# Nextomics/NextPolish2

Measured on AMD Instinct MI355X. Metric: polished reference Mbp/s (whole node) at 30x HiFi + k21/k31; FASTA identical to oracle, higher is better.
Workload: dtype u8

## Files before the change

### nextpolish2_amd/csrc/np2_cand.hip

```cpp
#include "np2_common.hpp"
#include "np2_kernels.hpp"
#include "np2_blockscan.hpp"
#include "np2_lookback.hpp"

namespace np2 {

template <int MODE>
__device__ __forceinline__ void k_scan_small(const uint32_t np2_bid, const uint32_t np2_nb, const uint32_t *__restrict__ in, uint32_t *__restrict__ out,
                                                     uint32_t n_host, const uint32_t *__restrict__ n_dev,
                                                     uint32_t *__restrict__ total_out, bool write_end) {
    __shared__ uint32_t sh[16];
    const uint32_t n = n_dev ? min(*n_dev, n_host) : n_host;
    uint32_t total;
    if (MODE == 2) {
        total = block_scan_array<OpMinI32>(
            n, sh, [&](uint32_t i) { return in[i]; },
            [&](uint32_t i, uint32_t pre, uint32_t v) { out[i] = OpMinI32::apply(pre, v); });
    } else {
        total = block_scan_array<OpAdd>(
            n, sh, [&](uint32_t i) { return in[i]; },
            [&](uint32_t i, uint32_t pre, uint32_t v) { out[i] = MODE == 0 ? pre : pre + v; });
    }
    if (threadIdx.x == 0) {
        if (MODE == 0 && write_end) out[n] = total;
        if (total_out) *total_out = total;
    }
}

static constexpr uint32_t SCAN_LB_ITEMS = 8;
static constexpr uint32_t SCAN_LB_THREADS = 1024;
static constexpr uint32_t SCAN_LB_BLOCK = SCAN_LB_ITEMS * SCAN_LB_THREADS;
template <bool POPC>
__device__ __forceinline__ void scan_lb_excl_body(const uint32_t np2_bid, const uint32_t np2_nb, Lookback lb, uint32_t n_blocks, const uint32_t *__restrict__ in,
                                                      uint32_t *__restrict__ out, uint32_t n, bool write_end,
                                                      uint32_t *__restrict__ err) {
    __shared__ uint32_t sh[16];
    const uint32_t bid = lb_block_id(lb, sh);
    const uint32_t i0 = bid * SCAN_LB_BLOCK + threadIdx.x * SCAN_LB_ITEMS;
    uint32_t v[SCAN_LB_ITEMS], sum = 0;
    const bool wide = (((uintptr_t)in | (uintptr_t)out) & 15) == 0;
    if (wide && i0 + SCAN_LB_ITEMS <= (POPC ? n - 1 : n)) {
        const uint4 a = *reinterpret_cast<const uint4 *>(in + i0), b = *reinterpret_cast<const uint4 *>(in + i0 + 4);
        v[0] = a.x, v[1] = a.y, v[2] = a.z, v[3] = a.w, v[4] = b.x, v[5] = b.y, v[6] = b.z, v[7] = b.w;
    } else {
#pragma unroll
        for (uint32_t k = 0; k < SCAN_LB_ITEMS; ++k) v[k] = i0 + k < (POPC ? n - 1 : n) ? in[i0 + k] : 0u;
    }
    if (POPC) {
#pragma unroll
        for (uint32_t k = 0; k < SCAN_LB_ITEMS; ++k) v[k] = (uint32_t)__builtin_popcount(v[k]);
    }
#pragma unroll
    for (uint32_t k = 0; k < SCAN_LB_ITEMS; ++k) sum += v[k];
    uint32_t total, pre, dummy;
    uint32_t run = block_excl_scan<OpAdd, 16>(sum, sh, total);
    lb_exclusive2(lb, bid, total, 0u, sh, err, pre, dummy);
    run += pre;
    if (wide && i0 + SCAN_LB_ITEMS <= n) {
        uint4 a, b;
        a.x = run, a.y = a.x + v[0], a.z = a.y + v[1], a.w = a.z + v[2];
        b.x = a.w + v[3], b.y = b.x + v[4], b.z = b.y + v[5], b.w = b.z + v[6];
        *reinterpret_cast<uint4 *>(out + i0) = a;
        *reinterpret_cast<uint4 *>(out + i0 + 4) = b;
        run = b.w + v[7];
    } else {
#pragma unroll
        for (uint32_t k = 0; k < SCAN_LB_ITEMS; ++k) {
            if (i0 + k < n) out[i0 + k] = run;
            run += v[k];
        }
    }
    if (write_end && n && i0 <= n - 1 && n - 1 < i0 + SCAN_LB_ITEMS) out[n] = run;
    if (write_end && n == 0 && bid == 0 && threadIdx.x == 0) out[0] = 0;
}

__device__ __forceinline__ void k_scan_lb_excl(const uint32_t np2_bid, const uint32_t np2_nb, Lookback lb, uint32_t n_blocks, const uint32_t *__restrict__ in,
                                               uint32_t *__restrict__ out, uint32_t n, bool write_end, uint32_t *__restrict__ err) {
    scan_lb_excl_body<false>(np2_bid, np2_nb, lb, n_blocks, in, out, n, write_end, err);
}
__device__ __forceinline__ void k_scan_lb_popc(const uint32_t np2_bid, const uint32_t np2_nb, Lookback lb, uint32_t n_blocks, const uint32_t *__restrict__ in,
                                               uint32_t *__restrict__ out, uint32_t n, bool write_end, uint32_t *__restrict__ err) {
    scan_lb_excl_body<true>(np2_bid, np2_nb, lb, n_blocks, in, out, n, write_end, err);
}

struct CandCtx {
    const np2_read_t *reads;
    const uint8_t *nib;
    const uint64_t *ck_off;
    const uint32_t *ckpt;
    const uint32_t *lq_start;
    const uint32_t *lq_end;
    const uint32_t *pj;
    const uint32_t *pcount;
    const uint8_t *alive;
    const ReadInfo *rinfo;
    const uint32_t *tile_rd_off;
    const uint32_t *tile_rd;
    uint32_t n_tiles;
    uint32_t ksize;
    const uint64_t *rec_key;
    const uint32_t *rec_read;
    const uint32_t *tile_n;
    const uint16_t *rec_pidx;
    uint32_t bucket_cap;
    const uint32_t *refnib;
    uint32_t L;
};

__device__ __forceinline__ void cand_anchor(const CandCtx &cx, uint32_t r, const np2_read_t &rd, uint64_t ck_off, uint32_t start,
                                            uint32_t &col, uint32_t &t) {
    col = 0;
    t = rd.aln_t_s;
    const uint32_t ck_first = (rd.aln_t_s + CKPT - 1) >> CKPT_SHIFT;
    const uint32_t cki = start >> CKPT_SHIFT;
    if (r == 0) {
        col = start;
        t = start;
    } else if (cki >= ck_first) {
        col = cx.ckpt[ck_off + (cki - ck_first)];
        t = cki << CKPT_SHIFT;
    }
}

__device__ __forceinline__ uint32_t nth_col16(uint64_t m64, uint32_t n) {
    uint32_t col = 0;
    uint32_t m = (uint32_t)m64;
    uint32_t c = (uint32_t)__builtin_popcount(m);
    if (n > c) n -= c, col = 8, m = (uint32_t)(m64 >> 32);
    c = (uint32_t)__builtin_popcount(m & 0xFFFFu);
    if (n > c) n -= c, col += 4, m >>= 16;
    c = (uint32_t)__builtin_popcount(m & 0xFFu);
    if (n > c) n -= c, col += 2, m >>= 8;
    c = (uint32_t)__builtin_popcount(m & 0xFu);
    if (n > c) col += 1;
    return col;
}

__device__ uint32_t cand_measure(const CandCtx &cx, uint32_t r, const np2_read_t &rd, uint64_t ck_off, uint32_t start,
                                 uint32_t end, uint32_t &col_start) {
    uint32_t col_ck, t_ck;
    cand_anchor(cx, r, rd, ck_off, start, col_ck, t_ck);
    col_start = col_ck;
    if (end < t_ck) return 0;
    const uint32_t want_s = (start > t_ck ? start - t_ck : 0u) + 1;
    const uint32_t want_e = end + 1 - t_ck + 1;
    const uint8_t *base = cx.nib + rd.nib_off;
    const uint32_t n_cols = rd.n_cols;
    uint32_t seen = 0, len = 0;
    bool started = false;
    uint4 win = make_uint4(0, 0, 0, 0);
    uint32_t win_blk = 0xFFFFFFFFu;
    const uint64_t N1 = 0x1111111111111111ULL;
    for (uint32_t wi = col_ck >> 4;; ++wi) {
        const uint32_t c0 = wi << 4;
        if (c0 >= n_cols) break;
        if ((wi >> 1) != win_blk) {
            win_blk = wi >> 1;
            win = *reinterpret_cast<const uint4 *>(base + ((size_t)win_blk << 4));
        }
        const uint32_t r0 = (wi & 1) ? win.z : win.x, r1 = (wi & 1) ? win.w : win.y;
        const uint64_t w = (uint64_t)(((r0 & 0x0F0F0F0Fu) << 4) | ((r0 >> 4) & 0x0F0F0F0Fu)) |
                           ((uint64_t)(((r1 & 0x0F0F0F0Fu) << 4) | ((r1 >> 4) & 0x0F0F0F0Fu)) << 32);
        uint64_t valid = N1;
        if (c0 < col_ck) valid &= ~((1ULL << (4 * (col_ck - c0))) - 1ULL);
        if (n_cols - c0 < 16) valid &= (1ULL << (4 * (n_cols - c0))) - 1ULL;
        uint64_t nonins = (~(w >> 3)) & valid;
        if (c0 == 0) nonins |= valid & 1ULL;
        const uint64_t x = (w & 0x7777777777777777ULL) ^ 0x4444444444444444ULL;
        const uint64_t nongap = (x | (x >> 1) | (x >> 2)) & valid;
        const uint32_t cn = (uint32_t)__builtin_popcountll(nonins);
        uint32_t lo = 0, hi = 16;
        bool done = false;
        if (!started && seen + cn >= want_s) {
            lo = nth_col16(nonins, want_s - seen);
            col_start = c0 + lo;
            started = true;
        }
        if (seen + cn >= want_e) {
            hi = nth_col16(nonins, want_e - seen);
            done = true;
        }
        if (started) {
            uint64_t m = nongap;
            if (lo) m &= ~((1ULL << (4 * lo)) - 1ULL);
            if (hi < 16) m &= (1ULL << (4 * hi)) - 1ULL;
            len += (uint32_t)__builtin_popcountll(m);
        }
        seen += cn;
        if (done) break;
    }
    return started ? len : 0u;
}

struct NibReader {
    const uint8_t *base;
    uint64_t w;
    uint32_t wbase;
    __device__ __forceinline__ uint8_t get(uint32_t c) {
        const uint32_t b = c & ~15u;
        if (b != wbase) {
            const uint2 v = *reinterpret_cast<const uint2 *>(base + (b >> 1));
            const uint32_t x = ((v.x & 0x0F0F0F0Fu) << 4) | ((v.x >> 4) & 0x0F0F0F0Fu);
            const uint32_t y = ((v.y & 0x0F0F0F0Fu) << 4) | ((v.y >> 4) & 0x0F0F0F0Fu);
            w = (uint64_t)x | ((uint64_t)y << 32);
            wbase = b;
        }
        return (uint8_t)((w >> (4 * (c & 15))) & 15);
    }
};

__device__ void cand_write(const CandCtx &cx, uint32_t r, const np2_read_t &rd, uint32_t pj, uint32_t g, uint32_t col, uint32_t t,
                           uint32_t len, uint8_t *__restrict__ seq_out, uint64_t *kmer_out) {
    const uint8_t *base = cx.nib + rd.nib_off;
    const uint32_t limit = cx.lq_end[pj] + cx.ksize;
    bool have_kmer = false;
    if (col + cx.ksize <= rd.n_cols) {
        const uint32_t k = cx.ksize, W0 = col >> 4, sh = (col & 15) * 4;
        auto ld = [&](uint32_t W) -> uint64_t {
            const uint2 v = *reinterpret_cast<const uint2 *>(base + ((size_t)W << 3));
            const uint32_t x = ((v.x & 0x0F0F0F0Fu) << 4) | ((v.x >> 4) & 0x0F0F0F0Fu);
            const uint32_t y = ((v.y & 0x0F0F0F0Fu) << 4) | ((v.y >> 4) & 0x0F0F0F0Fu);
            return (uint64_t)x | ((uint64_t)y << 32);
        };
        const uint64_t x0 = ld(W0), x1 = ld(W0 + 1), x2 = ld(W0 + 2);
        uint64_t lo = sh ? (x0 >> sh) | (x1 << (64 - sh)) : x0, hi = sh ? (x1 >> sh) | (x2 << (64 - sh)) : x1;
        auto nmask = [](uint32_t n) -> uint64_t { return n >= 16 ? ~0ULL : ((1ULL << (4 * n)) - 1ULL); };
        const uint64_t N1 = 0x1111111111111111ULL;
        const uint32_t avail = min(32u, rd.n_cols - col);
        const uint64_t a_lo = nmask(avail), a_hi = avail > 16 ? nmask(avail - 16) : 0ULL;
        const uint64_t ng_lo = ~(lo >> 2) & N1 & a_lo, ng_hi = ~(hi >> 2) & N1 & a_hi;
        const uint32_t c_lo = (uint32_t)__builtin_popcountll(ng_lo);
        if (c_lo + (uint32_t)__builtin_popcountll(ng_hi) >= k) {
            uint32_t kk = k, C = 0;
            uint64_t m = ng_lo;
            if (kk > c_lo) kk -= c_lo, C = 16, m = ng_hi;
            uint32_t c = (uint32_t)__builtin_popcount((uint32_t)m);
            if (kk > c) kk -= c, C += 8, m >>= 32;
            uint32_t m32 = (uint32_t)m;
            c = (uint32_t)__builtin_popcount(m32 & 0xFFFFu);
            if (kk > c) kk -= c, C += 4, m32 >>= 16;
            c = (uint32_t)__builtin_popcount(m32 & 0xFFu);
            if (kk > c) kk -= c, C += 2, m32 >>= 8;
            c = (uint32_t)__builtin_popcount(m32 & 0xFu);
            if (kk > c) C += 1;
            const uint64_t u_lo = nmask(C + 1), u_hi = C + 1 > 16 ? nmask(C + 1 - 16) : 0ULL;
            const uint64_t hi4_lo = (lo >> 2) & N1 & u_lo, hi4_hi = (hi >> 2) & N1 & u_hi;
            const bool plain = (((lo | (lo >> 1)) & hi4_lo) | ((hi | (hi >> 1)) & hi4_hi)) == 0;
            const uint64_t r_lo = nmask(C) & ~0xFULL, r_hi = C > 16 ? nmask(C - 16) : 0ULL;
            const uint32_t ins = (uint32_t)__builtin_popcountll(lo & r_lo & 0x8888888888888888ULL) +
                                 (uint32_t)__builtin_popcountll(hi & r_hi & 0x8888888888888888ULL);
            const uint32_t steps = C ? C - 1 : 0u;
            if (plain && t + (steps - ins) <= limit) {
                lo &= u_lo, hi &= u_hi;
                uint64_t g_lo = hi4_lo, g_hi = hi4_hi;
                while (g_lo | g_hi) {
                    if (g_lo) {
                        const uint64_t below = (g_lo & (0 - g_lo)) - 1;
                        lo = (lo & below) | (((lo >> 4) | (hi << 60)) & ~below);
                        g_lo = ((g_lo >> 4) | (g_hi << 60)) & ~below;
                        hi >>= 4;
                        g_hi >>= 4;
                    } else {
                        const uint64_t below = (g_hi & (0 - g_hi)) - 1;
                        hi = (hi & below) | ((hi >> 4) & ~below);
                        g_hi = (g_hi >> 4) & ~below;
                    }
                }
                auto squeeze = [](uint64_t x) -> uint64_t {
                    uint64_t y = x & 0x3333333333333333ULL;
                    y = (y | (y >> 2)) & 0x0F0F0F0F0F0F0F0FULL;
                    y = (y | (y >> 4)) & 0x00FF00FF00FF00FFULL;
                    y = (y | (y >> 8)) & 0x0000FFFF0000FFFFULL;
                    return (y | (y >> 16)) & 0xFFFFFFFFULL;
                };
                const uint64_t mask = (1ULL << (2 * (uint64_t)k)) - 1;
                const uint64_t codes = (squeeze(lo) | (squeeze(hi) << 32)) & mask;
                uint64_t rb = __builtin_bitreverse64(codes);
                rb = ((rb >> 1) & 0x5555555555555555ULL) | ((rb & 0x5555555555555555ULL) << 1);
                const uint64_t fw = rb >> (64 - 2 * k), rv = ~codes & mask;
                *kmer_out = yak_hash64(fw < rv ? fw : rv, mask);
                have_kmer = true;
            }
        }
    }
    if (!have_kmer) {
        NibReader nr{base, 0, 0xFFFFFFFFu};
        const uint64_t ksize = cx.ksize, shift = 2 * (ksize - 1), mask = (1ULL << (2 * ksize)) - 1;
        uint64_t fw = 0, rv = 0, l = 0;
        for (uint32_t c = col; c < rd.n_cols && l < ksize; ++c) {
            const uint8_t nb = nr.get(c);
            if (c != col && !(nb & 8)) ++t;
            const uint8_t q = nb & 7;
            if (q != 4) {
                fw = ((fw << 2) | (uint64_t)q) & mask;
                rv = (rv >> 2) | ((3ULL ^ (uint64_t)q) << shift);
                ++l;
            }
            if (t > limit) break;
        }
        uint64_t km = INVALID_KMER;
        if (l >= ksize) km = yak_hash64(fw < rv ? fw : rv, mask);
        *kmer_out = km;
    }
    const uint32_t LUT_LO = 0x54474341u, LUT_HI = 0x004D4E2Du;
    uint32_t o = 0;
    for (uint32_t wi = col >> 3; o < len; ++wi) {
        const uint32_t raw = *reinterpret_cast<const uint32_t *>(base + ((size_t)wi << 2));
        uint32_t w = (((raw & 0x0F0F0F0Fu) << 4) | ((raw >> 4) & 0x0F0F0F0Fu)) & 0x77777777u;
        uint32_t nc = 8;
        if (wi == (col >> 3)) {
            const uint32_t skip = col & 7;
            w >>= 4 * skip;
            nc = 8 - skip;
        }
        const uint32_t vm = nc == 8 ? 0x11111111u : ((1u << (4 * nc)) - 1u) & 0x11111111u;
        const uint32_t x = w ^ 0x44444444u;
        uint32_t gap = ~(x | (x >> 1) | (x >> 2)) & vm;
        const uint32_t cnt = min(nc - (uint32_t)__builtin_popcount(gap), len - o);
        while (gap) {
            const uint32_t below = (gap & (0u - gap)) - 1u;
            w = (w & below) | ((w >> 4) & ~below);
            gap = (gap >> 4) & ~below;
        }
        const uint32_t lo4 = w & 0xFFFFu, hi4 = w >> 16;
        uint32_t s0 = (lo4 | (lo4 << 8)) & 0x00FF00FFu, s1 = (hi4 | (hi4 << 8)) & 0x00FF00FFu;
        s0 = (s0 | (s0 << 4)) & 0x0F0F0F0Fu;
        s1 = (s1 | (s1 << 4)) & 0x0F0F0F0Fu;
        const uint32_t a0 = __builtin_amdgcn_perm(LUT_HI, LUT_LO, s0), a1 = __builtin_amdgcn_perm(LUT_HI, LUT_LO, s1);
        if (cnt == 8) {
            __builtin_memcpy(seq_out + o, &a0, 4);
            __builtin_memcpy(seq_out + o + 4, &a1, 4);
        } else {
            const uint64_t a = (uint64_t)a0 | ((uint64_t)a1 << 32);
#pragma unroll
            for (uint32_t k = 0; k < 7; ++k)
                if (k < cnt) seq_out[o + k] = (uint8_t)(a >> (8 * k));
        }
        o += cnt;
    }
}

__device__ __forceinline__ uint32_t wave_sum(uint32_t v) {
    for (int o = 32; o > 0; o >>= 1) v += __shfl_xor(v, o);
    return v;
}
__device__ __forceinline__ uint32_t wave_excl(uint32_t v) {
    const uint32_t lane = threadIdx.x & 63;
    uint32_t x = v;
#pragma unroll
    for (int o = 1; o < 64; o <<= 1) {
        const uint32_t t = __shfl_up(x, o);
        if (lane >= (uint32_t)o) x += t;
    }
    return x - v;
}

static constexpr uint32_t RM_WAVES = 8;
static constexpr uint32_t RM_RPW = 4;
static_assert(RM_RPW % 4 == 0 && RM_RPW <= 16, "regions per wavefront");
static constexpr uint32_t RM_REG = 4 * RM_RPW;
static constexpr uint32_t CAND_CLEAN = 0xFFFFFFFFu;
static constexpr uint32_t CLEAN_MAX_LEN = 64;

__device__ __forceinline__ void wave_lds_sync() {
    __builtin_amdgcn_fence(__ATOMIC_RELEASE, "wavefront");
    __builtin_amdgcn_wave_barrier();
    __builtin_amdgcn_fence(__ATOMIC_ACQUIRE, "wavefront");
}
__device__ __forceinline__ uint32_t lanes_below(uint64_t m) {
    return __builtin_amdgcn_mbcnt_hi((uint32_t)(m >> 32), __builtin_amdgcn_mbcnt_lo((uint32_t)m, 0u));
}
__device__ __forceinline__ np2_read_t rinfo_read(const ReadInfo &ri) {
    return np2_read_t{ri.aln_t_s, ri.aln_t_e, (uint64_t)ri.nib16 << 4, ri.n_cols, 0u};
}

__device__ __forceinline__ void region_measure_inline(const CandCtx &cx, uint32_t g, uint32_t st, uint32_t en, uint32_t la, uint32_t lb,
                                                      uint32_t *__restrict__ kept_read, uint32_t *__restrict__ kept_len,
                                                      uint32_t *__restrict__ kept_col, uint32_t &kept, uint32_t &bytes, uint32_t &mx) {
    const uint32_t lane = threadIdx.x & 63;
    kept = 0, bytes = 0, mx = 0;
    for (uint32_t c0 = la; c0 < lb && kept < LQSEQ_MAX_CAN_COUNT; c0 += 64) {
        const uint32_t i = c0 + lane;
        uint32_t r = 0, len = 0, col = 0;
        if (i < lb) {
            r = cx.tile_rd[i];
            const ReadInfo ri = cx.rinfo[r];
            if (ri.pcount != 0 && ri.pj <= g && g - ri.pj < ri.pcount) len = cand_measure(cx, r, rinfo_read(ri), ri.ck_off, st, en, col);
        }
        const uint64_t ne = __ballot(len > 0);
        const uint32_t before = kept + lanes_below(ne);
        const bool keep = len > 0 && before < LQSEQ_MAX_CAN_COUNT;
        if (keep) {
            const size_t slot = (size_t)g * LQSEQ_MAX_CAN_COUNT + before;
            kept_read[slot] = r;
            kept_len[slot] = len;
            kept_col[slot] = col;
        }
        kept = min(kept + (uint32_t)__builtin_popcountll(ne), (uint32_t)LQSEQ_MAX_CAN_COUNT);
        bytes += wave_sum(keep ? len : 0u);
        mx = max(mx, keep ? len : 0u);
    }
    for (int o = 32; o > 0; o >>= 1) mx = max(mx, (uint32_t)__shfl_xor(mx, o));
}

__device__ __forceinline__ void k_region_measure(const uint32_t np2_bid0, const uint32_t np2_nb, CandCtx cx, uint32_t n_reg, uint32_t *__restrict__ kept_read,
                                                        uint32_t *__restrict__ kept_len, uint32_t *__restrict__ kept_col,
                                                        uint32_t *__restrict__ reg_ncand, uint32_t *__restrict__ reg_bytes,
                                                        uint32_t *__restrict__ reg_maxlen, uint32_t *__restrict__ blk_sum) {
    const uint32_t np2_bid = xcd_order(np2_bid0, np2_nb);
    __shared__ uint32_t s_reads[RM_REG][64];
    __shared__ uint32_t s_dm[RM_REG][2];
    __shared__ uint32_t s_len[RM_REG][64];
    __shared__ uint32_t s_col[RM_REG][64];
    __shared__ uint32_t s_q[4][RM_RPW * 64];
    const uint32_t lane = threadIdx.x & 63, wv = (uint32_t)__builtin_amdgcn_readfirstlane((int)(threadIdx.x >> 6));
    const uint32_t n_mb = (n_reg + 3) / 4, g0 = (np2_bid * 4 + wv) * RM_RPW, mb0 = g0 / 4;
    uint32_t nq = 0;
    uint32_t st[RM_RPW], en[RM_RPW], tile[RM_RPW], la[RM_RPW], lb[RM_RPW], tn[RM_RPW];
    bool live[RM_RPW];
#pragma unroll
    for (uint32_t h = 0; h < RM_RPW; ++h) {
        const uint32_t g = g0 + h;
        live[h] = g < n_reg;
        const uint32_t gg = live[h] ? g : n_reg - 1;
        st[h] = cx.lq_start[gg], en[h] = cx.lq_end[gg];
    }
#pragma unroll
    for (uint32_t h = 0; h < RM_RPW; ++h) {
        tile[h] = min(en[h] >> TILE_SHIFT, cx.n_tiles - 1);
        la[h] = cx.tile_rd_off[tile[h]], lb[h] = cx.tile_rd_off[tile[h] + 1];
        tn[h] = cx.rec_pidx ? cx.tile_n[tile[h]] : 0u;
    }
    const ReadInfo r0 = cx.rinfo[0];
    uint32_t rr[RM_RPW], lo[RM_RPW], hi[RM_RPW], refw[RM_RPW];
    bool wok[RM_RPW];
#pragma unroll
    for (uint32_t h = 0; h < RM_RPW; ++h) {
        const uint32_t g = g0 + h, nlist = lb[h] - la[h], we = en[h] + cx.ksize + 2;
        wok[h] = live[h] && cx.rec_pidx != nullptr && nlist != 0 && nlist <= 64 && en[h] - st[h] + 1 <= CLEAN_MAX_LEN && we < cx.L &&
                 (st[h] >> TILE_SHIFT) == tile[h] && (we >> TILE_SHIFT) == tile[h] && tn[h] <= cx.bucket_cap &&
                 r0.pcount != 0 && r0.pj <= g && g - r0.pj < r0.pcount;
        rr[h] = (wok[h] && lane < nlist) ? cx.tile_rd[la[h] + lane] : 0xFFFFFFFFu;
        const uint32_t w0 = st[h] >> 3, w1 = (en[h] + cx.ksize) >> 3;
        refw[h] = 0;
        if (wok[h] && w0 + lane <= w1) {
            uint32_t m = 0x44444444u;
            if (lane == 0) m &= 0xFFFFFFFFu << (4 * (st[h] & 7));
            if (w0 + lane == w1) m &= 0xFFFFFFFFu >> (4 * (7 - ((en[h] + cx.ksize) & 7)));
            refw[h] = cx.refnib[w0 + lane] & m;
        }
        lo[h] = 0, hi[h] = 0;
        if (wok[h] && tn[h]) {
            const uint32_t tstart = tile[h] << TILE_SHIFT;
            const uint32_t j0 = (st[h] - tstart) >> 4, j1 = ((we - tstart) >> 4) + 1;
            lo[h] = cx.rec_pidx[(size_t)tile[h] * (TILE / 16) + j0];
            hi[h] = j1 < TILE / 16 ? (uint32_t)cx.rec_pidx[(size_t)tile[h] * (TILE / 16) + j1] : tn[h];
        }
    }
    uint32_t pjv[RM_RPW], pcv[RM_RPW], tev[RM_RPW], rpos[RM_RPW], rq[RM_RPW];
#pragma unroll
    for (uint32_t h = 0; h < RM_RPW; ++h) {
        pjv[h] = 0, pcv[h] = 0, tev[h] = 0, rpos[h] = 0xFFFFFFFFu, rq[h] = 0;
        if (rr[h] != 0xFFFFFFFFu) {
            const uint4 q = *reinterpret_cast<const uint4 *>(&cx.rinfo[rr[h]].aln_t_e);
            tev[h] = q.x, pjv[h] = q.y, pcv[h] = q.z;
        }
        const uint32_t i = lo[h] + lane;
        if (i < hi[h]) {
            const uint64_t a = (uint64_t)tile[h] * cx.bucket_cap + i;
            rpos[h] = (uint32_t)(cx.rec_key[a] >> 32), rq[h] = cx.rec_read[a];
        }
    }
    uint32_t fastmask = 0;
#pragma unroll
    for (uint32_t h = 0; h < RM_RPW; ++h) {
        const uint32_t slot = wv * RM_RPW + h;
        const bool fast = wok[h] && (uint32_t)__builtin_amdgcn_readfirstlane((int)rr[h]) == 0 && __ballot(refw[h] != 0) == 0;
        if (fast) fastmask |= 1u << h;
        s_reads[slot][lane] = rr[h];
        if (lane < 2) s_dm[slot][lane] = 0;
    }
    wave_lds_sync();
    auto mark = [&](uint32_t slot, uint32_t nlist, uint32_t pos, uint32_t q, uint32_t ws, uint32_t we) {
        if (pos >= ws && pos <= we) {
            uint32_t x = 0, y = nlist;
            while (x < y) {
                const uint32_t m = (x + y) >> 1;
                if (s_reads[slot][m] < q) x = m + 1; else y = m;
            }
            if (x < nlist && s_reads[slot][x] == q) atomicOr(&s_dm[slot][x >> 5], 1u << (x & 31));
        }
    };
#pragma unroll
    for (uint32_t h = 0; h < RM_RPW; ++h) {
        if (!((fastmask >> h) & 1u)) continue;
        const uint32_t slot = wv * RM_RPW + h, nlist = lb[h] - la[h], ws = st[h], we = en[h] + cx.ksize + 2;
        mark(slot, nlist, rpos[h], rq[h], ws, we);
        for (uint32_t c0 = lo[h] + 64; c0 < hi[h]; c0 += 64) {
            const uint32_t i = c0 + lane;
            if (i < hi[h]) {
                const uint64_t a = (uint64_t)tile[h] * cx.bucket_cap + i;
                mark(slot, nlist, (uint32_t)(cx.rec_key[a] >> 32), cx.rec_read[a], ws, we);
            }
        }
    }
    wave_lds_sync();
    uint32_t state[RM_RPW];
#pragma unroll
    for (uint32_t h = 0; h < RM_RPW; ++h) {
        state[h] = 0;
        if (!((fastmask >> h) & 1u)) continue;
        const uint32_t g = g0 + h, slot = wv * RM_RPW + h;
        const bool paired = rr[h] != 0xFFFFFFFFu && pcv[h] != 0 && pjv[h] <= g && g - pjv[h] < pcv[h];
        const bool marked = (s_dm[slot][lane >> 5] >> (lane & 31)) & 1u;
        const bool ends_inside = tev[h] < en[h] + cx.ksize;
        const uint32_t stt = !paired ? 0u : ((marked || ends_inside) && rr[h] != 0) ? 2u : 1u;
        state[h] = stt;
        const uint64_t dq = __ballot(stt == 2u);
        if (stt == 2u) s_q[wv][nq + lanes_below(dq)] = (slot << 6) | lane;
        nq += (uint32_t)__builtin_popcountll(dq);
    }
    uint32_t sum_k[RM_RPW / 4] = {}, sum_b[RM_RPW / 4] = {}, sum_m[RM_RPW / 4] = {};
#pragma unroll
    for (uint32_t h = 0; h < RM_RPW; ++h) {
        if (!live[h] || ((fastmask >> h) & 1u)) continue;
        const uint32_t g = g0 + h;
        uint32_t kept, bytes, mx;
        region_measure_inline(cx, g, st[h], en[h], la[h], lb[h], kept_read, kept_len, kept_col, kept, bytes, mx);
        if (lane == 0) {
            reg_ncand[g] = kept;
            reg_bytes[g] = bytes;
            reg_maxlen[g] = mx;
        }
        sum_k[h / 4] += kept, sum_b[h / 4] += bytes, sum_m[h / 4] += mx;
    }
    wave_lds_sync();
    for (uint32_t e = lane; e < nq; e += 64) {
        const uint32_t w = s_q[wv][e], slot = w >> 6, ln = w & 63;
        const uint32_t g = (np2_bid * 4 + slot / RM_RPW) * RM_RPW + slot % RM_RPW;
        const uint32_t r = s_reads[slot][ln];
        const ReadInfo ri = cx.rinfo[r];
        uint32_t col = 0;
        const uint32_t len = cand_measure(cx, r, rinfo_read(ri), ri.ck_off, cx.lq_start[g], cx.lq_end[g], col);
        s_len[slot][ln] = len;
        s_col[slot][ln] = col;
    }
    wave_lds_sync();
#pragma unroll
    for (uint32_t h = 0; h < RM_RPW; ++h) {
        if (!((fastmask >> h) & 1u)) continue;
        const uint32_t g = g0 + h, slot = wv * RM_RPW + h;
        uint32_t len = 0, col = CAND_CLEAN;
        if (state[h] == 1u) len = en[h] - st[h] + 1;
        else if (state[h] == 2u) len = s_len[slot][lane], col = s_col[slot][lane];
        const uint64_t ne = __ballot(len > 0);
        const uint32_t before = lanes_below(ne);
        const bool keep = len > 0 && before < LQSEQ_MAX_CAN_COUNT;
        if (keep) {
            const size_t ks = (size_t)g * LQSEQ_MAX_CAN_COUNT + before;
            kept_read[ks] = rr[h];
            kept_len[ks] = len;
            kept_col[ks] = col;
        }
        const uint32_t kept = min((uint32_t)__builtin_popcountll(ne), (uint32_t)LQSEQ_MAX_CAN_COUNT);
        const uint32_t bytes = wave_sum(keep ? len : 0u);
        uint32_t mx = keep ? len : 0u;
        for (int o = 32; o > 0; o >>= 1) mx = max(mx, (uint32_t)__shfl_xor(mx, o));
        if (lane == 0) {
            reg_ncand[g] = kept;
            reg_bytes[g] = bytes;
            reg_maxlen[g] = mx;
        }
        sum_k[h / 4] += kept, sum_b[h / 4] += bytes, sum_m[h / 4] += mx;
    }
#pragma unroll
    for (uint32_t q = 0; q < RM_RPW / 4; ++q)
        if (lane == 0 && mb0 + q < n_mb) {
            blk_sum[mb0 + q] = sum_k[q];
            blk_sum[n_mb + mb0 + q] = sum_b[q];
            blk_sum[2 * n_mb + mb0 + q] = sum_m[q];
        }
}

__device__ __forceinline__ void k_cand_offsets(const uint32_t np2_bid, const uint32_t np2_nb, const uint32_t *__restrict__ blk_sum, uint32_t n_blk,
                                                       uint32_t n_reg, uint32_t *__restrict__ blk_coff,
                                                       uint32_t *__restrict__ blk_soff, uint32_t *__restrict__ cand_off,
                                                       uint32_t *__restrict__ reg_soff, uint32_t *__restrict__ n_cand,
                                                       uint32_t *__restrict__ n_bytes, uint32_t *__restrict__ grow) {
    __shared__ uint32_t sh[16];
    const uint32_t ta = block_scan_array<OpAdd>(
        n_blk, sh, [&](uint32_t i) { return blk_sum[i]; }, [&](uint32_t i, uint32_t pre, uint32_t) { blk_coff[i] = pre; });
    const uint32_t tb = block_scan_array<OpAdd>(
        n_blk, sh, [&](uint32_t i) { return blk_sum[n_blk + i]; },
        [&](uint32_t i, uint32_t pre, uint32_t) { blk_soff[i] = pre; });
    const uint32_t tc = block_scan_array<OpAdd>(
        n_blk, sh, [&](uint32_t i) { return blk_sum[2 * n_blk + i]; }, [&](uint32_t, uint32_t, uint32_t) {});
    if (threadIdx.x == 0) {
        cand_off[n_reg] = ta;
        reg_soff[n_reg] = tb;
        *n_cand = ta;
        *n_bytes = tb;
        *grow = tc;
    }
}

__device__ __forceinline__ void k_cand_offsets_lb(const uint32_t np2_bid, const uint32_t np2_nb, Lookback lb, uint32_t n_blocks, const uint32_t *__restrict__ blk_sum,
                                                         uint32_t n_blk, uint32_t n_reg, uint32_t *__restrict__ blk_coff,
                                                         uint32_t *__restrict__ blk_soff, uint32_t *__restrict__ cand_off,
                                                         uint32_t *__restrict__ reg_soff, uint32_t *__restrict__ n_cand,
                                                         uint32_t *__restrict__ n_bytes, uint32_t *__restrict__ grow,
                                                         uint32_t *__restrict__ err) {
    __shared__ uint32_t sh[8];
    const uint32_t bid = lb_block_id(lb, sh);
    const uint32_t i0 = (bid * 256 + threadIdx.x) * 4;
    uint32_t a[4], b[4], sa = 0, sb = 0;
#pragma unroll
    for (uint32_t k = 0; k < 4; ++k) {
        a[k] = i0 + k < n_blk ? blk_sum[i0 + k] : 0u;
        b[k] = i0 + k < n_blk ? blk_sum[n_blk + i0 + k] : 0u;
        sa += a[k];
        sb += b[k];
    }
    uint32_t ta, tb, pa, pb;
    uint32_t ra = block_excl_scan<OpAdd, 4>(sa, sh, ta);
    uint32_t rb = block_excl_scan<OpAdd, 4>(sb, sh, tb);
    lb_exclusive2(lb, bid, ta, tb, sh, err, pa, pb);
    ra += pa, rb += pb;
#pragma unroll
    for (uint32_t k = 0; k < 4; ++k)
        if (i0 + k < n_blk) {
            blk_coff[i0 + k] = ra;
            blk_soff[i0 + k] = rb;
            ra += a[k];
            rb += b[k];
        }
    if (bid == n_blocks - 1 && threadIdx.x == 255) {
        cand_off[n_reg] = ra;
        reg_soff[n_reg] = rb;
        *n_cand = ra;
        *n_bytes = rb;
    }
    if (bid == 0) {
        uint32_t c = 0, tc;
        for (uint32_t i = threadIdx.x; i < n_blk; i += 256) c += blk_sum[2 * n_blk + i];
        (void)block_excl_scan<OpAdd, 4>(c, sh, tc);
        if (threadIdx.x == 0) *grow = tc;
    }
}

static constexpr uint32_t MERGE_LB_BLOCKS = 32;
__device__ __forceinline__ void k_lq_merge_scan_lb(const uint32_t np2_bid, const uint32_t np2_nb, Lookback lb, const uint32_t *__restrict__ raw_start,
                                                   const uint32_t *__restrict__ raw_end, const uint32_t *__restrict__ n_raw, uint32_t n_host,
                                                   uint32_t *__restrict__ headflag, uint32_t *__restrict__ hidx, uint32_t *__restrict__ err) {
    __shared__ uint32_t sh[16];
    const uint32_t bid = lb_block_id(lb, sh);
    const uint32_t n = min(*n_raw, n_host);
    const uint32_t seg = ((n + MERGE_LB_BLOCKS - 1) / MERGE_LB_BLOCKS + 1023u) & ~1023u;
    const uint32_t lo = min(bid * seg, n), hi = min(lo + seg, n);
    auto flag = [&](uint32_t j) { return (j >= 1 && raw_end[j] >= raw_start[j - 1]) ? 0u : 1u; };
    uint32_t cnt = 0;
    for (uint32_t j = lo + threadIdx.x; j < hi; j += 1024) cnt += flag(j);
    uint32_t total, pre, dummy;
    (void)block_excl_scan<OpAdd, 16>(cnt, sh, total);
    lb_exclusive2(lb, bid, total, 0u, sh, err, pre, dummy);
    uint32_t carry = pre;
    for (uint32_t j0 = lo; j0 < hi; j0 += 1024) {
        const uint32_t j = j0 + threadIdx.x;
        const uint32_t v = j < hi ? flag(j) : 0u;
        uint32_t tot;
        const uint32_t ex = block_excl_scan<OpAdd, 16>(v, sh, tot);
        if (j < hi) {
            hidx[j] = carry + ex;
            headflag[j] = v;
        }
        carry += tot;
    }
}

__device__ __forceinline__ void k_region_write(const uint32_t np2_bid0, const uint32_t np2_nb, CandCtx cx, uint32_t n_reg, const uint32_t *__restrict__ kept_read,
                                                      const uint32_t *__restrict__ kept_len,
                                                      const uint32_t *__restrict__ kept_col,
                                                      const uint32_t *__restrict__ reg_ncand,
                                                      const uint32_t *__restrict__ reg_bytes,
                                                      const uint32_t *__restrict__ blk_coff,
                                                      const uint32_t *__restrict__ blk_soff,
                                                      uint32_t *__restrict__ cand_off, uint32_t *__restrict__ reg_soff,
                                                      uint32_t cand_cap,
                                                      uint32_t seq_cap, uint32_t *__restrict__ cand_order,
                                                      uint64_t *__restrict__ cand_kmer, uint32_t *__restrict__ cand_seq_off,
                                                      uint8_t *__restrict__ cand_seq) {
    const uint32_t np2_bid = xcd_order(np2_bid0, np2_nb);
    __shared__ __attribute__((aligned(4))) uint8_t s_str[RM_REG][CLEAN_MAX_LEN];
    __shared__ uint64_t s_km[RM_REG];
    __shared__ uint32_t s_so[RM_REG][64];
    __shared__ uint32_t s_oc[RM_REG];
    __shared__ uint32_t s_q[4][RM_RPW * 64];
    const uint32_t lane = threadIdx.x & 63, wv = (uint32_t)__builtin_amdgcn_readfirstlane((int)(threadIdx.x >> 6));
    const uint32_t g0 = (np2_bid * 4 + wv) * RM_RPW, mb0 = g0 / 4;
    uint32_t nq = 0;
    uint32_t oc = 0, ob = 0;
    if (g0 < n_reg) oc = blk_coff[mb0], ob = blk_soff[mb0];
    uint32_t clean_h = 0;
    uint32_t my_len[RM_RPW], my_so[RM_RPW], my_ci[RM_RPW];
    bool my_clean[RM_RPW];
    uint32_t n[RM_RPW], rb[RM_RPW], st[RM_RPW], ln0[RM_RPW];
#pragma unroll
    for (uint32_t h = 0; h < RM_RPW; ++h) {
        const uint32_t g = g0 + h;
        n[h] = 0, rb[h] = 0, st[h] = 0, ln0[h] = 0;
        if (g < n_reg) n[h] = reg_ncand[g], rb[h] = reg_bytes[g], st[h] = cx.lq_start[g], ln0[h] = cx.lq_end[g] - st[h] + 1;
    }
    uint32_t len[RM_RPW], col[RM_RPW], rd_[RM_RPW], refc[RM_RPW];
#pragma unroll
    for (uint32_t h = 0; h < RM_RPW; ++h) {
        const size_t ks = (size_t)(g0 + h) * LQSEQ_MAX_CAN_COUNT + lane;
        const bool act = lane < n[h];
        len[h] = act ? kept_len[ks] : 0u;
        col[h] = act ? kept_col[ks] : 0u;
        rd_[h] = act ? kept_read[ks] : 0u;
        const uint32_t p = st[h] + lane;
        refc[h] = (n[h] && lane < ln0[h] && ln0[h] <= CLEAN_MAX_LEN) ? cx.refnib[p >> 3] >> (4 * (p & 7)) : 0u;
    }
#pragma unroll
    for (uint32_t h = 0; h < RM_RPW; ++h) {
        const uint32_t g = g0 + h, slot = wv * RM_RPW + h;
        my_len[h] = 0, my_so[h] = 0, my_ci[h] = 0, my_clean[h] = false;
        if (g >= n_reg) continue;
        if (g == n_reg - 1 && lane == 0 && cand_off[n_reg] < cand_cap) cand_seq_off[cand_off[n_reg]] = reg_soff[n_reg];
        if (lane == 0) {
            cand_off[g] = oc;
            reg_soff[g] = ob;
            s_oc[slot] = oc;
        }
        const bool act = lane < n[h];
        const uint32_t so = ob + wave_excl(len[h]);
        const uint32_t ci = oc + lane;
        const bool ok = act && ci < cand_cap && (uint64_t)so + len[h] <= seq_cap;
        if (ok) {
            cand_order[ci] = rd_[h];
            cand_seq_off[ci] = so;
        }
        const bool clean = ok && col[h] == CAND_CLEAN;
        const uint64_t cm = __ballot(clean);
        const bool queued = ok && (!clean || (lane == 0 && rd_[h] == 0));
        my_len[h] = len[h], my_so[h] = so, my_ci[h] = ci, my_clean[h] = clean && !queued;
        s_so[slot][lane] = so;
        if (cm) {
            clean_h |= 1u << h;
            if (lane < ln0[h]) s_str[slot][lane] = (uint8_t)((0x54474341u >> (8 * (refc[h] & 3))) & 0xFFu);
        }
        const uint64_t dq = __ballot(queued);
        if (queued) s_q[wv][nq + lanes_below(dq)] = (slot << 6) | lane;
        nq += (uint32_t)__builtin_popcountll(dq);
        oc += n[h];
        ob += rb[h];
    }
    wave_lds_sync();
    for (uint32_t e = lane; e < nq; e += 64) {
        const uint32_t w = s_q[wv][e], slot = w >> 6, li = w & 63;
        const uint32_t g = (np2_bid * 4 + slot / RM_RPW) * RM_RPW + slot % RM_RPW;
        const size_t ks = (size_t)g * LQSEQ_MAX_CAN_COUNT + li;
        const uint32_t r = kept_read[ks], len = kept_len[ks];
        uint32_t col = kept_col[ks];
        const ReadInfo ri = cx.rinfo[r];
        const np2_read_t rd = rinfo_read(ri);
        const uint32_t t0 = max(cx.lq_start[g], rd.aln_t_s);
        if (col == CAND_CLEAN) col = t0;
        const uint32_t ci = s_oc[slot] + li;
        uint64_t km;
        cand_write(cx, r, rd, ri.pj, g, col, t0, len, cand_seq + s_so[slot][li], &km);
        cand_kmer[ci] = km;
        if (li == 0 && r == 0) s_km[slot] = km;
    }
    wave_lds_sync();
#pragma unroll
    for (uint32_t h = 0; h < RM_RPW; ++h) {
        if (!((clean_h >> h) & 1u)) continue;
        const uint32_t slot = wv * RM_RPW + h;
        if (my_clean[h]) {
            cand_kmer[my_ci[h]] = s_km[slot];
            typedef uint32_t u32_any __attribute__((aligned(1)));
            uint8_t *dst = cand_seq + my_so[h];
            const uint32_t L4 = my_len[h] & ~3u;
            for (uint32_t j = 0; j < L4; j += 4) *reinterpret_cast<u32_any *>(dst + j) = *reinterpret_cast<const uint32_t *>(&s_str[slot][j]);
            for (uint32_t j = L4; j < my_len[h]; ++j) dst[j] = s_str[slot][j];
        }
    }
}

void launch_scan_small_excl(hipStream_t s, const uint32_t *in, uint32_t *out, uint32_t n, const uint32_t *n_dev,
                            uint32_t *total_out, bool write_end) {
    NP2_LAUNCH(k_scan_small<0>, dim3(1), 1024, s, in, out, n, n_dev, total_out, write_end);
}
void launch_scan_lb_excl(hipStream_t s, const Lookback &lb, const uint32_t *in, uint32_t *out, uint32_t n, bool write_end,
                          uint32_t *err) {
    const uint32_t nb = scan_lb_blocks(n);
    NP2_LAUNCH(k_scan_lb_excl, dim3(nb), SCAN_LB_THREADS, s, lb, nb, in, out, n, write_end, err);
}
void launch_scan_lb_popc(hipStream_t s, const Lookback &lb, const uint32_t *bits, uint32_t *out, uint32_t n_words, uint32_t *err) {
    const uint32_t nb = scan_lb_blocks((uint64_t)n_words + 1);
    NP2_LAUNCH(k_scan_lb_popc, dim3(nb), SCAN_LB_THREADS, s, lb, nb, bits, out, n_words + 1, false, err);
}
uint32_t scan_lb_blocks(uint64_t n) { return (uint32_t)std::max<uint64_t>(1, (n + SCAN_LB_BLOCK - 1) / SCAN_LB_BLOCK); }
void launch_scan_small_incl(hipStream_t s, const int32_t *in, int32_t *out, uint32_t n, const uint32_t *n_dev) {
    NP2_LAUNCH(k_scan_small<1>, dim3(1), 1024, s, (const uint32_t *)in, (uint32_t *)out, n, n_dev, (uint32_t *)nullptr, false);
}
void launch_scan_small_min(hipStream_t s, const int32_t *in, int32_t *out, uint32_t n, const uint32_t *n_dev) {
    NP2_LAUNCH(k_scan_small<2>, dim3(1), 1024, s, (const uint32_t *)in, (uint32_t *)out, n, n_dev, (uint32_t *)nullptr, false);
}
static CandCtx mk_cand(const CandPtrs &c) {
    return CandCtx{c.reads, c.nib,    c.ck_off, c.ckpt,        c.lq_start, c.lq_end, c.pj,
                   c.pcount, c.alive, c.rinfo, c.tile_rd_off, c.tile_rd, c.n_tiles,  c.ksize,
                   c.rec_key, c.rec_read, c.tile_n, c.rec_pidx, c.bucket_cap, c.refnib, c.L};
}
void launch_region_measure(hipStream_t s, const CandPtrs &c, uint32_t n_reg, uint32_t *kept_read, uint32_t *kept_len,
                           uint32_t *kept_col, uint32_t *reg_ncand, uint32_t *reg_bytes, uint32_t *reg_maxlen,
                           uint32_t *blk_sum) {
    if (n_reg)
        NP2_LAUNCH_WAVES(k_region_measure, RM_WAVES, dim3((n_reg + RM_REG - 1) / RM_REG), 256, s,
                         mk_cand(c), n_reg, kept_read, kept_len, kept_col, reg_ncand, reg_bytes, reg_maxlen, blk_sum);
}
uint32_t cand_offsets_blocks(uint32_t n_reg) { return ((n_reg + 3) / 4 + 1023) / 1024; }
void launch_cand_offsets(hipStream_t s, const uint32_t *blk_sum, uint32_t n_reg, uint32_t *blk_coff, uint32_t *blk_soff,
                         uint32_t *cand_off, uint32_t *reg_soff, uint32_t *n_cand, uint32_t *n_bytes, uint32_t *grow,
                         const Lookback *lb, uint32_t *err) {
    if (lb)
        NP2_LAUNCH(k_cand_offsets_lb, dim3(cand_offsets_blocks(n_reg)), 256, s, *lb, cand_offsets_blocks(n_reg), blk_sum, (n_reg + 3) / 4, n_reg, blk_coff, blk_soff, cand_off, reg_soff, n_cand, n_bytes, grow, err);
    else
        NP2_LAUNCH(k_cand_offsets, dim3(1), 1024, s, blk_sum, (n_reg + 3) / 4, n_reg, blk_coff, blk_soff, cand_off, reg_soff, n_cand, n_bytes, grow);
}
void launch_lq_merge_scan_lb(hipStream_t s, const Lookback &lb, const uint32_t *raw_start, const uint32_t *raw_end, const uint32_t *n_raw,
                             uint32_t n_host, uint32_t *headflag, uint32_t *hidx, uint32_t *err) {
    NP2_LAUNCH(k_lq_merge_scan_lb, dim3(MERGE_LB_BLOCKS), 1024, s, lb, raw_start, raw_end, n_raw, n_host, headflag, hidx, err);
}
uint32_t lq_merge_lb_blocks() { return MERGE_LB_BLOCKS; }
void launch_region_write(hipStream_t s, const CandPtrs &c, uint32_t n_reg, const uint32_t *kept_read,
                         const uint32_t *kept_len, const uint32_t *kept_col, const uint32_t *reg_ncand,
                         const uint32_t *reg_bytes, const uint32_t *blk_coff, const uint32_t *blk_soff, uint32_t *cand_off,
                         uint32_t *reg_soff, uint32_t cand_cap, uint32_t seq_cap, uint32_t *cand_order, uint64_t *cand_kmer,
                         uint32_t *cand_seq_off, uint8_t *cand_seq) {
    if (n_reg)
        NP2_LAUNCH(k_region_write, dim3((n_reg + RM_REG - 1) / RM_REG), 256, s, mk_cand(c), n_reg, kept_read, kept_len, kept_col, reg_ncand, reg_bytes, blk_coff, blk_soff, cand_off, reg_soff, cand_cap, seq_cap, cand_order, cand_kmer, cand_seq_off, cand_seq);
}

}
```

### nextpolish2_amd/csrc/np2_ctx.hpp

```cpp
#pragma once
#include "../../include/np2.h"
#include "np2_abi.hpp"
#include "np2_common.hpp"
#include "np2_kernels.hpp"
#include "np2_hostcpu.hpp"

#include <algorithm>
#include <chrono>
#include <cstdio>
#include <cstdlib>
#include <cstring>
#include <map>
#include <memory>
#include <exception>
#include <mutex>
#include <stdexcept>
#include <string>
#include <vector>

namespace np2h {

using namespace np2;


// ... 273 lines not shown
        }
        return true;
    }
};
inline PinnedPool &pinned_pool() {
    static PinnedPool *p = new PinnedPool();
    return *p;
}

struct PinnedBuf {
    void *p = nullptr;
    size_t cap = 0;
    ~PinnedBuf() {
        if (p) pinned_pool().put(p);
    }
    void *ensure(size_t n) {
        if (n > cap) {
            if (p) pinned_pool().put(p);
            p = nullptr;
            cap = 0;
            const size_t want = n + n / 4 + 65536;
            p = pinned_pool().get(want);
            if (!p) throw Np2Error(NP2_E_NOMEM, "hipHostMalloc failed");
            cap = want;
        }
        return p;
    }
};

struct CtxDeviceState {
    hipStream_t stream = nullptr, stream_out = nullptr;
    hipEvent_t ev_out = nullptr;
    uint32_t *mbox_host = nullptr, *mbox_dev = nullptr;
    void destroy() {
        if (ev_out) (void)hipEventDestroy(ev_out);
        if (stream_out) (void)hipStreamDestroy(stream_out);
        if (stream) (void)hipStreamDestroy(stream);
        if (mbox_host) (void)hipHostFree(mbox_host);
        *this = CtxDeviceState();
    }
};
struct CtxStatePool {
    std::mutex mu;
    std::map<int, std::vector<CtxDeviceState>> idle;
    bool get(int device, CtxDeviceState &out) {
        std::lock_guard<std::mutex> l(mu);
        auto &v = idle[device];
        if (v.empty()) return false;
        out = v.back();
        v.pop_back();
        return true;
    }
    void put(int device, CtxDeviceState &st) {
        {
            std::lock_guard<std::mutex> l(mu);
            auto &v = idle[device];
            if (v.size() < 32) {
                v.push_back(st);
                st = CtxDeviceState();
                return;
            }
        }
        st.destroy();
    }
};
inline CtxStatePool &ctx_state_pool() {
    static CtxStatePool *p = new CtxStatePool();
    return *p;
}

struct YakTable {
    uint32_t k = 0, cap_log2 = 0;
    std::shared_ptr<DevBuf<uint64_t>> table;
    std::shared_ptr<DevBuf<uint32_t>> ord;
    YakDev dev() const { return YakDev{table->p, cap_log2, k, ord ? ord->p : nullptr}; }
};

struct Timing {
    std::vector<std::string> names;
    std::vector<float> ms;
    std::string joined;
    std::vector<std::pair<std::string, float>> host;
};
inline double now_ms() {
    return std::chrono::duration<double, std::milli>(std::chrono::steady_clock::now().time_since_epoch()).count();
}


}

using namespace np2h;

struct np2_contig {
    np2_contig() {
        reads.cached = nib.cached = refnib.cached = ck_off.cached = ckpt.cached = descs.cached = true;
        tile_rd_off.cached = tile_rd.cached = true;
    }
    uint32_t L = 0, R = 0;
    uint64_t nib_bytes = 0, n_cols = 0, n_ckpt = 0;
    DevBuf<np2_read_t> reads;
    DevBuf<uint8_t> nib;
    DevBuf<uint8_t> refnib;
    uint32_t ref_stride = 0;
    DevBuf<uint64_t> ck_off;
    DevBuf<uint32_t> ckpt;
    uint32_t n_chunks = 0;
    DevBuf<ChunkDesc> descs;
    uint32_t n_tiles = 0;
    DevBuf<uint32_t> tile_rd_off, tile_rd;
    uint32_t tile_cap = TILE_CAP;
};

struct np2_ctx {
    int device = 0;
    hipStream_t stream = nullptr;
    hipStream_t stream_out = nullptr;
    hipEvent_t ev_out = nullptr;
    uint8_t *out_host[2] = {nullptr, nullptr};
    size_t out_host_cap[2] = {0, 0};
    int out_slot = 0;
    bool out_pending = false;
    uint64_t out_len = 0;
    std::vector<YakTable> yaks;
    std::string err;
    bool trace = false;
    std::map<std::string, std::vector<uint8_t>> trace_items;
    Timing timing;
    std::vector<std::pair<std::string, std::pair<hipEvent_t, hipEvent_t>>> pending_events;

    PinnedBuf pin_d2h, pin_h2d;
    uint32_t *mbox_host = nullptr, *mbox_dev = nullptr;
    uint32_t mbox_seq = 0;
    bool borrowed_state = false;
    uint8_t *sink_dst = nullptr;
    uint64_t sink_cap = 0;
    uint32_t last_first_pos = 0, last_last_pos = 0;
    const uint8_t *last_dbase = nullptr;
    const uint32_t *last_dpos = nullptr;
    DevBuf<uint32_t> shard_bounds;
    uint64_t last_len = 0;
    bool reuse_identical_pass = true;
    bool h2d_inflight = false;
    bool stage_timing = false;
    DevBuf<uint8_t> tmp;
    DevBuf<uint64_t> keys_raw, keys;
    DevBuf<uint32_t> vals_raw, vals;
    DevBuf<uint32_t> npos, ncount, nminr, nbesti, node_off, run_start, run_end, n0_besti, emit, eoff;
    DevBuf<uint16_t> nbases, ndelta;
    DevBuf<int64_t> nscore;
    DevBuf<int32_t> cov, mval, smin;
    DevBuf<uint8_t> alive, cns_base, cns_cls, lq_kind, lq_nothead;
    DevBuf<uint32_t> cns_pos, lq_next, rflag, rstart, rend, ridx, raw_start, raw_end, headflag, hidx, lq_start,
        lq_end;
    DevBuf<uint32_t> pj, pcount, reg_ncand, reg_bytes, reg_soff, reg_maxlen, blk_sum, blk_coff, blk_soff, kept_read, kept_len, kept_col, cand_off, cand_order, cand_seq_off, kill_ids;
    DevBuf<uint64_t> cand_kmer;
    DevBuf<uint8_t> cand_seq;
    DevBuf<uint16_t> kscore;
    DevBuf<uint32_t> scal;
    DevBuf<uint64_t> lb_status;
    DevBuf<uint32_t> lb_ticket;
    uint32_t lb_ticket_total = 0, lb_epoch = 0;
    bool lb_dirty = false;
    static constexpr size_t LB_MAX_BLOCKS = 1u << 20;
    DevBuf<uint32_t> mlen;
    DevBuf<uint8_t> reg_lable, grp, cns_base2, rech_groups, rech_groups_tmp;
    DevBuf<uint8_t> votepack;
    DevBuf<uint8_t> votepack2;
    DevBuf<uint32_t> rech_headjobs;
    DevBuf<uint32_t> ecount, eval, eval_s, eflag, eidx, seed_cand, keep_n, keep_list, cns_pos2, sp_idx_s,
        sp_idx_e, ap_g, ap_s, ap_e, rech, rech_joboff, job_len,
        job_off32;
    DevBuf<int32_t> ew, ap_delta, ap_shift;
    DevBuf<uint64_t> ekey, ekey_s;
    DevBuf<uint16_t> keep_ks;
    DevBuf<uint32_t> long_list;
    DevBuf<uint64_t> bt_path;
    DevBuf<uint64_t> chunk_st;
    uint32_t chunk_epoch = 0;
    DevBuf<uint32_t> tile_cur, tile_n, tile_scan, tile_scanb, tile_nn, tile_nr, tile_noff, tile_roff;
    uint32_t tile_cap = TILE_CAP;
    uint32_t bucket_cap = 0;
    DevBuf<uint2> nrec;
    DevBuf<uint8_t> votebuf;
    DevBuf<uint32_t> band, band_n, band_off;
    DevBuf<int64_t> run_gain, tile_gain;
    DevBuf<uint8_t> out_snap;
    DevBuf<uint8_t> run_flag;
    uint32_t deep_min = 65536;
    DevBuf<uint32_t> lq_list, hbits;
    DevBuf<uint16_t> tile_pidx;
    bool pidx_valid = false;
    DevBuf<ReadInfo> rinfo;
    DevBuf<uint32_t> lqc, lqoff;
    DevBuf<uint8_t> pflag;
    DevBuf<uint32_t> dp_list;
    DevBuf<uint16_t> pf_slots;
    DevBuf<uint32_t> pf_bad, pf_bad2;
    DevBuf<uint64_t> pf_prof;
    bool front_fused = false;
    struct Hooks {
        bool front_unfused = false, pf_prof = false, edge_sort = false;
        bool test_misspeculate = false, shard_spec_log = false, phase_profile = false, exact_grow = false, no_speculate = false;
        bool has_grow_guess = false;
        uint32_t grow_guess = 0;
        bool has_pf_cap = false, has_pf_cap_big = false, has_pf_halo = false, has_pf_cov_max = false;
        uint32_t pf_cap = 0, pf_cap_big = 0, pf_halo = 0, pf_cov_max = 0;
        void read() {
            auto on = [](const char *n) { return getenv(n) != nullptr; };
            auto u32 = [](const char *n, bool &has, uint32_t &v) {
                if (const char *e = getenv(n)) has = true, v = (uint32_t)atol(e);
            };
            front_unfused = on("NP2_FRONT_UNFUSED"), pf_prof = on("NP2_PF_PROF"), edge_sort = on("NP2_EDGE_SORT");
            test_misspeculate = on("NP2_TEST_MISSPECULATE");
            shard_spec_log = on("NP2_SHARD_SPEC_LOG"), phase_profile = on("NP2_PHASE_PROFILE"), exact_grow = on("NP2_EXACT_GROW");
            no_speculate = on("NP2_NO_SPECULATE");
            u32("NP2_TEST_GROW_GUESS", has_grow_guess, grow_guess);
            u32("NP2_PF_CAP", has_pf_cap, pf_cap), u32("NP2_PF_CAP_BIG", has_pf_cap_big, pf_cap_big);
            u32("NP2_PF_HALO", has_pf_halo, pf_halo), u32("NP2_PF_COV_MAX", has_pf_cov_max, pf_cov_max);
        }
    } hooks;
    bool pf_big = getenv("NP2_PF_BIG") != nullptr;
    uint32_t front_redos = 0;
    DevBuf<uint16_t> kscore_saved;
    DevBuf<uint8_t> sstr;
    DevBuf<uint64_t> soff;
    DevBuf<uint16_t> sscore;
};


namespace np2h {


enum Scal { S_ERR = 0, S_NNODES, S_NRUNS, S_BEST, S_PATHBEGIN, S_NRAW, S_NREG, S_DUP, S_LAST0, S_LAST1, S_GAIN0,
            S_GAIN1, S_DEEP, S_NDPLIST, S_NRECH, S_NGROUPS, S_NLONG, S_NLQ, S_PF, S_M0, S_M1, S_M2, S_M3, S_NC, S_SB, S_GROW,
            S_NBAD, S_PFOUT, S_PFGAIN0, S_PFGAIN1, S_PFEND0, S_PFEND1, S_NBAD2, S_PFPAD, S_COUNT = 34 };
static_assert(S_M1 % 2 == 0 && S_LAST0 % 2 == 0 && S_GAIN0 % 2 == 0 && S_PFGAIN0 % 2 == 0 && S_PFEND0 % 2 == 0,
              "64-bit device counters live in these slot pairs");

static constexpr int NP2_MAX_YAK = 15;
static constexpr uint32_t SCAL_TOTAL = 96;
static_assert(S_COUNT + 2 * (NP2_MAX_YAK + 2) <= SCAL_TOTAL && S_COUNT < 64, "round counters behind the posted block; the mailbox holds 64 words");

inline double thread_cpu_ms() {
    timespec ts;
    clock_gettime(CLOCK_THREAD_CPUTIME_ID, &ts);
    return ts.tv_sec * 1e3 + ts.tv_nsec * 1e-6;
}
struct WallTimer {
    np2_ctx *cx;
    const char *name;
    double t0, c0 = 0;
    WallTimer(np2_ctx *c, const char *n);
    ~WallTimer();
};

struct EventTimer {
    np2_ctx *cx;
    hipEvent_t a = nullptr, b = nullptr;
    bool on;
    EventTimer(np2_ctx *c, const char *name, bool always = false)
        : cx(c), on((always || c->stage_timing) && !tl_recorder()) {
        if (!on) return;
        (void)hipEventCreate(&a);
        (void)hipEventCreate(&b);
        (void)hipEventRecord(a, cx->stream);
        cx->pending_events.push_back({name, {a, b}});
    }
    ~EventTimer() {
        if (on) (void)hipEventRecord(b, cx->stream);
    }
};

inline WallTimer::WallTimer(np2_ctx *c, const char *n) : cx(c), name(n), t0(c->stage_timing ? now_ms() : 0.0), c0(c->stage_timing ? thread_cpu_ms() : 0.0) {}
inline WallTimer::~WallTimer() {
    if (cx->stage_timing) {
        cx->timing.host.push_back({name, (float)(now_ms() - t0)});
        if (strncmp(name, "wall", 4) == 0) cx->timing.host.push_back({std::string("cpu") + (name + 4), (float)(thread_cpu_ms() - c0)});
    }
}

inline void flush_timings(np2_ctx *cx) {
    std::map<std::string, float> acc;
    std::vector<std::string> order;
    for (auto &e : cx->pending_events) {
        float ms = 0;
        (void)hipEventSynchronize(e.second.second);
        (void)hipEventElapsedTime(&ms, e.second.first, e.second.second);
        if (!acc.count(e.first)) order.push_back(e.first);
        acc[e.first] += ms;
        (void)hipEventDestroy(e.second.first);
        (void)hipEventDestroy(e.second.second);
    }
    cx->pending_events.clear();
    for (auto &h : cx->timing.host) {
        if (!acc.count(h.first)) order.push_back(h.first);
        acc[h.first] += h.second;
    }
    cx->timing.host.clear();
    cx->timing.names = order;
    cx->timing.ms.clear();
    cx->timing.joined.clear();
    for (auto &n : order) {
        cx->timing.ms.push_back(acc[n]);
        cx->timing.joined += n;
        cx->timing.joined.push_back('\0');
    }
    cx->timing.joined.push_back('\0');
}
// ... 193 lines not shown
```

### nextpolish2_amd/csrc/np2_host.cpp

```cpp
#include "../../include/np2.h"
#include "np2_common.hpp"
#include "np2_kernels.hpp"
#include "np2_ctx.hpp"
#include "np2_phase_host.hpp"

#include <algorithm>
#include <atomic>
#include <thread>
#include <chrono>
#include <cstdio>
#include <cstdlib>
#include <cstring>
#include <map>
#include <mutex>
#include <stdexcept>
#include <string>
#include <unordered_map>
#include <unordered_set>
#include <future>
#include <functional>
#include <vector>

using namespace np2;

// ... 773 lines not shown
        launch_dp_short(s, gp, c->refnib.p, cx->run_start.p, cx->scal.p + S_NRUNS, n_runs, cx->run_end.p, cx->run_gain.p,
                        cx->emit.p, cx->scal.p + S_PATHBEGIN, cx->bt_path.p, dp_list, n_dp_list);
        launch_dp_long(s, gp, cx->run_start.p, n_runs, cx->nrec.p, cx->nscore.p, cx->nbesti.p, cx->n0_besti.p,
                       cx->run_end.p, (int64_t *)(cx->scal.p + S_LAST0), cx->run_gain.p, cx->emit.p,
                       cx->scal.p + S_PATHBEGIN, cx->bt_path.p, cx->run_flag.p, dp_list, n_dp_list);
        launch_dp_finish(s, gp, cx->run_start.p, cx->scal.p + S_NRUNS, cx->nscore.p, cx->nbesti.p, cx->n0_besti.p,
                         (const int64_t *)(cx->scal.p + S_LAST0), (unsigned long long *)(cx->scal.p + S_GAIN0),
                         cx->scal.p + S_DUP , cx->scal.p + S_BEST,
                         cx->run_gain.p, (const long long *)cx->tile_gain.p,
                         (c->L + TILE - 1) >> TILE_SHIFT, cx->emit.p, cx->scal.p + S_PATHBEGIN, cx->bt_path.p);
        exclusive_total(cx, cx->emit.p, cx->eoff.p, (size_t)L + 1);
        launch_bt_write(s, gp, cx->run_start.p, cx->scal.p + S_NRUNS, n_runs, cx->emit.p, cx->eoff.p, cx->bt_path.p,
                        cx->cns_pos.p, cx->cns_base.p, cx->cns_cls.p, cx->lq_nothead.p, cx->lqc.p);
        exclusive_total(cx, cx->lqc.p, cx->lqoff.p, (size_t)n_runs + 1);
        launch_lq_list(s, gp, cx->run_start.p, cx->scal.p + S_NRUNS, n_runs, cx->emit.p, cx->eoff.p, cx->bt_path.p,
                       cx->lqoff.p, lq_cap, cx->lq_list.p, cx->scal.p + S_ERR);
        launch_default_tail(s, gp, cx->scal.p + S_BEST, M_p, cx->cns_base.p, cx->cns_cls.p, cx->lq_list.p,
                            cx->lqoff.p + n_runs, lq_cap, cx->scal.p + S_ERR);
    }
    lq_regions_issue(cx, cb, M_p, n_lq);
}

bool front_can_fuse(np2_ctx *cx) {
    return !cx->hooks.front_unfused && cx->bucket_cap != 0 && cx->pidx_valid;
}
void pass_front_fused_issue(np2_ctx *cx, np2_contig *c, uint32_t T) {
    hipStream_t s = cx->stream;
    const uint32_t L = c->L;
    const uint32_t n_tiles = (L + TILE - 1) >> TILE_SHIFT;
    const CnsBounds cb = cns_buffers(cx, c, T, std::min<uint32_t>(T, L), T);
    cx->pf_slots.ensure(pf_slot_entries(n_tiles, T));
    cx->pf_bad.ensure((size_t)n_tiles + 2);
    cx->pf_bad2.ensure((size_t)n_tiles + 2);
    const np2_ctx::Hooks &hk = cx->hooks;
    const uint32_t cap_lim = hk.has_pf_cap ? hk.pf_cap : PF_CAP, cap_big = hk.has_pf_cap_big ? hk.pf_cap_big : PF_CAP_BIG,
                   halo_lim = (hk.has_pf_halo ? hk.pf_halo : PF_HALO) & ~15u, cov_max = hk.has_pf_cov_max ? hk.pf_cov_max : PF_COV_MAX;
    PfTile a{cx->keys_raw.p, cx->vals_raw.p, cx->tile_n.p, cx->tile_scan.p, cx->tile_pidx.p, cx->alive.p, c->reads.p,
             c->tile_rd_off.p, c->tile_rd.p, c->refnib.p, cx->pf_slots.p, cx->tile_nn.p, cx->tile_nr.p,
             (long long *)cx->tile_gain.p, cx->scal.p + S_PF, cx->scal.p + S_NBAD, cx->pf_bad.p, cx->scal.p + S_NBAD2, cx->pf_bad2.p,
             (long long *)(cx->scal.p + S_PFEND0), (unsigned long long *)(cx->scal.p + S_PFGAIN0), nullptr, L, n_tiles, cx->bucket_cap,
             cap_lim, cap_big, halo_lim, std::min(cov_max, cx->deep_min), cx->pf_big ? 1u : 0u};
    uint32_t *const M_p = cx->eoff.p + L;
    uint32_t *const n_lq = cx->scal.p + S_NRUNS;
    const bool prof = cx->hooks.pf_prof && tl_recorder() == nullptr;
    if (prof) {
        cx->pf_prof.ensure((size_t)n_tiles * 8 + 8);
        zero32(cx, cx->pf_prof.p, (size_t)n_tiles * 8, 8);
        a.prof = (unsigned long long *)cx->pf_prof.p;
    }
    {
        EventTimer t(cx, "pass_front");
        launch_pf_tile(s, a);
        if (prof) {
            auto st = d2h(cx, cx->pf_prof.p, (size_t)n_tiles * 8);
            double sum[8] = {0}, mx[8] = {0};
            size_t cnt = 0;
            for (uint32_t t = 0; t < n_tiles; ++t) {
                const uint64_t *q = st.data() + (size_t)t * 8;
                if (!q[7] || !q[0]) continue;
                ++cnt;
                for (int i = 1; i < 8; ++i) {
                    const double d = (double)(q[i] - q[i - 1]);
                    sum[i] += d, mx[i] = std::max(mx[i], d);
                }
            }
            {
                auto tn = d2h(cx, cx->tile_n.p, n_tiles);
                uint32_t h[6] = {0};
                for (uint32_t v : tn) ++h[v <= 480 ? 0 : v <= 960 ? 1 : v <= 1440 ? 2 : v <= 1920 ? 3 : v <= 3584 ? 4 : 5];
                fprintf(stderr, "[pf_prof] records per tile <=480 / 960 / 1440 / 1920 / 3584 / more: %u %u %u %u %u %u; ", h[0], h[1], h[2], h[3], h[4], h[5]);
            }
            fprintf(stderr, "listed for the middle / the big variant: %u / %u; ", d2h(cx, cx->scal.p + S_NBAD, 1)[0], d2h(cx, cx->scal.p + S_NBAD2, 1)[0]);
            fprintf(stderr, "tiles %zu of %u; mean / max clocks per phase (loads, cover+nodes, offsets+sort, DP, reduce, count+scan, write):", cnt, n_tiles);
            for (int i = 1; i < 8; ++i) fprintf(stderr, " %.0f/%.0f", cnt ? sum[i] / cnt : 0.0, mx[i]);
            fprintf(stderr, "\n");
        }
        const bool wide = n_tiles >= 2048;
        Lookback lb{};
        if (wide) lb = next_lookback(cx, tile_scan_blocks(n_tiles));
        launch_tile_offsets(s, cx->tile_nn.p, cx->tile_nr.p, n_tiles, cx->tile_noff.p, cx->tile_roff.p, M_p, n_lq,
                            cx->scal.p + S_BEST, S_NLQ + 1 - S_BEST, wide ? &lb : nullptr, cx->scal.p + S_ERR,
                            (const long long *)cx->tile_gain.p, (unsigned long long *)(cx->scal.p + S_PFGAIN0));
        launch_pf_compact(s, n_tiles, cx->pf_slots.p, cx->tile_scan.p, cx->tile_nn.p, cx->tile_noff.p, cx->tile_roff.p,
                          cx->cns_pos.p, cx->cns_base.p, cx->cns_cls.p, cx->lq_nothead.p, cx->lq_list.p, cb.lq_cap,
                          cx->scal.p + S_ERR, cx->scal.p + S_PF, cx->scal.p + S_PFOUT, cx->scal.p + S_NBAD, cx->scal.p + S_NBAD2);
    }
    lq_regions_issue(cx, cb, M_p, n_lq);
}

void pass_front_issue(np2_ctx *cx, np2_contig *c, uint32_t T, int pass, bool force_unfused = false) {
    cx->front_fused = !force_unfused && front_can_fuse(cx);
    if (!cx->front_fused || cx->trace) {
        uint32_t n_nodes = 0, n_runs = 0;
        {
            WallTimer w(cx, "wall_graph");
            build_graph(cx, c, T, n_nodes, n_runs);
        }
        trace_graph(cx, c, pass, n_nodes);
        if (!cx->front_fused) {
            consensus_and_regions_issue(cx, c, n_nodes, n_runs, T);
            return;
        }
    }
    pass_front_fused_issue(cx, c, T);
}
void consensus_and_regions_finish(np2_ctx *cx, np2_contig *c, uint32_t T, int pass, uint32_t &M, uint32_t &n_reg, bool whole_contig = true) {
    const uint32_t *M_p = cx->eoff.p + c->L;
    std::vector<uint32_t> sc = fetch_scal(cx, cx->scal.p + S_M0, M_p);
    if (cx->front_fused) {
        const int64_t total = (int64_t)(((uint64_t)sc[S_PFGAIN1] << 32) | sc[S_PFGAIN0]);
        const int64_t end_rel = (int64_t)(((uint64_t)sc[S_PFEND1] << 32) | sc[S_PFEND0]);
        const bool negative = end_rel <= SCORE_NEG / 2 || total + end_rel < 0;
        if (sc[S_PFOUT] & PF_NEED_BIG) cx->pf_big = true;
        if ((sc[S_PFOUT] & PF_REDO) || negative) {
            ++cx->front_redos;
            cx->timing.host.push_back({"front_redo", 1.0f});
            pass_front_issue(cx, c, T, pass, true);
            sc = fetch_scal(cx, cx->scal.p + S_M0, M_p);
        }
    }
    check_region_err(cx, sc[S_ERR]);
    if (!cx->front_fused && sc[S_BEST] == 0xFFFFFFFFu && !whole_contig)
        throw Np2Error(NP2_E_UNSUPPORTED,
                       "best path score is negative at the end of a shard (the reference's default node is chosen by the whole "
                       "contig's score): polish this contig unsharded");
    M = sc[S_M0];
    if (M == 0) throw Np2Error(NP2_E_REFPANIC, "reference would panic: empty consensus");
    n_reg = sc[S_NRAW] ? sc[S_NREG] : 0;
}

void extract_candidates(np2_ctx *cx, np2_contig *c, uint32_t n_reg, uint16_t min_kmer_count, int pass,
                        PassCounts &pc) {
    hipStream_t s = cx->stream;
    const uint32_t R = c->R;
    REFPANIC_IF(cx->yaks.empty(), "index out of bounds: opt.yak[0]");
    if ((uint64_t)n_reg * LQSEQ_MAX_CAN_COUNT >= 0xFFFFFFF0ull) throw Np2Error(NP2_E_NOMEM, "too many LQ regions");
    const uint32_t NC_cap = n_reg * LQSEQ_MAX_CAN_COUNT;
    static const uint64_t exact_from = getenv("NP2_CAND_EXACT_FROM") ? strtoull(getenv("NP2_CAND_EXACT_FROM"), nullptr, 10) : (1ull << 28);
    const bool exact_bytes = c->n_cols >= exact_from && !cx->trace;
    uint32_t SB_cap = (uint32_t)std::min<uint64_t>(c->n_cols + 64, 0xFFFFFFF0ull);
    cx->mval.ensure(R + 2);
    cx->smin.ensure(R + 2);
    cx->pj.ensure(R + 2);
    cx->pcount.ensure(R + 2);
    cx->rinfo.ensure(R + 2);
    cx->reg_ncand.ensure(n_reg + 2);
    cx->reg_bytes.ensure(n_reg + 2);
    cx->reg_soff.ensure(n_reg + 2);
    cx->reg_maxlen.ensure(n_reg + 2);
    cx->blk_sum.ensure(3 * ((size_t)n_reg / 4 + 2));
    cx->blk_coff.ensure((size_t)n_reg / 4 + 2);
    cx->blk_soff.ensure((size_t)n_reg / 4 + 2);
    cx->cand_off.ensure(n_reg + 2);
    cx->kept_read.ensure((size_t)NC_cap + 2);
    cx->kept_len.ensure((size_t)NC_cap + 2);
    cx->kept_col.ensure((size_t)NC_cap + 2);
    cx->cand_order.ensure((size_t)NC_cap + 2);
    cx->cand_kmer.ensure((size_t)NC_cap + 2);
    cx->cand_seq_off.ensure((size_t)NC_cap + 2);
    if (!exact_bytes) cx->cand_seq.ensure((size_t)SB_cap + 64);
    cx->kscore.ensure((size_t)NC_cap + 2);
    cx->long_list.ensure((size_t)NC_cap + 2);
    CandPtrs cp{c->reads.p,   c->nib.p,   c->ck_off.p,      c->ckpt.p,    cx->lq_start.p, cx->lq_end.p, cx->pj.p,
                cx->pcount.p, cx->alive.p, cx->rinfo.p, c->tile_rd_off.p, c->tile_rd.p, c->n_tiles, cx->yaks[0].k,
                cx->keys_raw.p, cx->vals_raw.p, cx->tile_n.p,
                (cx->pidx_valid && cx->bucket_cap) ? cx->tile_pidx.p : nullptr, cx->bucket_cap,
                (const uint32_t *)c->refnib.p, c->L};
    {
        EventTimer t(cx, "candidates");
        launch_read_m(s, c->reads.p, R, cx->alive.p, cx->lq_start.p, n_reg, cx->mval.p);
        scan_incl_min(cx, cx->mval.p, cx->smin.p, R);
        launch_pair_count(s, c->reads.p, R, cx->alive.p, cx->lq_start.p, cx->lq_end.p, n_reg, cx->smin.p, cx->pj.p,
                          cx->pcount.p, c->ck_off.p, cx->rinfo.p);
        launch_region_measure(s, cp, n_reg, cx->kept_read.p, cx->kept_len.p, cx->kept_col.p, cx->reg_ncand.p,
                              cx->reg_bytes.p, cx->reg_maxlen.p, cx->blk_sum.p);
        {
            const bool wide = n_reg > 0;
            Lookback lb{};
            if (wide) lb = next_lookback(cx, cand_offsets_blocks(n_reg));
            launch_cand_offsets(s, cx->blk_sum.p, n_reg, cx->blk_coff.p, cx->blk_soff.p, cx->cand_off.p, cx->reg_soff.p,
                                cx->scal.p + S_NC, cx->scal.p + S_SB, cx->scal.p + S_GROW, wide ? &lb : nullptr,
                                cx->scal.p + S_ERR);
        }
        if (exact_bytes) {
            const std::vector<uint32_t> sc = fetch_scal(cx);
            check_region_err(cx, sc[S_ERR]);
            pc.resolve(sc);
            SB_cap = (uint32_t)std::min<uint64_t>((uint64_t)pc.SB + 64, SB_cap);
            cx->cand_seq.ensure((size_t)SB_cap + 64);
        }
        launch_region_write(s, cp, n_reg, cx->kept_read.p, cx->kept_len.p, cx->kept_col.p, cx->reg_ncand.p,
                            cx->reg_bytes.p, cx->blk_coff.p, cx->blk_soff.p, cx->cand_off.p, cx->reg_soff.p, NC_cap + 1,
                            SB_cap, cx->cand_order.p, cx->cand_kmer.p, cx->cand_seq_off.p, cx->cand_seq.p);
    }
    {
        EventTimer t(cx, "kmer_score");
        launch_cand_score(s, cx->yaks[0].dev(), cx->cand_seq_off.p, cx->cand_seq.p, cx->cand_kmer.p, cx->scal.p + S_NC,
                          NC_cap, min_kmer_count, cx->kscore.p, cx->long_list.p, cx->scal.p + S_NLONG);
    }
    pc.n_reg = n_reg;
    pc.NC_cap = NC_cap;
    pc.SB_cap = SB_cap;
    pc.known = exact_bytes;
    if (cx->trace) pc.resolve(fetch_scal(cx));
    trace_region_tables(cx, pass, "cand", pc, false);
}

Cns fetch_cns(np2_ctx *cx, uint32_t M) {
    Cns c;
    c.pos = d2h(cx, cx->cns_pos.p, M);
    c.base = d2h(cx, cx->cns_base.p, M);
    return c;
}

struct ResultOut {
    uint8_t *bases = nullptr;
    uint32_t *pos = nullptr;
    uint64_t len = 0;
    bool want_pos = true;
    bool want_bases = true;
    void release() {
        if (bases) pinned_pool().put(bases), bases = nullptr;
        if (pos) pinned_pool().put(pos), pos = nullptr;
    }
};
void fetch_result(np2_ctx *cx, const uint32_t *dpos, const uint8_t *dbase, const uint32_t *M_p, uint32_t M_cap, ResultOut &r,
                  uint32_t M_likely = 0xFFFFFFFFu) {
    const double t0 = now_ms();
    std::vector<uint32_t> sc;
    if (cx->sink_dst && cx->sink_cap) launch_copy_len(cx->stream, cx->sink_dst, dbase, M_p, 1, cx->sink_cap);
    if (r.want_bases || r.want_pos) {
        const uint32_t seq = ++cx->mbox_seq;
        launch_post(cx->stream, cx->scal.p, S_COUNT, cx->mbox_dev, seq, cx->scal.p + S_M0, M_p, nullptr, nullptr, nullptr, nullptr,
                    nullptr, nullptr, dpos, cx->scal.p + S_M1);
        if (r.want_bases) r.bases = (uint8_t *)pinned_pool().get((size_t)M_cap + 1);
        if (r.want_pos) r.pos = (uint32_t *)pinned_pool().get(((size_t)M_cap + 1) * 4);
        if ((r.want_bases && !r.bases) || (r.want_pos && !r.pos)) throw Np2Error(NP2_E_NOMEM, "pinned result allocation failed");
        uint32_t first = std::min(M_cap, M_likely);
        const bool exact_b = r.want_bases && op_d2h_len(cx, r.bases, dbase, M_p, 1, M_cap);
        const bool exact_p = r.want_pos && op_d2h_len(cx, r.pos, dpos, M_p, 4, (size_t)M_cap * 4);
        if (r.want_bases && !exact_b) op_d2h(cx, r.bases, dbase, first);
        if (r.want_pos && !exact_p) op_d2h(cx, r.pos, dpos, (size_t)first * 4);
        if ((exact_b || !r.want_bases) && (exact_p || !r.want_pos)) first = M_cap;
        op_sync(cx);
        if (__atomic_load_n(&cx->mbox_host[0], __ATOMIC_ACQUIRE) != seq)
            throw Np2Error(NP2_E_DEVICE, "mailbox not posted after a synchronisation");
        sc.assign(cx->mbox_host + 1, cx->mbox_host + 1 + S_COUNT);
        if (sc[S_M0] > first && sc[S_M0] <= M_cap) {
            const uint32_t rest = sc[S_M0] - first;
            if (r.want_bases) op_d2h(cx, r.bases + first, dbase + first, rest);
            if (r.want_pos) op_d2h(cx, r.pos + first, dpos + first, (size_t)rest * 4);
            op_sync(cx);
        }
    } else {
        sc = fetch_scal(cx, cx->scal.p + S_M0, M_p, nullptr, nullptr, nullptr, nullptr, nullptr, nullptr, dpos, cx->scal.p + S_M1);
    }
    check_region_err(cx, sc[S_ERR]);
    const uint32_t M = sc[S_M0];
    if (M == 0) throw Np2Error(NP2_E_REFPANIC, "reference would panic: empty consensus");
    if (M > M_cap) throw Np2Error(NP2_E_DEVICE, "internal: consensus longer than its bound");
    r.len = M;
    cx->last_first_pos = sc[S_M1];
    cx->last_last_pos = sc[S_M2];
    cx->last_dbase = dbase;
    cx->last_dpos = dpos;
    cx->last_len = M;
    if (cx->stage_timing) cx->timing.host.push_back({"wall_fetch_result", (float)(now_ms() - t0)});
}

struct PolishRun {
    np2_ctx *cx = nullptr;
    np2_contig *c = nullptr;
    np2_opts_t o{};
    uint32_t own_lo = 0, own_hi = 0xFFFFFFFFu;
    uint32_t T = 0, pass = 0, M = 0, n_reg = 0;
    bool reuse = false;
    bool front_issued = false;
    uint32_t grow_prev = 0xFFFFFFFFu;
    bool wide_votes = false;
    uint64_t key_add = 0;
    PassCounts pc;
    bool final_pass() const { return pass + 1 == o.iter_count; }
};

void run_begin(PolishRun &r) {
    np2_ctx *cx = r.cx;
    if (r.o.iter_count < 1) throw Np2Error(NP2_E_ARG, "iter_count must be >= 1");
    HIPCHK(hipSetDevice(cx->device));
    cx->trace_items.clear();
    cx->last_dbase = nullptr;
    cx->last_dpos = nullptr;
    cx->scal.ensure(SCAL_TOTAL);
    cx->alive.ensure(r.c->R + 2);
    {
        WallTimer w(cx, "wall_diff");
        run_diff(cx, r.c, r.T);
    }
    launch_init_alive(cx->stream, r.c->reads.p, r.c->R, cx->alive.p);
    r.pass = 0;
    r.reuse = false;
}

void run_pass_front(PolishRun &r) {
    np2_ctx *cx = r.cx;
    np2_contig *c = r.c;
    if (!r.reuse) {
        {
            WallTimer w(cx, "wall_cns_lq");
            if (!r.front_issued) pass_front_issue(cx, c, r.T, (int)r.pass);
            r.front_issued = false;
            consensus_and_regions_finish(cx, c, r.T, (int)r.pass, r.M, r.n_reg, !r.wide_votes);
        }
        if (cx->trace) {
            trace_cns(cx, (int)r.pass, "cns_raw", fetch_cns(cx, r.M));
            trace_put(cx, (int)r.pass, "lq.start", d2h(cx, cx->lq_start.p, r.n_reg));
            trace_put(cx, (int)r.pass, "lq.end", d2h(cx, cx->lq_end.p, r.n_reg));
        }
    }
    if (r.n_reg == 0) return;
    if (!r.reuse) {
        r.pc = PassCounts();
        r.pc.M = r.M;
        WallTimer w(cx, "wall_extract");
        extract_candidates(cx, c, r.n_reg, r.o.min_kmer_count, (int)r.pass, r.pc);
    } else if (r.pc.NC_cap) {
        op_copy_d2d(cx, cx->kscore.p, cx->kscore_saved.p, (size_t)(r.pc.known ? r.pc.NC : r.pc.NC_cap) * 2);
    }
}

void run_vote_pass(PolishRun &r, VoteData &vd, const std::function<void()> *after_front = nullptr) {
    np2_ctx *cx = r.cx;
    vd = VoteData();
    vd.R = r.c->R;
    run_pass_front(r);
    if (after_front) (*after_front)();
    if (r.n_reg == 0) return;
    WallTimer w(cx, "wall_vote");
    const bool may_reuse = cx->reuse_identical_pass && !cx->trace;
    if (may_reuse && r.pc.NC_cap) {
        cx->kscore_saved.ensure((size_t)r.pc.NC_cap + 2);
        op_copy_d2d(cx, cx->kscore_saved.p, cx->kscore.p, (size_t)(r.pc.known ? r.pc.NC : r.pc.NC_cap) * 2);
    }
    vote_collect(cx, r.c, r.pc, r.o.model_ref != 0, r.o.use_all_reads != 0, (int)r.pass, r.own_lo, r.own_hi, vd, r.wide_votes, r.key_add);
    if (r.pc.known) r.grow_prev = r.pc.grow;
}

void run_apply_losers(PolishRun &r, const std::vector<uint32_t> &losers) {
    np2_ctx *cx = r.cx;
    if (r.n_reg) trace_put(cx, (int)r.pass, "invalid_ids", losers);
    for (uint32_t id : losers) REFPANIC_IF(id >= r.c->R, "index out of bounds: alignseqs[id]");
    const bool may_reuse = cx->reuse_identical_pass && !cx->trace;
// ... 1180 lines not shown
```

### nextpolish2_amd/csrc/np2_kernels.hip

```cpp
#include "np2_common.hpp"
#include "np2_kernels.hpp"
#include "np2_blockscan.hpp"
#include "np2_nib128.hpp"
#include "../../include/np2.h"

namespace np2 {

__device__ __forceinline__ uint8_t ref_code(const uint8_t *__restrict__ refnib, uint32_t p) {
    return (refnib[p >> 1] >> (4 * (p & 1))) & 7;
}

__device__ __forceinline__ void k_encode_ref(const uint32_t np2_bid, const uint32_t np2_nb, const uint8_t *__restrict__ read0, uint32_t L, uint8_t *__restrict__ refnib,
                             uint32_t nbytes_total, uint32_t stride, uint32_t *__restrict__ err) {
    uint32_t i = np2_bid * blockDim.x + threadIdx.x;
    if (i >= nbytes_total) return;
    uint32_t c0 = 2 * i, c1 = 2 * i + 1;
    uint8_t b = c0 < L ? read0[i] : 0;
    uint8_t hi = c0 < L ? (b >> 4) : 0, lo = c1 < L ? (b & 15) : 0;
    if ((c0 < L && c0 != 0 && (hi & 8)) || (c1 < L && (lo & 8))) atomicOr(err, 1u);
    if (c0 < L && (hi & 7) == 7) atomicOr(err, 1u);
    if (c1 < L && (lo & 7) == 7) atomicOr(err, 1u);
    refnib[i] = (uint8_t)((hi & 7) | ((lo & 7) << 4));
    const uint8_t nx = c1 + 1 < L ? (uint8_t)((read0[i + 1] >> 4) & 7) : (uint8_t)0;
    refnib[stride + i] = (uint8_t)(((hi & 7) << 4) | (lo & 7));
    refnib[2 * (size_t)stride + i] = (uint8_t)(((lo & 7) << 4) | nx);
}

__device__ __forceinline__ void k_post(const uint32_t np2_bid, const uint32_t np2_nb, uint32_t *__restrict__ scal, uint32_t n_scal, uint32_t *__restrict__ mbox, uint32_t seq,
                       uint32_t *__restrict__ dst0, const uint32_t *__restrict__ src0, uint32_t *__restrict__ dst1,
                       const uint32_t *__restrict__ src1, uint32_t *__restrict__ dst2, const uint32_t *__restrict__ src2,
                       uint32_t *__restrict__ dst3, const uint32_t *__restrict__ src3,
                       const uint32_t *__restrict__ ends_of, uint32_t *__restrict__ ends_dst) {
    if (threadIdx.x == 0) {
        if (dst0) *dst0 = *src0;
        if (dst1) *dst1 = *src1;
        if (dst2) *dst2 = *src2;
        if (dst3) *dst3 = *src3;
        if (ends_of) {
            const uint32_t n = *dst0;
            ends_dst[0] = n ? ends_of[0] : 0u;
            ends_dst[1] = n ? ends_of[n - 1] : 0u;
        }
    }
    __threadfence();
    if (threadIdx.x < n_scal)
        mbox[1 + threadIdx.x] = __hip_atomic_load(&scal[threadIdx.x], __ATOMIC_RELAXED, __HIP_MEMORY_SCOPE_AGENT);
    __threadfence_system();
    if (threadIdx.x == 0) __hip_atomic_store(&mbox[0], seq, __ATOMIC_RELEASE, __HIP_MEMORY_SCOPE_SYSTEM);
}
__device__ __forceinline__ void k_fill(const uint32_t np2_bid, const uint32_t np2_nb, uint8_t *__restrict__ p, uint64_t n, uint32_t v4) {
    const uint64_t o = ((uint64_t)np2_bid * 256 + threadIdx.x) * 16;
    if (o >= n) return;
    if ((((uintptr_t)p) & 15) == 0 && o + 16 <= n) {
        *reinterpret_cast<uint4 *>(p + o) = make_uint4(v4, v4, v4, v4);
    } else {
        for (uint64_t i = o; i < min(o + 16, n); ++i) p[i] = (uint8_t)v4;
    }
}
__device__ __forceinline__ void k_copy(const uint32_t np2_bid, const uint32_t np2_nb, uint8_t *__restrict__ dst, const uint8_t *__restrict__ src, uint64_t n) {
    const uint64_t o = ((uint64_t)np2_bid * 256 + threadIdx.x) * 16;
    if (o >= n) return;
    const uintptr_t al = ((uintptr_t)dst) | ((uintptr_t)src);
    if ((al & 15) == 0 && o + 16 <= n) {
        *reinterpret_cast<uint4 *>(dst + o) = *reinterpret_cast<const uint4 *>(src + o);
    } else if ((al & 3) == 0 && o + 16 <= n) {
#pragma unroll
        for (uint32_t q = 0; q < 4; ++q)
            *reinterpret_cast<uint32_t *>(dst + o + 4 * q) = *reinterpret_cast<const uint32_t *>(src + o + 4 * q);
    } else {
        for (uint64_t i = o; i < min(o + 16, n); ++i) dst[i] = src[i];
    }
}
__device__ __forceinline__ void k_copy_len(const uint32_t np2_bid, const uint32_t np2_nb, uint8_t *__restrict__ dst, const uint8_t *__restrict__ src,
                                           const uint32_t *__restrict__ n_dev, uint32_t elem, uint64_t cap) {
    k_copy(np2_bid, np2_nb, dst, src, min((uint64_t)*n_dev * elem, cap));
}
__device__ __forceinline__ void k_copy_counted(const uint32_t np2_bid, const uint32_t np2_nb, uint32_t *__restrict__ dst, const uint32_t *__restrict__ src,
                                               const uint32_t *__restrict__ n_dev, uint32_t cap) {
    const uint32_t n = min(*n_dev, cap);
    const bool wide = ((((uintptr_t)dst) | ((uintptr_t)src)) & 15) == 0;
    for (uint64_t o = ((uint64_t)np2_bid * 256 + threadIdx.x) * 4; o < n; o += (uint64_t)np2_nb * 256 * 4) {
        if (wide && o + 4 <= n) {
            *reinterpret_cast<uint4 *>(dst + o) = *reinterpret_cast<const uint4 *>(src + o);
        } else {
            for (uint64_t i = o; i < min(o + 4, (uint64_t)n); ++i) dst[i] = src[i];
        }
    }
}
__device__ __forceinline__ void k_init_alive(const uint32_t np2_bid, const uint32_t np2_nb, const np2_read_t *__restrict__ reads, uint32_t R, uint8_t *__restrict__ alive) {
    uint32_t r = np2_bid * blockDim.x + threadIdx.x;
    if (r < R) alive[r] = (reads[r].flags & NP2_READ_DROPPED) ? 0 : 1;
}
__device__ __forceinline__ void k_kill_flagged(const uint32_t np2_bid, const uint32_t np2_nb, const uint8_t *__restrict__ flag, uint32_t n, uint8_t *__restrict__ alive) {
    uint32_t i = np2_bid * blockDim.x + threadIdx.x;
    if (i < n && flag[i]) alive[i] = 0;
}
__device__ __forceinline__ void k_kill_reads(const uint32_t np2_bid, const uint32_t np2_nb, const uint32_t *__restrict__ ids, uint32_t n, uint8_t *__restrict__ alive) {
    uint32_t i = np2_bid * blockDim.x + threadIdx.x;
    if (i < n) alive[ids[i]] = 0;
}
__device__ __forceinline__ void k_revive_reads(const uint32_t np2_bid, const uint32_t np2_nb, const uint32_t *__restrict__ ids, uint32_t n, uint8_t *__restrict__ alive) {
    uint32_t i = np2_bid * blockDim.x + threadIdx.x;
    if (i < n) alive[ids[i]] = 1;
}

struct Graph {
    const uint8_t *refnib;
    const uint32_t *node_off;
    NodeArrays nd;
    const int32_t *cov;
    uint32_t L;
    const uint2 *nrec;
    const uint32_t *deep;
};
__device__ __forceinline__ void n0_key(const Graph &g, uint32_t p, uint16_t &bases, uint16_t &delta) {
    const uint8_t c = ref_code(g.refnib, p);
    if (p >= 2) {
        bases = (uint16_t)((ref_code(g.refnib, p - 2) << 8) | (ref_code(g.refnib, p - 1) << 4) | c);
        delta = 0;
    } else if (p == 1) {
        bases = (uint16_t)(0x0F00 | (ref_code(g.refnib, 0) << 4) | c);
        delta = 1;
    } else {
        bases = (uint16_t)(0x4FF0 | c);
        delta = 0;
    }
}
__device__ __forceinline__ uint32_t n0_count(const Graph &g, uint32_t p) {
    uint32_t e0 = 0;
    for (uint32_t i = g.node_off[p]; i < g.node_off[p + 1]; ++i)
    {
        const uint2 rc = g.nrec[i];
        if (node_delta3((uint16_t)rc.x, (uint16_t)(rc.x >> 16)) == 0) e0 += rc.y;
    }
    return (uint32_t)g.cov[p] - e0;
}

__device__ __forceinline__ int64_t early_run_base(const Graph &g, uint32_t a) {
    if (a != 1 && a != 2) return 0;
    int64_t s = 10 * (int64_t)(int32_t)n0_count(g, 0) - 4 * (int64_t)g.cov[0];
    if (a == 2) s += 6 * (int64_t)g.cov[1];
    return s;
}

static constexpr uint32_t RW_P = 13;
static constexpr uint32_t RW_N = 8;
struct __attribute__((packed, aligned(4))) U32x4 {
    uint32_t x, y, z, w;
};
struct __attribute__((packed, aligned(4))) U32x2 {
    uint32_t x, y;
};
__device__ __forceinline__ uint32_t short_run_len(const uint32_t (&off)[RW_P + 1], uint32_t a, uint32_t L) {
    const uint32_t lim = min(RW_P, L - a);
    uint32_t len = RW_P;
#pragma unroll
// ... 854 lines not shown
        }
        lq_kind[p] = kind;
        lq_next[p] = pp;
        if (kind == LQK_LINK) lq_nothead[pp] = 1;
    }
}

__device__ __forceinline__ void k_lq_region(const uint32_t np2_bid, const uint32_t np2_nb, const uint32_t *__restrict__ cns_pos, const uint8_t *__restrict__ cns_base,
                            const uint32_t *__restrict__ M_p, const uint32_t *__restrict__ lq_list,
                            const uint32_t *__restrict__ n_lq_p, uint32_t lq_cap,
                            const uint8_t *__restrict__ lq_kind, const uint32_t *__restrict__ lq_next,
                            const uint8_t *__restrict__ lq_nothead, uint32_t *__restrict__ hbits,
                            uint32_t *__restrict__ rstart, uint32_t *__restrict__ rend) {
    const uint32_t M = *M_p, n_lq = min(*n_lq_p, lq_cap);
    for (uint32_t j = np2_bid * blockDim.x + threadIdx.x; j < n_lq; j += np2_nb * blockDim.x) {
        const uint32_t p = M - 1 - lq_list[j];
        if (lq_nothead[p]) continue;
        uint32_t q = p;
        while (lq_kind[q] == LQK_LINK) q = lq_next[q];
        if (lq_kind[q] != LQK_CLOSE) continue;
        const uint32_t pe = lq_next[q];
        const uint32_t lq_e = pe - 2;
        uint32_t lq_s = p > 2 ? p - 2 : 1;
#define CP(x) cns_pos[M - 1 - (x)]
#define CB(x) cns_base[M - 1 - (x)]
        for (;;) {
            const uint32_t i = M - 1 - lq_s;
            if (lq_s <= 1) break;
            if (lq_s >= 9 && i + 8 < M) {
                uint32_t ps[9];
                uint8_t bs[9];
                __builtin_memcpy(ps, cns_pos + i, 36);
                __builtin_memcpy(bs, cns_base + i, 9);
                uint32_t k = 0;
                while (k < 8 && (ps[k + 1] == ps[k] || bs[k + 1] == bs[k])) ++k;
                lq_s -= k;
                if (k < 8) break;
            } else {
                if (CP(lq_s - 1) == CP(lq_s) || CB(lq_s - 1) == CB(lq_s)) --lq_s; else break;
            }
        }
        rend[p] = CP(lq_s);
        rstart[p] = CP(lq_e);
#undef CP
#undef CB
        atomicOr(&hbits[p >> 5], 1u << (p & 31));
    }
}
__device__ __forceinline__ void k_lq_bits_count(const uint32_t np2_bid, const uint32_t np2_nb, const uint32_t *__restrict__ hbits, uint32_t n_words,
                                uint32_t *__restrict__ wcnt) {
    const uint32_t w = np2_bid * blockDim.x + threadIdx.x;
    if (w <= n_words) wcnt[w] = w < n_words ? (uint32_t)__builtin_popcount(hbits[w]) : 0u;
}
__device__ __forceinline__ void k_scatter_regions(const uint32_t np2_bid, const uint32_t np2_nb, const uint32_t *__restrict__ hbits, uint32_t n_words,
                                  const uint32_t *__restrict__ woff, const uint32_t *__restrict__ rstart,
                                  const uint32_t *__restrict__ rend, uint32_t *__restrict__ raw_start,
                                  uint32_t *__restrict__ raw_end, uint32_t *__restrict__ n_raw) {
    const uint32_t w = np2_bid * blockDim.x + threadIdx.x;
    if (w == 0) *n_raw = woff[n_words];
    if (w >= n_words) return;
    uint32_t bits = hbits[w], k = woff[w];
    for (; bits; bits &= bits - 1, ++k) {
        const uint32_t p = (w << 5) + (uint32_t)__builtin_ctz(bits);
        raw_start[k] = rstart[p];
        raw_end[k] = rend[p];
    }
}

__device__ __forceinline__ void k_lq_merge_flag(const uint32_t np2_bid, const uint32_t np2_nb, const uint32_t *__restrict__ raw_start, const uint32_t *__restrict__ raw_end,
                                const uint32_t *__restrict__ n_raw, uint32_t *__restrict__ headflag) {
    const uint32_t n = *n_raw;
    for (uint32_t j = np2_bid * blockDim.x + threadIdx.x; j < n; j += np2_nb * blockDim.x)
        headflag[j] = !(j >= 1 && raw_end[j] >= raw_start[j - 1]);
}
__device__ __forceinline__ void k_lq_merge_scan(const uint32_t np2_bid, const uint32_t np2_nb, const uint32_t *__restrict__ raw_start, const uint32_t *__restrict__ raw_end,
                                                const uint32_t *__restrict__ n_raw, uint32_t n_host, uint32_t *__restrict__ headflag,
                                                uint32_t *__restrict__ hidx) {
    __shared__ uint32_t sh[16];
    const uint32_t n = min(*n_raw, n_host);
    block_scan_array<OpAdd>(
        n, sh, [&](uint32_t j) { return (j >= 1 && raw_end[j] >= raw_start[j - 1]) ? 0u : 1u; },
        [&](uint32_t j, uint32_t pre, uint32_t v) {
            hidx[j] = pre;
            headflag[j] = v;
        });
}
__device__ __forceinline__ void k_lq_merge_write(const uint32_t np2_bid, const uint32_t np2_nb, const uint32_t *__restrict__ raw_start, const uint32_t *__restrict__ raw_end,
                                 const uint32_t *__restrict__ n_raw, const uint32_t *__restrict__ headflag,
                                 const uint32_t *__restrict__ hidx, uint32_t *__restrict__ lq_start,
                                 uint32_t *__restrict__ lq_end, uint32_t *__restrict__ n_reg) {
    const uint32_t n = *n_raw;
    for (uint32_t j = np2_bid * blockDim.x + threadIdx.x; j < n; j += np2_nb * blockDim.x) {
        if (headflag[j]) {
            uint32_t l = j;
            while (l + 1 < n && !headflag[l + 1]) ++l;
            lq_end[hidx[j]] = raw_end[j];
            lq_start[hidx[j]] = raw_start[l];
        }
        if (j == n - 1) *n_reg = hidx[j] + headflag[j];
    }
}

__device__ __forceinline__ uint32_t count_ge_desc(const uint32_t *a, uint32_t n, uint32_t v) {
    uint32_t lo = 0, hi = n;
    while (lo < hi) {
        uint32_t mid = (lo + hi) >> 1;
        if (a[mid] >= v) lo = mid + 1; else hi = mid;
    }
    return lo;
}
__device__ __forceinline__ uint32_t count_gt_desc(const uint32_t *a, uint32_t n, uint32_t v) {
    uint32_t lo = 0, hi = n;
    while (lo < hi) {
        uint32_t mid = (lo + hi) >> 1;
        if (a[mid] > v) lo = mid + 1; else hi = mid;
    }
    return lo;
}

__device__ __forceinline__ void k_read_m(const uint32_t np2_bid, const uint32_t np2_nb, const np2_read_t *__restrict__ reads, uint32_t R, const uint8_t *__restrict__ alive,
                         const uint32_t *__restrict__ lq_start, uint32_t n_reg, int32_t *__restrict__ mval) {
    uint32_t r = np2_bid * blockDim.x + threadIdx.x;
    if (r >= R) return;
    if (!alive[r]) {
        mval[r] = 0x7FFFFFFF;
        return;
    }
    const uint32_t c = count_ge_desc(lq_start, n_reg, reads[r].aln_t_s);
    mval[r] = c ? (int32_t)(c - 1) : 0;
}

__device__ __forceinline__ void k_pair_count(const uint32_t np2_bid, const uint32_t np2_nb, const np2_read_t *__restrict__ reads, uint32_t R, const uint8_t *__restrict__ alive,
                             const uint32_t *__restrict__ lq_start, const uint32_t *__restrict__ lq_end,
                             uint32_t n_reg, const int32_t *__restrict__ smin, uint32_t *__restrict__ pj,
                             uint32_t *__restrict__ pcount, const uint64_t *__restrict__ ck_off,
                             ReadInfo *__restrict__ rinfo) {
    uint32_t r = np2_bid * blockDim.x + threadIdx.x;
    if (r >= R) return;
    uint32_t cnt = 0, j = 0;
    const np2_read_t rd = reads[r];
    if (alive[r]) {
        const uint32_t s = min((uint32_t)smin[r], n_reg - 1);
        const uint32_t ts = rd.aln_t_s, te = rd.aln_t_e;
        if (!(lq_start[s] < ts || lq_end[s] > te)) {
            j = count_gt_desc(lq_end, n_reg, te);
            cnt = s - j + 1;
        }
    }
    pj[r] = j;
    pcount[r] = cnt;
    rinfo[r] = ReadInfo{rd.aln_t_s, rd.n_cols, (uint32_t)(rd.nib_off >> 4), (uint32_t)ck_off[r], rd.aln_t_e, j, cnt, 0u};
}

static constexpr uint64_t YAK_EMPTY = ~0ULL;

__global__ void k_yak_insert(const uint64_t *__restrict__ words, const uint64_t *__restrict__ bucket_off,
                             uint32_t n_buckets, uint64_t *__restrict__ table, uint32_t cap_log2,
                             uint32_t *__restrict__ dup_flag, uint32_t gap) {
    const uint32_t b = blockIdx.y;
    if (b >= n_buckets) return;
    const uint64_t n = bucket_off[b + 1] - bucket_off[b] - gap;
    const uint64_t capm = (1ULL << cap_log2) - 1;
    uint64_t *tb = table + ((uint64_t)b << cap_log2);
    for (uint64_t i = (uint64_t)blockIdx.x * blockDim.x + threadIdx.x; i < n; i += (uint64_t)gridDim.x * blockDim.x) {
        const uint64_t w = words[bucket_off[b] + i];
        const uint64_t key = w >> 10;
        uint64_t s = key & capm;
        for (;;) {
            const unsigned long long old = atomicCAS((unsigned long long *)&tb[s], (unsigned long long)YAK_EMPTY,
                                                     (unsigned long long)w);
            if (old == YAK_EMPTY) break;
            if ((old >> 10) == key) {
                atomicOr(dup_flag, 1u);
                break;
            }
            s = (s + 1) & capm;
        }
    }
}

__global__ void k_yak_insert_dup(const uint64_t *__restrict__ words, const uint64_t *__restrict__ bucket_off,
                                 uint32_t n_buckets, uint64_t *__restrict__ table, uint32_t cap_log2,
                                 uint32_t *__restrict__ ord, uint32_t gap) {
    const uint32_t b = blockIdx.y;
    if (b >= n_buckets) return;
    const uint64_t n = bucket_off[b + 1] - bucket_off[b] - gap;
    const uint64_t capm = (1ULL << cap_log2) - 1;
    uint64_t *tb = table + ((uint64_t)b << cap_log2);
    uint32_t *ob = ord + ((uint64_t)b << cap_log2);
    for (uint64_t i = (uint64_t)blockIdx.x * blockDim.x + threadIdx.x; i < n; i += (uint64_t)gridDim.x * blockDim.x) {
        const uint64_t w = words[bucket_off[b] + i];
        uint64_t s = (w >> 10) & capm;
        while (atomicCAS((unsigned long long *)&tb[s], (unsigned long long)YAK_EMPTY, (unsigned long long)w) != YAK_EMPTY)
            s = (s + 1) & capm;
        ob[s] = (uint32_t)i;
    }
}

__device__ __forceinline__ uint16_t yak_get(const YakDev &y, uint64_t x, uint16_t min_count) {
    const uint64_t capm = (1ULL << y.cap_log2) - 1;
    const uint64_t *tb = y.table + ((x & 1023) << y.cap_log2);
    const uint64_t key = x >> 10;
    uint64_t s = key & capm;
    if (y.ord) {
        const uint32_t *ob = y.ord + ((x & 1023) << y.cap_log2);
        uint16_t c = 0;
        int64_t at = -1;
        for (;;) {
            const uint64_t w = tb[s];
            if (w == YAK_EMPTY) return c;
            if ((w >> 10) == key && (uint16_t)(w & 1023) >= min_count && (int64_t)ob[s] > at) at = ob[s], c = (uint16_t)(w & 1023);
            s = (s + 1) & capm;
        }
    }
    for (;;) {
        const uint64_t w = tb[s];
        if (w == YAK_EMPTY) return 0;
        if ((w >> 10) == key) {
            const uint16_t c = (uint16_t)(w & 1023);
            return c >= min_count ? c : 0;
        }
        s = (s + 1) & capm;
    }
}

__device__ __forceinline__ void k_lookup(const uint32_t np2_bid, const uint32_t np2_nb, YakDev y, const uint64_t *__restrict__ hashes, uint64_t n, uint16_t min_count,
                         uint16_t *__restrict__ out) {
    uint64_t i = (uint64_t)np2_bid * blockDim.x + threadIdx.x;
    if (i < n) out[i] = yak_get(y, hashes[i], min_count);
}

__device__ __forceinline__ uint16_t wave_score_string_any(const YakDev &y, const uint8_t *__restrict__ s, uint32_t len,
                                                          uint16_t min_count) {
    const uint32_t lane = threadIdx.x & 63;
    const uint32_t k = y.k;
    const uint64_t mask = (1ULL << (2 * (uint64_t)k)) - 1, shift = 2 * ((uint64_t)k - 1);
    uint32_t mn = 0xFFFFFFFFu;
    if (len >= k) {
        for (uint32_t st = lane; st + k <= len; st += 64) {
            uint64_t fw = 0, rv = 0;
            bool ok = true;
            for (uint32_t j = 0; j < k; ++j) {
                const uint64_t c = ascii_to_code(s[st + j]);
                if (c >= 4) {
                    ok = false;
                    break;
                }
                fw = ((fw << 2) | c) & mask;
                rv = (rv >> 2) | ((3ULL ^ c) << shift);
            }
            if (ok) mn = min(mn, (uint32_t)yak_get(y, yak_hash64(fw < rv ? fw : rv, mask), min_count));
        }
    }
    for (int o = 32; o > 0; o >>= 1) mn = min(mn, (uint32_t)__shfl_xor(mn, o));
    return mn == 0xFFFFFFFFu ? (uint16_t)0 : (uint16_t)mn;
}
__device__ __forceinline__ uint16_t wave_score_string(const YakDev &y, const uint8_t *__restrict__ s, uint32_t len,
                                                      uint16_t min_count) {
    const uint32_t lane = threadIdx.x & 63;
    const uint32_t k = y.k;
    const uint64_t mask = (1ULL << (2 * (uint64_t)k)) - 1;
    uint32_t mn = 0xFFFFFFFFu;
    if (len >= k) {
        for (uint32_t st = lane; st + k <= len; st += 64) {
            uint64_t codes = 0, bad = 0;
#pragma unroll
            for (uint32_t wd = 0; wd < 4; ++wd) {
                uint64_t x;
                __builtin_memcpy(&x, s + st + 8 * wd, 8);
                uint64_t c = ((x >> 1) ^ (x >> 2)) & 0x0303030303030303ULL;
                c = (c | (c >> 6)) & 0x000F000F000F000FULL;
                c = (c | (c >> 12)) & 0x000000FF000000FFULL;
                c = (c | (c >> 24)) & 0xFFFFULL;
                codes |= c << (16 * wd);
                uint64_t b = (x >> 3) & 0x0101010101010101ULL;
                b = (b | (b >> 7)) & 0x0003000300030003ULL;
                b = (b | (b >> 14)) & 0x0000000F0000000FULL;
                b = (b | (b >> 28)) & 0xFFULL;
                bad |= b << (8 * wd);
            }
            if ((bad & ((1ULL << k) - 1ULL)) == 0) {
                codes &= mask;
                uint64_t rb = __builtin_bitreverse64(codes);
                rb = ((rb >> 1) & 0x5555555555555555ULL) | ((rb & 0x5555555555555555ULL) << 1);
                const uint64_t fw = rb >> (64 - 2 * k), rv = ~codes & mask;
                mn = min(mn, (uint32_t)yak_get(y, yak_hash64(fw < rv ? fw : rv, mask), min_count));
            }
        }
    }
    for (int o = 32; o > 0; o >>= 1) mn = min(mn, (uint32_t)__shfl_xor(mn, o));
    return mn == 0xFFFFFFFFu ? (uint16_t)0 : (uint16_t)mn;
}

__device__ __forceinline__ void k_score_strings(const uint32_t np2_bid, const uint32_t np2_nb, YakDev y, const uint8_t *__restrict__ strs, const uint64_t *__restrict__ off,
                                uint64_t n, uint16_t min_count, uint16_t *__restrict__ out, uint32_t own_strings) {
    const uint64_t w = ((uint64_t)np2_bid * (blockDim.x >> 6)) + (uint32_t)__builtin_amdgcn_readfirstlane((int)(threadIdx.x >> 6));
    if (w >= n) return;
    const uint16_t sc = own_strings ? wave_score_string(y, strs + off[w], (uint32_t)(off[w + 1] - off[w]), min_count)
                                    : wave_score_string_any(y, strs + off[w], (uint32_t)(off[w + 1] - off[w]), min_count);
    if ((threadIdx.x & 63) == 0) out[w] = sc;
}

__device__ __forceinline__ void k_cand_score(const uint32_t np2_bid, const uint32_t np2_nb, YakDev y, const uint32_t *__restrict__ cand_seq_off, const uint64_t *__restrict__ cand_kmer,
                             const uint32_t *__restrict__ n_cand_p, uint16_t min_count,
                             uint16_t *__restrict__ kscore, uint32_t *__restrict__ long_list,
                             uint32_t *__restrict__ n_long) {
    const uint32_t c = np2_bid * blockDim.x + threadIdx.x;
    const bool live = c < *n_cand_p;
    const uint32_t len = live ? cand_seq_off[c + 1] - cand_seq_off[c] : 0u;
    const bool is_long = live && len > y.k;
    const uint64_t m = __ballot(is_long);
    if (m) {
        const uint32_t lane = threadIdx.x & 63, lead = (uint32_t)__builtin_ctzll(m);
        uint32_t base = 0;
        if (lane == lead) base = atomicAdd(n_long, (uint32_t)__builtin_popcountll(m));
        base = __shfl(base, lead);
        if (is_long) long_list[base + (uint32_t)__builtin_popcountll(m & ((1ULL << lane) - 1ULL))] = c;
    }
    if (!live) return;
    uint16_t sc = 0;
    if (!is_long) {
        const uint64_t km = cand_kmer[c];
        if (km != INVALID_KMER) sc = yak_get(y, km, min_count);
    }
    kscore[c] = sc;
}
__device__ __forceinline__ void k_cand_score_long(const uint32_t np2_bid, const uint32_t np2_nb, YakDev y, const uint32_t *__restrict__ cand_seq_off,
                                  const uint8_t *__restrict__ cand_seq, const uint32_t *__restrict__ long_list,
                                  const uint32_t *__restrict__ n_long, uint16_t min_count,
                                  uint16_t *__restrict__ kscore) {
    const uint32_t nl = *n_long;
    for (uint32_t w = (uint32_t)__builtin_amdgcn_readfirstlane((int)((np2_bid * blockDim.x + threadIdx.x) >> 6)); w < nl; w += (np2_nb * blockDim.x) >> 6) {
        const uint32_t c = long_list[w];
        const uint16_t sc = wave_score_string(y, cand_seq + cand_seq_off[c], cand_seq_off[c + 1] - cand_seq_off[c],
                                              min_count);
        if ((threadIdx.x & 63) == 0) kscore[c] = sc;
    }
}

}

namespace np2 {
static inline dim3 grid1(uint64_t n, uint32_t bs = 256) { return dim3((unsigned)((n + bs - 1) / bs)); }

void launch_encode_ref(hipStream_t s, const uint8_t *read0, uint32_t L, uint8_t *refnib, uint32_t nbytes,
                       uint32_t stride, uint32_t *err) {
    NP2_LAUNCH(k_encode_ref, grid1(nbytes), 256, s, read0, L, refnib, nbytes, stride, err);
}
void launch_post(hipStream_t s, uint32_t *scal, uint32_t n_scal, uint32_t *mbox, uint32_t seq, uint32_t *d0,
                 const uint32_t *s0, uint32_t *d1, const uint32_t *s1, uint32_t *d2, const uint32_t *s2, uint32_t *d3,
                 const uint32_t *s3, const uint32_t *ends_of, uint32_t *ends_dst) {
    NP2_LAUNCH(k_post, dim3(1), 64, s, scal, n_scal, mbox, seq, d0, s0, d1, s1, d2, s2, d3, s3, ends_of, ends_dst);
}
void launch_fill(hipStream_t s, uint8_t *p, uint64_t bytes, uint8_t byte) {
    if (bytes) NP2_LAUNCH(k_fill, grid1((bytes + 15) / 16), 256, s, p, bytes, 0x01010101u * byte);
}
void launch_copy(hipStream_t s, uint8_t *dst, const uint8_t *src, uint64_t bytes) {
    if (bytes) NP2_LAUNCH(k_copy, grid1((bytes + 15) / 16), 256, s, dst, src, bytes);
}
void launch_copy_len(hipStream_t s, uint8_t *dst, const uint8_t *src, const uint32_t *n_dev, uint32_t elem, uint64_t cap_bytes) {
    if (cap_bytes) NP2_LAUNCH(k_copy_len, grid1((cap_bytes + 15) / 16), 256, s, dst, src, n_dev, elem, cap_bytes);
}
void launch_copy_counted(hipStream_t s, uint32_t *dst, const uint32_t *src, const uint32_t *n_dev, uint32_t cap) {
    if (cap) NP2_LAUNCH(k_copy_counted, dim3(std::max<uint32_t>(1, std::min<uint32_t>((cap + 1023) / 1024, 2048))), 256, s, dst, src, n_dev, cap);
}
void launch_init_alive(hipStream_t s, const np2_read_t *reads, uint32_t R, uint8_t *alive) {
    NP2_LAUNCH(k_init_alive, grid1(R), 256, s, reads, R, alive);
}
void launch_kill_flagged(hipStream_t s, const uint8_t *flag, uint32_t n, uint8_t *alive) {
    if (n) NP2_LAUNCH(k_kill_flagged, grid1(n), 256, s, flag, n, alive);
}
void launch_kill_reads(hipStream_t s, const uint32_t *ids, uint32_t n, uint8_t *alive) {
    if (n) NP2_LAUNCH(k_kill_reads, grid1(n), 256, s, ids, n, alive);
}
void launch_revive_reads(hipStream_t s, const uint32_t *ids, uint32_t n, uint8_t *alive) {
    if (n) NP2_LAUNCH(k_revive_reads, grid1(n), 256, s, ids, n, alive);
}
static Graph mk_graph(const GraphPtrs &gp) { return Graph{gp.refnib, gp.node_off, gp.nd, gp.cov, gp.L, gp.nrec, gp.deep}; }

void launch_dp_short(hipStream_t s, const GraphPtrs &gp, const void *refw, const uint32_t *run_start,
                     const uint32_t *n_runs, uint32_t max_runs, uint32_t *run_end, int64_t *run_gain, uint32_t *emit,
                     uint32_t *path_begin, uint64_t *path, uint32_t *dp_list, uint32_t *n_dp_list) {
    if (max_runs)
        NP2_LAUNCH(k_dp_bt_short, dim3(std::min<uint32_t>((max_runs + 63) / 64, DP_GRID_CAP)), 64, s, run_start, n_runs, mk_graph(gp), (const uint32_t *)refw, run_end, run_gain, emit, path_begin, path, dp_list, n_dp_list);
}
void launch_dp_long(hipStream_t s, const GraphPtrs &gp, const uint32_t *run_start, uint32_t max_runs, const uint2 *nrec,
                    int64_t *nscore, uint32_t *nbesti, uint32_t *n0_besti, uint32_t *run_end, int64_t *last_n0_score,
                    int64_t *run_gain, uint32_t *emit, uint32_t *path_begin, uint64_t *path, uint8_t *run_flag,
                    const uint32_t *dp_list, const uint32_t *n_dp_list) {
    if (!max_runs) return;
    NP2_LAUNCH(k_dp_bt_oct, dim3(std::min<uint32_t>((max_runs + 7) / 8, 2048u)), 64, s, run_start, mk_graph(gp), nrec, nscore, nbesti, n0_besti, run_end, last_n0_score, run_gain, emit, path_begin, path, run_flag, dp_list, n_dp_list);
    NP2_LAUNCH(k_dp_bt_long, dim3(std::min<uint32_t>((max_runs + DP_BLOCK - 1) / DP_BLOCK, 512u)), DP_BLOCK, s, run_start, mk_graph(gp), nrec, nscore, nbesti, n0_besti, run_end, last_n0_score, run_gain, emit, path_begin, path, run_flag, dp_list, n_dp_list);
}
void launch_dp_finish(hipStream_t s, const GraphPtrs &gp, const uint32_t *run_start, const uint32_t *n_runs,
                      const int64_t *nscore, const uint32_t *nbesti, const uint32_t *n0_besti, const int64_t *last_n0_score,
                      unsigned long long *total_gain, uint32_t *blocks_done, uint32_t *best_idx, const int64_t *run_gain,
                      const long long *tile_gain, uint32_t n_tiles, uint32_t *emit, uint32_t *path_begin, uint64_t *path) {
    NP2_LAUNCH(k_dp_finish, dim3(64), 256, s, run_gain, n_runs, tile_gain, n_tiles, total_gain, blocks_done, mk_graph(gp), nscore, last_n0_score, run_start, nbesti, n0_besti, best_idx, emit, path_begin, path);
}
static inline dim3 run_grid(uint32_t bound) { return dim3(std::max<uint32_t>(1, std::min<uint32_t>((bound + 256) / 256, 4096))); }
void launch_bt_write(hipStream_t s, const GraphPtrs &gp, const uint32_t *run_start, const uint32_t *n_runs,
                     uint32_t run_bound, const uint32_t *emit, const uint32_t *eoff, const uint64_t *path,
                     uint32_t *cns_pos, uint8_t *cns_base, uint8_t *cns_cls, uint8_t *lq_nothead, uint32_t *lqc) {
    NP2_LAUNCH(k_cns_write, grid1(gp.L), 256, s, gp.refnib, gp.pflag, emit, eoff, gp.L, cns_pos, cns_base, cns_cls, lq_nothead);
    NP2_LAUNCH(k_cns_runs, run_grid(4 * (uint64_t)run_bound > 0xFFFFFFF0ull ? 0xFFFFFFF0u : 4 * run_bound), 256, s, run_start, n_runs, run_bound, gp.node_off, emit, eoff, path, cns_pos, cns_base, cns_cls, lq_nothead, lqc);
}
void launch_lq_list(hipStream_t s, const GraphPtrs &gp, const uint32_t *run_start, const uint32_t *n_runs,
                    uint32_t run_bound, const uint32_t *emit, const uint32_t *eoff, const uint64_t *path,
                    const uint32_t *lqoff, uint32_t cap, uint32_t *lq_list, uint32_t *err) {
    NP2_LAUNCH(k_lq_list, run_grid(run_bound), 256, s, run_start, n_runs, run_bound, gp.node_off, emit, eoff, path, lqoff, cap, lq_list, err);
}
void launch_default_tail(hipStream_t s, const GraphPtrs &gp, const uint32_t *best_idx, const uint32_t *M_p, uint8_t *cns_base,
                         uint8_t *cns_cls, uint32_t *lq_list, uint32_t *n_lq, uint32_t cap, uint32_t *err) {
    NP2_LAUNCH(k_default_tail, 1, 64, s, best_idx, gp.node_off, gp.pflag, gp.L, M_p, cns_base, cns_cls, lq_list, n_lq, cap, err);
}
static inline dim3 lq_grid(uint32_t cap) { return dim3(std::max<uint32_t>(1, std::min<uint32_t>((cap + 2047) / 2048, 2048))); }
void launch_lq_scan(hipStream_t s, const uint32_t *cns_pos, const uint8_t *cns_base, const uint8_t *cns_cls,
                    const uint32_t *M_p, const uint32_t *lq_list, const uint32_t *n_lq, uint32_t lq_cap, uint8_t *lq_kind,
                    uint32_t *lq_next, uint8_t *lq_nothead, uint32_t *hbits, uint32_t n_hwords, uint32_t *rstart, uint32_t *rend) {
    NP2_LAUNCH(k_lq_scan, lq_grid(std::max(lq_cap, n_hwords / 4)), 256, s, cns_pos, cns_base, cns_cls, M_p, lq_list, n_lq, lq_cap, lq_kind, lq_next, lq_nothead, hbits, n_hwords);
    NP2_LAUNCH(k_lq_region, lq_grid(lq_cap), 256, s, cns_pos, cns_base, M_p, lq_list, n_lq, lq_cap, lq_kind, lq_next, lq_nothead, hbits, rstart, rend);
}
void launch_lq_bits_count(hipStream_t s, const uint32_t *hbits, uint32_t n_words, uint32_t *wcnt) {
    NP2_LAUNCH(k_lq_bits_count, grid1((uint64_t)n_words + 1), 256, s, hbits, n_words, wcnt);
}
void launch_scatter_regions(hipStream_t s, const uint32_t *hbits, uint32_t n_words, const uint32_t *woff,
                            const uint32_t *rstart, const uint32_t *rend, uint32_t *raw_start, uint32_t *raw_end,
                            uint32_t *n_raw) {
    NP2_LAUNCH(k_scatter_regions, grid1(std::max<uint32_t>(n_words, 1)), 256, s, hbits, n_words, woff, rstart, rend, raw_start, raw_end, n_raw);
}
void launch_lq_merge_flag(hipStream_t s, const uint32_t *raw_start, const uint32_t *raw_end, const uint32_t *n_raw,
                          uint32_t *headflag) {
    NP2_LAUNCH(k_lq_merge_flag, dim3(256), 256, s, raw_start, raw_end, n_raw, headflag);
}
void launch_lq_merge_scan(hipStream_t s, const uint32_t *raw_start, const uint32_t *raw_end, const uint32_t *n_raw, uint32_t n_host,
                          uint32_t *headflag, uint32_t *hidx) {
    NP2_LAUNCH(k_lq_merge_scan, dim3(1), 1024, s, raw_start, raw_end, n_raw, n_host, headflag, hidx);
}
void launch_lq_merge_write(hipStream_t s, const uint32_t *raw_start, const uint32_t *raw_end, const uint32_t *n_raw,
                           const uint32_t *headflag, const uint32_t *hidx, uint32_t *lq_start, uint32_t *lq_end,
                           uint32_t *n_reg) {
    NP2_LAUNCH(k_lq_merge_write, dim3(256), 256, s, raw_start, raw_end, n_raw, headflag, hidx, lq_start, lq_end, n_reg);
}
void launch_read_m(hipStream_t s, const np2_read_t *reads, uint32_t R, const uint8_t *alive, const uint32_t *lq_start,
                   uint32_t n_reg, int32_t *mval) {
    NP2_LAUNCH(k_read_m, grid1(R), 256, s, reads, R, alive, lq_start, n_reg, mval);
}
void launch_pair_count(hipStream_t s, const np2_read_t *reads, uint32_t R, const uint8_t *alive,
                       const uint32_t *lq_start, const uint32_t *lq_end, uint32_t n_reg, const int32_t *smin,
                       uint32_t *pj, uint32_t *pcount, const uint64_t *ck_off, ReadInfo *rinfo) {
    NP2_LAUNCH(k_pair_count, grid1(R), 256, s, reads, R, alive, lq_start, lq_end, n_reg, smin, pj, pcount, ck_off, rinfo);
}
void launch_yak_insert(hipStream_t s, const uint64_t *words, const uint64_t *bucket_off, uint32_t n_buckets,
                       uint64_t max_bucket, uint64_t *table, uint32_t cap_log2, uint32_t *dup_flag, uint32_t gap) {
    uint32_t gx = (uint32_t)((max_bucket + 255) / 256);
    if (gx == 0) gx = 1;
    if (gx > 64) gx = 64;
    hipLaunchKernelGGL(k_yak_insert, dim3(gx, n_buckets), dim3(256), 0, s, words, bucket_off, n_buckets, table,
                       cap_log2, dup_flag, gap);
}
void launch_yak_insert_dup(hipStream_t s, const uint64_t *words, const uint64_t *bucket_off, uint32_t n_buckets,
                           uint64_t max_bucket, uint64_t *table, uint32_t cap_log2, uint32_t *ord, uint32_t gap) {
    uint32_t gx = (uint32_t)((max_bucket + 255) / 256);
    gx = std::min<uint32_t>(64, std::max<uint32_t>(1, gx));
    hipLaunchKernelGGL(k_yak_insert_dup, dim3(gx, n_buckets), dim3(256), 0, s, words, bucket_off, n_buckets, table,
                       cap_log2, ord, gap);
}
void launch_lookup(hipStream_t s, const YakDev &y, const uint64_t *hashes, uint64_t n, uint16_t min_count,
                   uint16_t *out) {
    if (n) NP2_LAUNCH(k_lookup, grid1(n), 256, s, y, hashes, n, min_count, out);
}
void launch_score_strings(hipStream_t s, const YakDev &y, const uint8_t *strs, const uint64_t *off, uint64_t n,
                          uint16_t min_count, uint16_t *out, bool own_strings) {
    if (n) NP2_LAUNCH(k_score_strings, grid1(n * 64), 256, s, y, strs, off, n, min_count, out, own_strings ? 1u : 0u);
}
void launch_cand_score(hipStream_t s, const YakDev &y, const uint32_t *cand_seq_off, const uint8_t *cand_seq,
                       const uint64_t *cand_kmer, const uint32_t *n_cand_p, uint32_t cand_cap, uint16_t min_count,
                       uint16_t *kscore, uint32_t *long_list, uint32_t *n_long) {
    if (!cand_cap) return;
    NP2_LAUNCH(k_cand_score, grid1(cand_cap), 256, s, y, cand_seq_off, cand_kmer, n_cand_p, min_count, kscore, long_list, n_long);
    NP2_LAUNCH(k_cand_score_long, dim3(std::max<uint32_t>(16, std::min<uint32_t>(1024, cand_cap / 4096))), 256, s, y, cand_seq_off, cand_seq, long_list, n_long, min_count, kscore);
}
}
```

### nextpolish2_amd/csrc/np2_kernels.hpp

```cpp
#pragma once
#include <cstddef>
#include <cstdint>
#include <hip/hip_runtime.h>
#include "../../include/np2.h"
#include "np2_lookback.hpp"
#include "np2_launch.hpp"

namespace np2 {

static constexpr uint32_t TILE_SHIFT = 10;
static constexpr uint32_t TILE = 1u << TILE_SHIFT;
static constexpr uint32_t TILE_CAP = 4096;

static constexpr uint32_t DENSE_COLS = 4096;
struct ChunkDesc {
    uint64_t nib_off;
    uint64_t ckbase;
    uint32_t read, ts;
    uint32_t c0, ncols;
    uint32_t first_chunk;
    uint32_t aln_t_e, nck;
    uint32_t pad0;
    uint32_t pad[4];
};

struct NodeArrays {
    uint32_t *pos;
    uint16_t *bases;
    uint16_t *delta;
    uint32_t *count;
    uint32_t *minr;
};
struct GraphPtrs {
    const uint8_t *refnib;
    const uint32_t *node_off;
    NodeArrays nd;
    const int32_t *cov;
    uint32_t L;
    const uint2 *nrec;
    const uint32_t *deep;
    const uint8_t *pflag;
};
struct __attribute__((aligned(16))) ReadInfo {
    uint32_t aln_t_s, n_cols;
    uint32_t nib16;
    uint32_t ck_off;
    uint32_t aln_t_e;
    uint32_t pj, pcount;
    uint32_t pad;
};
struct CandPtrs {
    const np2_read_t *reads;
    const uint8_t *nib;
    const uint64_t *ck_off;
    const uint32_t *ckpt;
    const uint32_t *lq_start;
    const uint32_t *lq_end;
    const uint32_t *pj;
    const uint32_t *pcount;
    const uint8_t *alive;
    const ReadInfo *rinfo;
    const uint32_t *tile_rd_off;
    const uint32_t *tile_rd;
    uint32_t n_tiles;
    uint32_t ksize;
    const uint64_t *rec_key;
    const uint32_t *rec_read;
    const uint32_t *tile_n;
    const uint16_t *rec_pidx;
    uint32_t bucket_cap;
    const uint32_t *refnib;
    uint32_t L;
};
struct YakDev {
    const uint64_t *table;
    uint32_t cap_log2;
    uint32_t k;
    const uint32_t *ord;
};

void launch_encode_ref(hipStream_t s, const uint8_t *read0, uint32_t L, uint8_t *refnib, uint32_t nbytes, uint32_t stride, uint32_t *err);
void launch_chunk_counts(hipStream_t s, const ChunkDesc *descs, uint32_t n_chunks, const uint8_t *nib, uint64_t *chunk_st, uint32_t epoch);
void launch_diff_reads(hipStream_t s, const ChunkDesc *descs, uint32_t n_chunks, const uint8_t *nib, const uint64_t *refw,
                       const uint8_t *refnib, const uint8_t *refeo, uint32_t eo_stride, uint32_t L, uint64_t *keys, uint32_t *vals, uint32_t *tile_cur,
                       uint32_t n_tiles, uint32_t bucket_cap, uint64_t ovf_base, uint32_t ovf_cap, uint32_t *ovf_cnt,
                       uint32_t *ckpt, uint64_t *chunk_st, uint32_t epoch, uint32_t *err);
void launch_post(hipStream_t s, uint32_t *scal, uint32_t n_scal, uint32_t *mbox, uint32_t seq, uint32_t *d0 = nullptr,
                 const uint32_t *s0 = nullptr, uint32_t *d1 = nullptr, const uint32_t *s1 = nullptr, uint32_t *d2 = nullptr,
                 const uint32_t *s2 = nullptr, uint32_t *d3 = nullptr, const uint32_t *s3 = nullptr,
                 const uint32_t *ends_of = nullptr, uint32_t *ends_dst = nullptr);
void launch_fill(hipStream_t s, uint8_t *p, uint64_t bytes, uint8_t byte);
void launch_copy(hipStream_t s, uint8_t *dst, const uint8_t *src, uint64_t bytes);
void launch_copy_len(hipStream_t s, uint8_t *dst, const uint8_t *src, const uint32_t *n_dev, uint32_t elem, uint64_t cap_bytes);
void launch_copy_counted(hipStream_t s, uint32_t *dst, const uint32_t *src, const uint32_t *n_dev, uint32_t cap);
void launch_init_alive(hipStream_t s, const np2_read_t *reads, uint32_t R, uint8_t *alive);
void launch_kill_reads(hipStream_t s, const uint32_t *ids, uint32_t n, uint8_t *alive);
void launch_revive_reads(hipStream_t s, const uint32_t *ids, uint32_t n, uint8_t *alive);
void launch_kill_flagged(hipStream_t s, const uint8_t *flag, uint32_t n, uint8_t *alive);
void launch_dp_short(hipStream_t s, const GraphPtrs &gp, const void *refw, const uint32_t *run_start,
                     const uint32_t *n_runs, uint32_t max_runs, uint32_t *run_end, int64_t *run_gain, uint32_t *emit,
                     uint32_t *path_begin, uint64_t *path, uint32_t *dp_list, uint32_t *n_dp_list);
void launch_dp_long(hipStream_t s, const GraphPtrs &gp, const uint32_t *run_start, uint32_t max_runs, const uint2 *nrec,
                    int64_t *nscore, uint32_t *nbesti, uint32_t *n0_besti, uint32_t *run_end, int64_t *last_n0_score,
                    int64_t *run_gain, uint32_t *emit, uint32_t *path_begin, uint64_t *path, uint8_t *run_flag,
                    const uint32_t *dp_list, const uint32_t *n_dp_list);
void launch_dp_finish(hipStream_t s, const GraphPtrs &gp, const uint32_t *run_start, const uint32_t *n_runs,
                      const int64_t *nscore, const uint32_t *nbesti, const uint32_t *n0_besti, const int64_t *last_n0_score,
                      unsigned long long *total_gain, uint32_t *blocks_done, uint32_t *best_idx, const int64_t *run_gain,
                      const long long *tile_gain, uint32_t n_tiles, uint32_t *emit, uint32_t *path_begin, uint64_t *path);
void launch_bt_write(hipStream_t s, const GraphPtrs &gp, const uint32_t *run_start, const uint32_t *n_runs,
                     uint32_t run_bound, const uint32_t *emit, const uint32_t *eoff, const uint64_t *path,
                     uint32_t *cns_pos, uint8_t *cns_base, uint8_t *cns_cls, uint8_t *lq_nothead, uint32_t *lqc);
void launch_lq_list(hipStream_t s, const GraphPtrs &gp, const uint32_t *run_start, const uint32_t *n_runs,
                    uint32_t run_bound, const uint32_t *emit, const uint32_t *eoff, const uint64_t *path,
                    const uint32_t *lqoff, uint32_t cap, uint32_t *lq_list, uint32_t *err);
void launch_default_tail(hipStream_t s, const GraphPtrs &gp, const uint32_t *best_idx, const uint32_t *M_p, uint8_t *cns_base,
                         uint8_t *cns_cls, uint32_t *lq_list, uint32_t *n_lq, uint32_t cap, uint32_t *err);
void launch_lq_scan(hipStream_t s, const uint32_t *cns_pos, const uint8_t *cns_base, const uint8_t *cns_cls,
                    const uint32_t *M_p, const uint32_t *lq_list, const uint32_t *n_lq, uint32_t lq_cap, uint8_t *lq_kind,
                    uint32_t *lq_next, uint8_t *lq_nothead, uint32_t *hbits, uint32_t n_hwords, uint32_t *rstart, uint32_t *rend);
void launch_lq_merge_scan_lb(hipStream_t s, const Lookback &lb, const uint32_t *raw_start, const uint32_t *raw_end, const uint32_t *n_raw,
                             uint32_t n_host, uint32_t *headflag, uint32_t *hidx, uint32_t *err);
uint32_t lq_merge_lb_blocks();
void launch_lq_merge_scan(hipStream_t s, const uint32_t *raw_start, const uint32_t *raw_end, const uint32_t *n_raw, uint32_t n_host,
                          uint32_t *headflag, uint32_t *hidx);
void launch_scan_lb_popc(hipStream_t s, const Lookback &lb, const uint32_t *bits, uint32_t *out, uint32_t n_words, uint32_t *err);
void launch_lq_bits_count(hipStream_t s, const uint32_t *hbits, uint32_t n_words, uint32_t *wcnt);
void launch_scatter_regions(hipStream_t s, const uint32_t *hbits, uint32_t n_words, const uint32_t *woff,
                            const uint32_t *rstart, const uint32_t *rend, uint32_t *raw_start, uint32_t *raw_end,
                            uint32_t *n_raw);
void launch_lq_merge_flag(hipStream_t s, const uint32_t *raw_start, const uint32_t *raw_end, const uint32_t *n_raw,
                          uint32_t *headflag);
void launch_lq_merge_write(hipStream_t s, const uint32_t *raw_start, const uint32_t *raw_end, const uint32_t *n_raw,
                           const uint32_t *headflag, const uint32_t *hidx, uint32_t *lq_start, uint32_t *lq_end,
                           uint32_t *n_reg);
void launch_read_m(hipStream_t s, const np2_read_t *reads, uint32_t R, const uint8_t *alive, const uint32_t *lq_start,
                   uint32_t n_reg, int32_t *mval);
void launch_yak_insert(hipStream_t s, const uint64_t *words, const uint64_t *bucket_off, uint32_t n_buckets,
                       uint64_t max_bucket, uint64_t *table, uint32_t cap_log2, uint32_t *dup_flag, uint32_t gap = 0);
void launch_yak_insert_dup(hipStream_t s, const uint64_t *words, const uint64_t *bucket_off, uint32_t n_buckets,
                           uint64_t max_bucket, uint64_t *table, uint32_t cap_log2, uint32_t *ord, uint32_t gap = 0);
void launch_lookup(hipStream_t s, const YakDev &y, const uint64_t *hashes, uint64_t n, uint16_t min_count, uint16_t *out);
void launch_score_strings(hipStream_t s, const YakDev &y, const uint8_t *strs, const uint64_t *off, uint64_t n,
                          uint16_t min_count, uint16_t *out, bool own_strings);
void launch_cand_score(hipStream_t s, const YakDev &y, const uint32_t *cand_seq_off, const uint8_t *cand_seq,
                       const uint64_t *cand_kmer, const uint32_t *n_cand_p, uint32_t cand_cap, uint16_t min_count,
                       uint16_t *kscore, uint32_t *long_list, uint32_t *n_long);


void launch_pair_count(hipStream_t s, const np2_read_t *reads, uint32_t R, const uint8_t *alive,
                       const uint32_t *lq_start, const uint32_t *lq_end, uint32_t n_reg, const int32_t *smin,
                       uint32_t *pj, uint32_t *pcount, const uint64_t *ck_off, ReadInfo *rinfo);
void launch_scan_lb_excl(hipStream_t s, const Lookback &lb, const uint32_t *in, uint32_t *out, uint32_t n, bool write_end,
                          uint32_t *err);
uint32_t scan_lb_blocks(uint64_t n);
void launch_scan_small_excl(hipStream_t s, const uint32_t *in, uint32_t *out, uint32_t n, const uint32_t *n_dev,
                            uint32_t *total_out, bool write_end);
void launch_scan_small_incl(hipStream_t s, const int32_t *in, int32_t *out, uint32_t n, const uint32_t *n_dev);
void launch_scan_small_min(hipStream_t s, const int32_t *in, int32_t *out, uint32_t n, const uint32_t *n_dev);
void launch_region_measure(hipStream_t s, const CandPtrs &c, uint32_t n_reg, uint32_t *kept_read, uint32_t *kept_len,
                           uint32_t *kept_col, uint32_t *reg_ncand, uint32_t *reg_bytes, uint32_t *reg_maxlen,
                           uint32_t *blk_sum);
uint32_t cand_offsets_blocks(uint32_t n_reg);
void launch_cand_offsets(hipStream_t s, const uint32_t *blk_sum, uint32_t n_reg, uint32_t *blk_coff, uint32_t *blk_soff,
                         uint32_t *cand_off, uint32_t *reg_soff, uint32_t *n_cand, uint32_t *n_bytes, uint32_t *grow,
                         const Lookback *lb = nullptr, uint32_t *err = nullptr);
void launch_region_write(hipStream_t s, const CandPtrs &c, uint32_t n_reg, const uint32_t *kept_read,
                         const uint32_t *kept_len, const uint32_t *kept_col, const uint32_t *reg_ncand,
                         const uint32_t *reg_bytes, const uint32_t *blk_coff, const uint32_t *blk_soff, uint32_t *cand_off,
                         uint32_t *reg_soff, uint32_t cand_cap, uint32_t seq_cap, uint32_t *cand_order, uint64_t *cand_kmer,
                         uint32_t *cand_seq_off, uint8_t *cand_seq);

uint32_t tile_scan_blocks(uint32_t n_tiles);
void launch_tile_layout(hipStream_t s, uint32_t *tile_cur, uint32_t n_tiles, uint32_t bucket_cap, uint32_t *tile_n,
                        uint32_t *tile_scan, uint32_t *tile_scanb, const uint32_t *ovf_cnt, uint32_t *out,
                        const Lookback *lb = nullptr, uint32_t *err = nullptr);
void launch_tile_sort(hipStream_t s, uint16_t *pidx, const np2_read_t *reads, const uint8_t *nib, const uint32_t *tile_n,
                      uint32_t n_tiles, uint32_t bucket_cap, uint32_t max_tile, uint64_t *keys, uint32_t *vals,
                      uint32_t *err);
void launch_gather_buckets(hipStream_t s, const np2_read_t *reads, const uint8_t *nib, const uint32_t *tile_n,
                           const uint32_t *tile_scanb, uint32_t n_tiles, uint32_t bucket_cap, const uint64_t *bkeys,
                           const uint32_t *bvals, uint64_t *keys, uint32_t *vals);
void launch_gather_spill(hipStream_t s, const np2_read_t *reads, const uint8_t *nib, const uint64_t *okeys,
                         const uint32_t *ovals, uint32_t n, uint64_t *keys, uint32_t *vals);
void launch_tile_count(hipStream_t s, const uint64_t *keys, const uint32_t *vals, const uint32_t *tile_n,
                       const uint32_t *tile_scan, uint32_t bucket_cap, uint32_t n_tiles, const uint8_t *alive,
                       uint32_t *tile_nn, uint32_t *tile_nr);
void launch_tile_offsets(hipStream_t s, const uint32_t *tile_nn, const uint32_t *tile_nr, uint32_t n_tiles,
                         uint32_t *tile_noff, uint32_t *tile_roff, uint32_t *n_nodes, uint32_t *n_runs, uint32_t *reset,
                         uint32_t n_reset, const Lookback *lb = nullptr, uint32_t *err = nullptr,
                         const long long *tile_gain = nullptr, unsigned long long *gain_total = nullptr);
void launch_tile_write(hipStream_t s, const uint64_t *keys, const uint32_t *vals, const uint32_t *tile_n,
                       const uint32_t *tile_scan, uint32_t bucket_cap, const uint32_t *tile_noff, const uint32_t *tile_roff,
                       uint32_t n_tiles, const uint8_t *alive, uint32_t L, NodeArrays nd, uint2 *nrec, uint32_t *node_off,
                       uint32_t *run_start, const np2_read_t *reads, const uint32_t *tile_rd_off, const uint32_t *tile_rd,
                       int32_t *cov, const uint8_t *refnib, uint32_t *emit, long long *tile_gain, uint32_t *deep_flag, uint32_t deep_min,
                       uint8_t *pflag);

static constexpr uint32_t PF_CAP = 960;
static constexpr uint32_t PF_HALO = 64;
static constexpr uint32_t PF_CAP_MID = 2048;
static constexpr uint32_t PF_CAP_BIG = 3584;
static constexpr uint32_t PF_COV_MAX = 8192;
static constexpr uint32_t PF_REDO = 1u;
static constexpr uint32_t PF_NEED_BIG = 2u;
struct PfTile {
    const uint64_t *keys;
    const uint32_t *vals;
    const uint32_t *tile_n, *tile_scan;
    const uint16_t *pidx;
    const uint8_t *alive;
    const np2_read_t *reads;
    const uint32_t *tile_rd_off, *tile_rd;
    const uint8_t *refnib;
    uint16_t *slots;
    uint32_t *tile_cnt, *tile_lq;
    long long *tile_gain;
    uint32_t *flags, *n_bad, *bad_list, *n_bad2, *bad_list2;
    long long *end_rel;
    unsigned long long *gain_total;
    unsigned long long *prof;
    uint32_t L, n_tiles, bucket_cap;
    uint32_t cap_lim, cap_lim_big, halo_lim, cov_max;
    uint32_t big_enabled;
};
uint64_t pf_slot_entries(uint32_t n_tiles, uint64_t T);
void launch_pf_tile(hipStream_t s, const PfTile &a);
void launch_pf_compact(hipStream_t s, uint32_t n_tiles, const uint16_t *slots, const uint32_t *tile_scan, const uint32_t *tile_cnt,
                       const uint32_t *tile_coff, const uint32_t *tile_lqoff, uint32_t *cns_pos, uint8_t *cns_base,
                       uint8_t *cns_cls, uint8_t *lq_nothead, uint32_t *lq_list, uint32_t lq_cap, uint32_t *err, uint32_t *flags,
                       uint32_t *flags_out, uint32_t *n_bad, uint32_t *n_bad2);

struct RegionTables {
    const uint32_t *cand_off;
    const uint32_t *order;
    uint16_t *kscore;
    const uint32_t *seq_off;
    const uint8_t *seq;
    uint32_t n_reg;
};
struct RechPtrs {
    const void *groups;
    const uint32_t *job_off;
    const uint32_t *rech;
    const uint32_t *cand_off;
    const uint32_t *keep_list;
    const uint32_t *seq_off;
    const uint8_t *seq;
    const uint8_t *cns_base;
    uint32_t n_groups;
};
void launch_vote_phase(hipStream_t s, const RegionTables &rt, bool asref, bool use_all, const uint32_t *lq_start,
                       uint32_t own_lo, uint32_t own_hi, uint8_t *reg_lable, uint8_t *grp, uint32_t *ecount, int32_t *ref_w,
                       uint8_t *ref_seen, uint8_t *bad, uint32_t *first_reg, uint32_t *err);
void launch_vote_counts(hipStream_t s, const uint32_t *first_reg, const uint8_t *bad, uint32_t R, uint32_t *out);
void launch_edges_write(hipStream_t s, const RegionTables &rt, const uint8_t *reg_lable, const uint8_t *grp,
                        const uint32_t *ecount, const uint32_t *eoff, uint64_t *ekey, uint32_t *eval);
static constexpr uint32_t EDGE_BAND = 256;
void launch_edges_row(hipStream_t s, const RegionTables &rt, const uint8_t *grp, const uint32_t *ecount, const uint32_t *pj,
                      const uint32_t *pcount, const uint8_t *alive, uint32_t R, uint32_t *band, uint32_t *row_n, uint32_t *ovf);
void launch_band_emit(hipStream_t s, const uint32_t *band, uint32_t R, const uint32_t *row_off, uint64_t *ukey, uint32_t *uw,
                      uint32_t *n_out, uint64_t key_add = 0);
static constexpr uint32_t VOTE_CNT_MAX = 0xFFFu;
void launch_band_emit_compact(hipStream_t s, const uint32_t *band, uint32_t R, const uint32_t *row_off, uint32_t *pairs,
                              uint32_t *n_out, uint32_t *ovf);
void launch_edge_reduce(hipStream_t s, const uint64_t *ekey, const uint32_t *eval, uint32_t n, uint32_t *flag, uint32_t *wout);
void launch_edge_compact(hipStream_t s, const uint64_t *ekey, const uint32_t *flag, const uint32_t *idx, const uint32_t *wout,
                         uint32_t n, uint64_t *ukey, uint32_t *uw, uint32_t *n_out);
void launch_seed(hipStream_t s, const RegionTables &rt, int32_t max_indel_len, uint8_t *reg_lable, uint32_t *seed_cand,
                 uint32_t *keep_n, uint32_t *keep_list, uint16_t *keep_ks, uint32_t *err);
uint32_t region_lb_blocks(uint32_t n_reg);
void launch_splice_find(hipStream_t s, const uint32_t *cns_pos, const uint32_t *M_p, const uint32_t *lq_start,
                        const uint32_t *lq_end, const uint8_t *reg_lable, uint8_t lable, uint32_t n_reg, uint32_t *idx_s,
                        uint32_t *idx_e, uint32_t *stuck);
void launch_splice_plan(hipStream_t s, const Lookback &lb, const uint8_t *reg_lable, uint8_t lable, uint32_t n_reg,
                        const uint32_t *stuck, const uint32_t *idx_s, const uint32_t *idx_e, const uint32_t *seed_cand,
                        const uint32_t *seq_off, uint32_t *ap_g, uint32_t *ap_s, uint32_t *ap_e, int32_t *ap_delta,
                        int32_t *ap_shift_incl, uint32_t *n_ap, const uint32_t *M_in, uint32_t *M_out, uint32_t out_cap , uint32_t *err);
void launch_splice_write(hipStream_t s, const uint32_t *in_pos, const uint8_t *in_base, const uint32_t *M_p, uint32_t M_cap,
                         const uint32_t *ap_g, const uint32_t *ap_s, const uint32_t *ap_e, const int32_t *ap_delta,
                         const int32_t *ap_shift_incl, const uint32_t *n_ap, uint32_t max_ap, const uint32_t *lq_start,
                         const uint32_t *seed_cand, const uint32_t *seq_off, const uint8_t *seq, uint32_t *out_pos,
                         uint8_t *out_base);
void launch_shard_bounds(hipStream_t s, const uint32_t *cns_pos, const uint32_t *M_p, const uint32_t *t, uint32_t *out);
void launch_rech_list(hipStream_t s, const Lookback &lb, const uint8_t *reg_lable, uint32_t n_reg, uint32_t *rech,
                      uint32_t *n_rech, unsigned long long *blob_bound, uint32_t *err);
void launch_rech_groups(hipStream_t s, const Lookback &lb, const uint32_t *rech, const uint32_t *n_rech_p, uint32_t max_rech,
                        const uint32_t *cns_pos, const uint32_t *M_p, const uint32_t *lq_start, const uint32_t *lq_end,
                        const uint32_t *keep_n, uint32_t ksize, const uint32_t *reg_maxlen, void *tmp_groups,
                        uint32_t *head_jobs, void *groups, uint32_t *job_off, uint32_t *n_groups, uint32_t *n_jobs,
                        unsigned long long *blob_bound, uint32_t *err);
size_t rech_group_bytes();
void launch_rech_job_len(hipStream_t s, const RechPtrs &p, uint32_t n_jobs, uint32_t *len);
void launch_rech_job_build(hipStream_t s, const RechPtrs &p, uint32_t n_jobs, const uint32_t *soff32, uint64_t *soff64,
                           uint8_t *blob);
void launch_rech_apply(hipStream_t s, const RechPtrs &p, const uint16_t *score, uint16_t *keep_ks);
void launch_rech_select(hipStream_t s, const uint32_t *rech, const uint32_t *n_rech_p, uint32_t max_rech,
                        const uint32_t *cand_off, const uint32_t *keep_n, const uint32_t *keep_list, const uint16_t *keep_ks,
                        const uint32_t *order, bool first_yak, uint8_t *reg_lable, uint32_t *seed_cand);
void launch_rech_relabel(hipStream_t s, uint8_t *reg_lable, uint32_t n_reg);

struct FrontOp {
    uint32_t col0, q0, t0;
    uint32_t len_type;
};
struct FrontRec {
    uint32_t pos, n_ops;
    uint64_t op_off;
    uint64_t seq_off;
    uint64_t out_off;
    uint32_t n_cols;
    uint32_t pad;
};
struct FrontOut {
    uint32_t aln_t_s, aln_t_e, n_cols, pad;
};
void launch_columnarise(hipStream_t s, const FrontRec *recs, uint32_t n_recs, const FrontOp *ops, const uint8_t *ref,
                        const uint8_t *seq4, uint8_t *nib, FrontOut *out);
void launch_pack_ref(hipStream_t s, const uint8_t *ref, uint32_t L, uint8_t *dst);

size_t prim_temp_bytes(size_t n);
int prim_sort_pairs_u64_u32(hipStream_t s, void *tmp, size_t tmp_bytes, const uint64_t *kin, uint64_t *kout,
                            const uint32_t *vin, uint32_t *vout, size_t n, unsigned end_bit);
int prim_exclusive_sum_u32(hipStream_t s, void *tmp, size_t tmp_bytes, const uint32_t *in, uint32_t *out, size_t n);
// ... 5 lines not shown
```

Before: 4039.

## Fuse candidate k-mer scoring into region write and compact per-region records

Short-candidate k-mer scoring and long-list construction move from a separate cand_score kernel into the region write kernel. For clean candidates the k-mer hash is computed directly from reference nibbles with ballots, and the first hash-table probe is issued early. Region measure now emits a packed 32-byte per-region record with kept/clean lane masks and a combined len/col array, so region write reads fewer scattered arrays and skips per-candidate loads for clean reads. This removes a kernel launch and one pass over candidate k-mers, but region write becomes heavier and uses more LDS and registers.

Result: no change. 4005 (median of 3 runs) (-0.8%).

```diff
diff --git a/nextpolish2_amd/csrc/np2_cand.hip b/nextpolish2_amd/csrc/np2_cand.hip
--- a/nextpolish2_amd/csrc/np2_cand.hip
+++ b/nextpolish2_amd/csrc/np2_cand.hip
@@ -1,5 +1,6 @@
 #include "np2_common.hpp"
 #include "np2_kernels.hpp"
+#include "np2_yak.hpp"
 #include "np2_blockscan.hpp"
 #include "np2_lookback.hpp"
 
@@ -84,15 +85,10 @@
 }
 
 struct CandCtx {
-    const np2_read_t *reads;
     const uint8_t *nib;
-    const uint64_t *ck_off;
     const uint32_t *ckpt;
     const uint32_t *lq_start;
     const uint32_t *lq_end;
-    const uint32_t *pj;
-    const uint32_t *pcount;
-    const uint8_t *alive;
     const ReadInfo *rinfo;
     const uint32_t *tile_rd_off;
     const uint32_t *tile_rd;
@@ -209,7 +205,8 @@
     }
 };
 
-__device__ void cand_write(const CandCtx &cx, uint32_t r, const np2_read_t &rd, uint32_t pj, uint32_t g, uint32_t col, uint32_t t,
+template <class Ctx>
+__device__ void cand_write(const Ctx &cx, uint32_t r, const np2_read_t &rd, uint32_t pj, uint32_t g, uint32_t col, uint32_t t,
                            uint32_t len, uint8_t *__restrict__ seq_out, uint64_t *kmer_out) {
     const uint8_t *base = cx.nib + rd.nib_off;
     const uint32_t limit = cx.lq_end[pj] + cx.ksize;
@@ -374,9 +371,16 @@
     return np2_read_t{ri.aln_t_s, ri.aln_t_e, (uint64_t)ri.nib16 << 4, ri.n_cols, 0u};
 }
 
+static constexpr uint32_t REC_SLOTS = 0xFFFFFFFFu;
+__device__ __forceinline__ void rrec_put(RegionRec *p, uint32_t la, uint32_t ncand, uint32_t bytes, uint64_t kept, uint64_t clean) {
+    uint4 *q = reinterpret_cast<uint4 *>(p);
+    q[0] = make_uint4(la, ncand, bytes, 0u);
+    q[1] = make_uint4((uint32_t)kept, (uint32_t)(kept >> 32), (uint32_t)clean, (uint32_t)(clean >> 32));
+}
+
 __device__ __forceinline__ void region_measure_inline(const CandCtx &cx, uint32_t g, uint32_t st, uint32_t en, uint32_t la, uint32_t lb,
-                                                      uint32_t *__restrict__ kept_read, uint32_t *__restrict__ kept_len,
-                                                      uint32_t *__restrict__ kept_col, uint32_t &kept, uint32_t &bytes, uint32_t &mx) {
+                                                      uint32_t *__restrict__ kept_read, uint2 *__restrict__ kept_lc,
+                                                      uint32_t &kept, uint32_t &bytes, uint32_t &mx) {
     const uint32_t lane = threadIdx.x & 63;
     kept = 0, bytes = 0, mx = 0;
     for (uint32_t c0 = la; c0 < lb && kept < LQSEQ_MAX_CAN_COUNT; c0 += 64) {
@@ -393,8 +397,7 @@
         if (keep) {
             const size_t slot = (size_t)g * LQSEQ_MAX_CAN_COUNT + before;
             kept_read[slot] = r;
-            kept_len[slot] = len;
-            kept_col[slot] = col;
+            kept_lc[slot] = make_uint2(len, col);
         }
         kept = min(kept + (uint32_t)__builtin_popcountll(ne), (uint32_t)LQSEQ_MAX_CAN_COUNT);
         bytes += wave_sum(keep ? len : 0u);
@@ -403,8 +406,8 @@
     for (int o = 32; o > 0; o >>= 1) mx = max(mx, (uint32_t)__shfl_xor(mx, o));
 }
 
-__device__ __forceinline__ void k_region_measure(const uint32_t np2_bid0, const uint32_t np2_nb, CandCtx cx, uint32_t n_reg, uint32_t *__restrict__ kept_read,
-                                                        uint32_t *__restrict__ kept_len, uint32_t *__restrict__ kept_col,
+__device__ __forceinline__ void k_region_measure(const uint32_t np2_bid0, const uint32_t np2_nb, CandCtx cx, uint32_t n_reg, RegionRec *__restrict__ rrec, uint32_t *__restrict__ kept_read,
+                                                        uint2 *__restrict__ kept_lc,
                                                         uint32_t *__restrict__ reg_ncand, uint32_t *__restrict__ reg_bytes,
                                                         uint32_t *__restrict__ reg_maxlen, uint32_t *__restrict__ blk_sum) {
     const uint32_t np2_bid = xcd_order(np2_bid0, np2_nb);
@@ -526,11 +529,12 @@
         if (!live[h] || ((fastmask >> h) & 1u)) continue;
         const uint32_t g = g0 + h;
         uint32_t kept, bytes, mx;
-        region_measure_inline(cx, g, st[h], en[h], la[h], lb[h], kept_read, kept_len, kept_col, kept, bytes, mx);
+        region_measure_inline(cx, g, st[h], en[h], la[h], lb[h], kept_read, kept_lc, kept, bytes, mx);
         if (lane == 0) {
             reg_ncand[g] = kept;
             reg_bytes[g] = bytes;
             reg_maxlen[g] = mx;
+            rrec_put(rrec + g, REC_SLOTS, kept, bytes, 0, 0);
         }
         sum_k[h / 4] += kept, sum_b[h / 4] += bytes, sum_m[h / 4] += mx;
     }
@@ -556,12 +560,9 @@
         const uint64_t ne = __ballot(len > 0);
         const uint32_t before = lanes_below(ne);
         const bool keep = len > 0 && before < LQSEQ_MAX_CAN_COUNT;
-        if (keep) {
-            const size_t ks = (size_t)g * LQSEQ_MAX_CAN_COUNT + before;
-            kept_read[ks] = rr[h];
-            kept_len[ks] = len;
-            kept_col[ks] = col;
-        }
+        const uint64_t km = __ballot(keep), dm = __ballot(keep && state[h] == 2u), cm = km & ~dm;
+        if (keep && state[h] == 2u)
+            kept_lc[(size_t)g * LQSEQ_MAX_CAN_COUNT + lanes_below(dm)] = make_uint2(len, col);
         const uint32_t kept = min((uint32_t)__builtin_popcountll(ne), (uint32_t)LQSEQ_MAX_CAN_COUNT);
         const uint32_t bytes = wave_sum(keep ? len : 0u);
         uint32_t mx = keep ? len : 0u;
@@ -570,6 +571,7 @@
             reg_ncand[g] = kept;
             reg_bytes[g] = bytes;
             reg_maxlen[g] = mx;
+            rrec_put(rrec + g, la[h], kept, bytes, km, cm);
         }
         sum_k[h / 4] += kept, sum_b[h / 4] += bytes, sum_m[h / 4] += mx;
     }
@@ -677,113 +679,182 @@
     }
 }
 
-__device__ __forceinline__ void k_region_write(const uint32_t np2_bid0, const uint32_t np2_nb, CandCtx cx, uint32_t n_reg, const uint32_t *__restrict__ kept_read,
-                                                      const uint32_t *__restrict__ kept_len,
-                                                      const uint32_t *__restrict__ kept_col,
-                                                      const uint32_t *__restrict__ reg_ncand,
-                                                      const uint32_t *__restrict__ reg_bytes,
-                                                      const uint32_t *__restrict__ blk_coff,
-                                                      const uint32_t *__restrict__ blk_soff,
-                                                      uint32_t *__restrict__ cand_off, uint32_t *__restrict__ reg_soff,
-                                                      uint32_t cand_cap,
-                                                      uint32_t seq_cap, uint32_t *__restrict__ cand_order,
-                                                      uint64_t *__restrict__ cand_kmer, uint32_t *__restrict__ cand_seq_off,
-                                                      uint8_t *__restrict__ cand_seq) {
+__device__ __forceinline__ void long_push(bool is_long, uint32_t c, uint32_t *__restrict__ long_list, uint32_t *__restrict__ n_long) {
+    const uint64_t m = __ballot(is_long);
+    if (m) {
+        const uint32_t lane = threadIdx.x & 63, lead = (uint32_t)__builtin_ctzll(m);
+        uint32_t base = 0;
+        if (lane == lead) base = atomicAdd(n_long, (uint32_t)__builtin_popcountll(m));
+        base = __shfl(base, lead);
+        if (is_long) long_list[base + lanes_below(m)] = c;
+    }
+}
+
+__device__ __forceinline__ uint64_t spread32(uint32_t v) {
+    uint64_t x = v;
+    x = (x | (x << 16)) & 0x0000FFFF0000FFFFULL;
+    x = (x | (x << 8)) & 0x00FF00FF00FF00FFULL;
+    x = (x | (x << 4)) & 0x0F0F0F0F0F0F0F0FULL;
+    x = (x | (x << 2)) & 0x3333333333333333ULL;
+    return (x | (x << 1)) & 0x5555555555555555ULL;
+}
+
+__device__ __forceinline__ void k_region_write(const uint32_t np2_bid0, const uint32_t np2_nb, RegionWriteCtx cx) {
     const uint32_t np2_bid = xcd_order(np2_bid0, np2_nb);
     __shared__ __attribute__((aligned(4))) uint8_t s_str[RM_REG][CLEAN_MAX_LEN];
-    __shared__ uint64_t s_km[RM_REG];
     __shared__ uint32_t s_so[RM_REG][64];
+    __shared__ uint32_t s_rd[RM_REG][64];
+    __shared__ uint32_t s_me[RM_REG][64];
     __shared__ uint32_t s_oc[RM_REG];
+    __shared__ uint32_t s_st[RM_REG];
     __shared__ uint32_t s_q[4][RM_RPW * 64];
     const uint32_t lane = threadIdx.x & 63, wv = (uint32_t)__builtin_amdgcn_readfirstlane((int)(threadIdx.x >> 6));
-    const uint32_t g0 = (np2_bid * 4 + wv) * RM_RPW, mb0 = g0 / 4;
+    const uint32_t n_reg = cx.n_reg, g0 = (np2_bid * 4 + wv) * RM_RPW, mb0 = g0 / 4, k = cx.ksize;
     uint32_t nq = 0;
     uint32_t oc = 0, ob = 0;
-    if (g0 < n_reg) oc = blk_coff[mb0], ob = blk_soff[mb0];
+    if (g0 < n_reg) oc = cx.blk_coff[mb0], ob = cx.blk_soff[mb0];
     uint32_t clean_h = 0;
-    uint32_t my_len[RM_RPW], my_so[RM_RPW], my_ci[RM_RPW];
-    bool my_clean[RM_RPW];
-    uint32_t n[RM_RPW], rb[RM_RPW], st[RM_RPW], ln0[RM_RPW];
+    uint32_t n[RM_RPW], rb[RM_RPW], st[RM_RPW], ln0[RM_RPW], la[RM_RPW];
+    uint64_t km[RM_RPW], cm[RM_RPW];
 #pragma unroll
     for (uint32_t h = 0; h < RM_RPW; ++h) {
         const uint32_t g = g0 + h;
-        n[h] = 0, rb[h] = 0, st[h] = 0, ln0[h] = 0;
-        if (g < n_reg) n[h] = reg_ncand[g], rb[h] = reg_bytes[g], st[h] = cx.lq_start[g], ln0[h] = cx.lq_end[g] - st[h] + 1;
-    }
-    uint32_t len[RM_RPW], col[RM_RPW], rd_[RM_RPW], refc[RM_RPW];
-#pragma unroll
-    for (uint32_t h = 0; h < RM_RPW; ++h) {
-        const size_t ks = (size_t)(g0 + h) * LQSEQ_MAX_CAN_COUNT + lane;
-        const bool act = lane < n[h];
-        len[h] = act ? kept_len[ks] : 0u;
-        col[h] = act ? kept_col[ks] : 0u;
-        rd_[h] = act ? kept_read[ks] : 0u;
+        n[h] = 0, rb[h] = 0, st[h] = 0, ln0[h] = 0, la[h] = REC_SLOTS, km[h] = 0, cm[h] = 0;
+        if (g < n_reg) {
+            const uint4 a = reinterpret_cast<const uint4 *>(cx.rrec + g)[0], b = reinterpret_cast<const uint4 *>(cx.rrec + g)[1];
+            la[h] = a.x, n[h] = a.y, rb[h] = a.z;
+            km[h] = (uint64_t)b.x | ((uint64_t)b.y << 32), cm[h] = (uint64_t)b.z | ((uint64_t)b.w << 32);
+            st[h] = cx.lq_start[g], ln0[h] = cx.lq_end[g] - st[h] + 1;
+        }
+    }
+    uint32_t len[RM_RPW], rd_[RM_RPW], refc[RM_RPW], rank[RM_RPW], drank[RM_RPW];
+    bool act[RM_RPW], cl[RM_RPW];
+#pragma unroll
+    for (uint32_t h = 0; h < RM_RPW; ++h) {
+        const bool fastr = la[h] != REC_SLOTS;
+        act[h] = fastr ? ((km[h] >> lane) & 1ULL) != 0 : lane < n[h];
+        cl[h] = fastr && ((cm[h] >> lane) & 1ULL) != 0;
+        rank[h] = fastr ? lanes_below(km[h]) : lane;
+        drank[h] = fastr ? lanes_below(km[h] & ~cm[h]) : lane;
+        const size_t ks = (size_t)(g0 + h) * LQSEQ_MAX_CAN_COUNT;
+        len[h] = !act[h] ? 0u : cl[h] ? ln0[h] : cx.kept_lc[ks + drank[h]].x;
+        rd_[h] = !act[h] ? 0u : fastr ? cx.tile_rd[la[h] + lane] : cx.kept_read[ks + lane];
         const uint32_t p = st[h] + lane;
-        refc[h] = (n[h] && lane < ln0[h] && ln0[h] <= CLEAN_MAX_LEN) ? cx.refnib[p >> 3] >> (4 * (p & 7)) : 0u;
-    }
+        refc[h] = (fastr && lane < max(ln0[h], k)) ? cx.refnib[p >> 3] >> (4 * (p & 7)) : 0u;
+    }
+    uint64_t own_km = INVALID_KMER, own_w0 = 0;
+    bool own_probe = false;
+    const uint64_t kmask = (1ULL << (2 * (uint64_t)k)) - 1;
 #pragma unroll
     for (uint32_t h = 0; h < RM_RPW; ++h) {
         const uint32_t g = g0 + h, slot = wv * RM_RPW + h;
-        my_len[h] = 0, my_so[h] = 0, my_ci[h] = 0, my_clean[h] = false;
         if (g >= n_reg) continue;
-        if (g == n_reg - 1 && lane == 0 && cand_off[n_reg] < cand_cap) cand_seq_off[cand_off[n_reg]] = reg_soff[n_reg];
+        if (g == n_reg - 1 && lane == 0 && cx.cand_off[n_reg] < cx.cand_cap) cx.cand_seq_off[cx.cand_off[n_reg]] = cx.reg_soff[n_reg];
         if (lane == 0) {
-            cand_off[g] = oc;
-            reg_soff[g] = ob;
+            cx.cand_off[g] = oc;
+            cx.reg_soff[g] = ob;
             s_oc[slot] = oc;
-        }
-        const bool act = lane < n[h];
+            s_st[slot] = st[h];
+        }
         const uint32_t so = ob + wave_excl(len[h]);
-        const uint32_t ci = oc + lane;
-        const bool ok = act && ci < cand_cap && (uint64_t)so + len[h] <= seq_cap;
+        const uint32_t ci = oc + rank[h];
+        const bool ok = act[h] && ci < cx.cand_cap && (uint64_t)so + len[h] <= cx.seq_cap;
         if (ok) {
-            cand_order[ci] = rd_[h];
-            cand_seq_off[ci] = so;
-        }
-        const bool clean = ok && col[h] == CAND_CLEAN;
-        const uint64_t cm = __ballot(clean);
-        const bool queued = ok && (!clean || (lane == 0 && rd_[h] == 0));
-        my_len[h] = len[h], my_so[h] = so, my_ci[h] = ci, my_clean[h] = clean && !queued;
+            cx.cand_order[ci] = rd_[h];
+            cx.cand_seq_off[ci] = so;
+        } else if (act[h] && ci < cx.cand_cap) {
+            cx.kscore[ci] = 0;
+        }
+        const bool clean = ok && cl[h], queued = ok && !cl[h];
+        const uint64_t cmk = __ballot(clean);
         s_so[slot][lane] = so;
-        if (cm) {
+        s_rd[slot][lane] = rd_[h];
+        s_me[slot][lane] = rank[h] | (clean ? (len[h] << 8) | (1u << 16) : 0u);
+        if (cmk) {
             clean_h |= 1u << h;
             if (lane < ln0[h]) s_str[slot][lane] = (uint8_t)((0x54474341u >> (8 * (refc[h] & 3))) & 0xFFu);
+            const uint64_t codes = (spread32((uint32_t)__ballot((refc[h] & 1u) != 0)) | (spread32((uint32_t)__ballot((refc[h] & 2u) != 0)) << 1)) & kmask;
+            uint64_t rbv = __builtin_bitreverse64(codes);
+            rbv = ((rbv >> 1) & 0x5555555555555555ULL) | ((rbv & 0x5555555555555555ULL) << 1);
+            const uint64_t fw = rbv >> (64 - 2 * k), rv = ~codes & kmask;
+            const uint64_t hk = yak_hash64(fw < rv ? fw : rv, kmask);
+            if (lane == h) {
+                own_km = hk;
+                own_probe = ln0[h] <= k;
+                if (own_probe) own_w0 = yak_first(cx.yak, hk);
+            }
         }
         const uint64_t dq = __ballot(queued);
-        if (queued) s_q[wv][nq + lanes_below(dq)] = (slot << 6) | lane;
+        if (queued) s_q[wv][nq + lanes_below(dq)] = (drank[h] << 16) | (slot << 12) | (rank[h] << 6) | lane;
         nq += (uint32_t)__builtin_popcountll(dq);
         oc += n[h];
         ob += rb[h];
     }
     wave_lds_sync();
-    for (uint32_t e = lane; e < nq; e += 64) {
-        const uint32_t w = s_q[wv][e], slot = w >> 6, li = w & 63;
-        const uint32_t g = (np2_bid * 4 + slot / RM_RPW) * RM_RPW + slot % RM_RPW;
-        const size_t ks = (size_t)g * LQSEQ_MAX_CAN_COUNT + li;
-        const uint32_t r = kept_read[ks], len = kept_len[ks];
-        uint32_t col = kept_col[ks];
-        const ReadInfo ri = cx.rinfo[r];
-        const np2_read_t rd = rinfo_read(ri);
-        const uint32_t t0 = max(cx.lq_start[g], rd.aln_t_s);
-        if (col == CAND_CLEAN) col = t0;
-        const uint32_t ci = s_oc[slot] + li;
-        uint64_t km;
-        cand_write(cx, r, rd, ri.pj, g, col, t0, len, cand_seq + s_so[slot][li], &km);
-        cand_kmer[ci] = km;
-        if (li == 0 && r == 0) s_km[slot] = km;
-    }
-    wave_lds_sync();
-#pragma unroll
-    for (uint32_t h = 0; h < RM_RPW; ++h) {
+    for (uint32_t e0 = 0; e0 < nq; e0 += 64) {
+        const uint32_t e = e0 + lane;
+        bool is_long = false;
+        uint32_t ci = 0;
+        if (e < nq) {
+            const uint32_t w = s_q[wv][e], slot = (w >> 12) & 15u, rk = (w >> 6) & 63u, li = w & 63u;
+            const uint32_t g = (np2_bid * 4 + slot / RM_RPW) * RM_RPW + slot % RM_RPW;
+            const uint2 lc = cx.kept_lc[(size_t)g * LQSEQ_MAX_CAN_COUNT + (w >> 16)];
+            const uint32_t r = s_rd[slot][li], len_c = lc.x, col_c = lc.y;
+            const ReadInfo ri = cx.rinfo[r];
+            const np2_read_t rd = rinfo_read(ri);
+            const uint32_t t0 = max(s_st[slot], rd.aln_t_s);
+            ci = s_oc[slot] + rk;
+            uint64_t kmv;
+            cand_write(cx, r, rd, ri.pj, g, col_c, t0, len_c, cx.cand_seq + s_so[slot][li], &kmv);
+            if (cx.cand_kmer) cx.cand_kmer[ci] = kmv;
+            is_long = len_c > k;
+            if (!is_long) cx.kscore[ci] = kmv != INVALID_KMER ? yak_get(cx.yak, kmv, cx.min_count) : (uint16_t)0;
+        }
+        long_push(is_long, ci, cx.long_list, cx.n_long);
+    }
+    uint32_t my_ci[RM_RPW];
+    bool my_clean[RM_RPW];
+#pragma unroll
+    for (uint32_t h = 0; h < RM_RPW; ++h) {
+        my_ci[h] = 0, my_clean[h] = false;
         if (!((clean_h >> h) & 1u)) continue;
         const uint32_t slot = wv * RM_RPW + h;
+        const uint32_t me = s_me[slot][lane], my_len = (me >> 8) & 0xFFu;
+        my_clean[h] = (me >> 16) != 0;
+        my_ci[h] = s_oc[slot] + (me & 0xFFu);
         if (my_clean[h]) {
-            cand_kmer[my_ci[h]] = s_km[slot];
             typedef uint32_t u32_any __attribute__((aligned(1)));
-            uint8_t *dst = cand_seq + my_so[h];
-            const uint32_t L4 = my_len[h] & ~3u;
+            uint8_t *dst = cx.cand_seq + s_so[slot][lane];
+            const uint32_t L4 = my_len & ~3u;
             for (uint32_t j = 0; j < L4; j += 4) *reinterpret_cast<u32_any *>(dst + j) = *reinterpret_cast<const uint32_t *>(&s_str[slot][j]);
-            for (uint32_t j = L4; j < my_len[h]; ++j) dst[j] = s_str[slot][j];
+            for (uint32_t j = L4; j < my_len; ++j) dst[j] = s_str[slot][j];
+        }
+    }
+    const uint32_t own_sc = own_probe ? yak_get_after(cx.yak, own_km, cx.min_count, own_w0) : 0u;
+    uint64_t lm[RM_RPW];
+    uint32_t n_lm = 0;
+#pragma unroll
+    for (uint32_t h = 0; h < RM_RPW; ++h) {
+        lm[h] = 0;
+        if (!((clean_h >> h) & 1u)) continue;
+        const bool lg = ln0[h] > k;
+        const uint32_t sc = (uint32_t)__shfl((int)own_sc, (int)h);
+        const uint64_t kmh = ((uint64_t)(uint32_t)__shfl((int)(uint32_t)(own_km >> 32), (int)h) << 32) | (uint32_t)__shfl((int)(uint32_t)own_km, (int)h);
+        if (my_clean[h]) {
+            if (cx.cand_kmer) cx.cand_kmer[my_ci[h]] = kmh;
+            if (!lg) cx.kscore[my_ci[h]] = (uint16_t)sc;
+        }
+        lm[h] = __ballot(my_clean[h] && lg);
+        n_lm += (uint32_t)__builtin_popcountll(lm[h]);
+    }
+    if (n_lm) {
+        uint32_t base = 0;
+        if (lane == 0) base = atomicAdd(cx.n_long, n_lm);
+        base = (uint32_t)__builtin_amdgcn_readfirstlane((int)base);
+#pragma unroll
+        for (uint32_t h = 0; h < RM_RPW; ++h) {
+            if ((lm[h] >> lane) & 1ULL) cx.long_list[base + lanes_below(lm[h])] = my_ci[h];
+            base += (uint32_t)__builtin_popcountll(lm[h]);
         }
     }
 }
@@ -809,16 +880,17 @@
     NP2_LAUNCH(k_scan_small<2>, dim3(1), 1024, s, (const uint32_t *)in, (uint32_t *)out, n, n_dev, (uint32_t *)nullptr, false);
 }
 static CandCtx mk_cand(const CandPtrs &c) {
-    return CandCtx{c.reads, c.nib,    c.ck_off, c.ckpt,        c.lq_start, c.lq_end, c.pj,
-                   c.pcount, c.alive, c.rinfo, c.tile_rd_off, c.tile_rd, c.n_tiles,  c.ksize,
+    return CandCtx{c.nib, c.ckpt, c.lq_start, c.lq_end, c.rinfo, c.tile_rd_off, c.tile_rd, c.n_tiles,  c.ksize,
                    c.rec_key, c.rec_read, c.tile_n, c.rec_pidx, c.bucket_cap, c.refnib, c.L};
 }
-void launch_region_measure(hipStream_t s, const CandPtrs &c, uint32_t n_reg, uint32_t *kept_read, uint32_t *kept_len,
-                           uint32_t *kept_col, uint32_t *reg_ncand, uint32_t *reg_bytes, uint32_t *reg_maxlen,
-                           uint32_t *blk_sum) {
+static_assert(Sig<decltype(&k_region_measure)>::N >= 17 && Sig<decltype(&k_region_write)>::N >= 17,
+              "argument packs of the region kernels: a 17-contig batch must fit one launch");
+void launch_region_measure(hipStream_t s, const CandPtrs &c, uint32_t n_reg, RegionRec *rrec, uint32_t *kept_read,
+                           uint2 *kept_lc, uint32_t *reg_ncand, uint32_t *reg_bytes,
+                           uint32_t *reg_maxlen, uint32_t *blk_sum) {
     if (n_reg)
         NP2_LAUNCH_WAVES(k_region_measure, RM_WAVES, dim3((n_reg + RM_REG - 1) / RM_REG), 256, s,
-                         mk_cand(c), n_reg, kept_read, kept_len, kept_col, reg_ncand, reg_bytes, reg_maxlen, blk_sum);
+                         mk_cand(c), n_reg, rrec, kept_read, kept_lc, reg_ncand, reg_bytes, reg_maxlen, blk_sum);
 }
 uint32_t cand_offsets_blocks(uint32_t n_reg) { return ((n_reg + 3) / 4 + 1023) / 1024; }
 void launch_cand_offsets(hipStream_t s, const uint32_t *blk_sum, uint32_t n_reg, uint32_t *blk_coff, uint32_t *blk_soff,
@@ -834,13 +906,8 @@
     NP2_LAUNCH(k_lq_merge_scan_lb, dim3(MERGE_LB_BLOCKS), 1024, s, lb, raw_start, raw_end, n_raw, n_host, headflag, hidx, err);
 }
 uint32_t lq_merge_lb_blocks() { return MERGE_LB_BLOCKS; }
-void launch_region_write(hipStream_t s, const CandPtrs &c, uint32_t n_reg, const uint32_t *kept_read,
-                         const uint32_t *kept_len, const uint32_t *kept_col, const uint32_t *reg_ncand,
-                         const uint32_t *reg_bytes, const uint32_t *blk_coff, const uint32_t *blk_soff, uint32_t *cand_off,
-                         uint32_t *reg_soff, uint32_t cand_cap, uint32_t seq_cap, uint32_t *cand_order, uint64_t *cand_kmer,
-                         uint32_t *cand_seq_off, uint8_t *cand_seq) {
-    if (n_reg)
-        NP2_LAUNCH(k_region_write, dim3((n_reg + RM_REG - 1) / RM_REG), 256, s, mk_cand(c), n_reg, kept_read, kept_len, kept_col, reg_ncand, reg_bytes, blk_coff, blk_soff, cand_off, reg_soff, cand_cap, seq_cap, cand_order, cand_kmer, cand_seq_off, cand_seq);
-}
-
-}
+void launch_region_write(hipStream_t s, const RegionWriteCtx &w) {
+    if (w.n_reg) NP2_LAUNCH_WAVES(k_region_write, RM_WAVES, dim3((w.n_reg + RM_REG - 1) / RM_REG), 256, s, w);
+}
+
+}
diff --git a/nextpolish2_amd/csrc/np2_ctx.hpp b/nextpolish2_amd/csrc/np2_ctx.hpp
--- a/nextpolish2_amd/csrc/np2_ctx.hpp
+++ b/nextpolish2_amd/csrc/np2_ctx.hpp
@@ -449,8 +449,10 @@
     DevBuf<uint8_t> alive, cns_base, cns_cls, lq_kind, lq_nothead;
     DevBuf<uint32_t> cns_pos, lq_next, rflag, rstart, rend, ridx, raw_start, raw_end, headflag, hidx, lq_start,
         lq_end;
-    DevBuf<uint32_t> pj, pcount, reg_ncand, reg_bytes, reg_soff, reg_maxlen, blk_sum, blk_coff, blk_soff, kept_read, kept_len, kept_col, cand_off, cand_order, cand_seq_off, kill_ids;
+    DevBuf<uint32_t> pj, pcount, reg_ncand, reg_bytes, reg_soff, reg_maxlen, blk_sum, blk_coff, blk_soff, kept_read, cand_off, cand_order, cand_seq_off, kill_ids;
     DevBuf<uint64_t> cand_kmer;
+    DevBuf<uint2> kept_lc;
+    DevBuf<RegionRec> rrec;
     DevBuf<uint8_t> cand_seq;
     DevBuf<uint16_t> kscore;
     DevBuf<uint32_t> scal;
diff --git a/nextpolish2_amd/csrc/np2_host.cpp b/nextpolish2_amd/csrc/np2_host.cpp
--- a/nextpolish2_amd/csrc/np2_host.cpp
+++ b/nextpolish2_amd/csrc/np2_host.cpp
@@ -949,11 +949,11 @@
     cx->blk_coff.ensure((size_t)n_reg / 4 + 2);
     cx->blk_soff.ensure((size_t)n_reg / 4 + 2);
     cx->cand_off.ensure(n_reg + 2);
+    cx->rrec.ensure((size_t)n_reg + 2);
     cx->kept_read.ensure((size_t)NC_cap + 2);
-    cx->kept_len.ensure((size_t)NC_cap + 2);
-    cx->kept_col.ensure((size_t)NC_cap + 2);
+    cx->kept_lc.ensure((size_t)NC_cap + 2);
     cx->cand_order.ensure((size_t)NC_cap + 2);
-    cx->cand_kmer.ensure((size_t)NC_cap + 2);
+    if (cx->trace) cx->cand_kmer.ensure((size_t)NC_cap + 2);
     cx->cand_seq_off.ensure((size_t)NC_cap + 2);
     if (!exact_bytes) cx->cand_seq.ensure((size_t)SB_cap + 64);
     cx->kscore.ensure((size_t)NC_cap + 2);
@@ -969,7 +969,7 @@
         scan_incl_min(cx, cx->mval.p, cx->smin.p, R);
         launch_pair_count(s, c->reads.p, R, cx->alive.p, cx->lq_start.p, cx->lq_end.p, n_reg, cx->smin.p, cx->pj.p,
                           cx->pcount.p, c->ck_off.p, cx->rinfo.p);
-        launch_region_measure(s, cp, n_reg, cx->kept_read.p, cx->kept_len.p, cx->kept_col.p, cx->reg_ncand.p,
+        launch_region_measure(s, cp, n_reg, cx->rrec.p, cx->kept_read.p, cx->kept_lc.p, cx->reg_ncand.p,
                               cx->reg_bytes.p, cx->reg_maxlen.p, cx->blk_sum.p);
         {
             const bool wide = n_reg > 0;
@@ -986,14 +986,17 @@
             SB_cap = (uint32_t)std::min<uint64_t>((uint64_t)pc.SB + 64, SB_cap);
             cx->cand_seq.ensure((size_t)SB_cap + 64);
         }
-        launch_region_write(s, cp, n_reg, cx->kept_read.p, cx->kept_len.p, cx->kept_col.p, cx->reg_ncand.p,
-                            cx->reg_bytes.p, cx->blk_coff.p, cx->blk_soff.p, cx->cand_off.p, cx->reg_soff.p, NC_cap + 1,
-                            SB_cap, cx->cand_order.p, cx->cand_kmer.p, cx->cand_seq_off.p, cx->cand_seq.p);
+        const RegionWriteCtx w{c->nib.p, cx->lq_start.p, cx->lq_end.p, cx->rinfo.p, c->tile_rd.p, (const uint32_t *)c->refnib.p,
+                               cx->rrec.p, cx->kept_read.p, cx->kept_lc.p, cx->blk_coff.p, cx->blk_soff.p,
+                               cx->cand_off.p, cx->reg_soff.p, cx->cand_order.p, cx->trace ? cx->cand_kmer.p : nullptr,
+                               cx->cand_seq_off.p, cx->cand_seq.p, cx->kscore.p, cx->long_list.p, cx->scal.p + S_NLONG,
+                               cx->yaks[0].dev(), n_reg, cx->yaks[0].k, NC_cap + 1, SB_cap, min_kmer_count};
+        launch_region_write(s, w);
     }
     {
         EventTimer t(cx, "kmer_score");
-        launch_cand_score(s, cx->yaks[0].dev(), cx->cand_seq_off.p, cx->cand_seq.p, cx->cand_kmer.p, cx->scal.p + S_NC,
-                          NC_cap, min_kmer_count, cx->kscore.p, cx->long_list.p, cx->scal.p + S_NLONG);
+        launch_cand_score_long(s, cx->yaks[0].dev(), cx->cand_seq_off.p, cx->cand_seq.p, NC_cap, min_kmer_count, cx->kscore.p,
+                               cx->long_list.p, cx->scal.p + S_NLONG);
     }
     pc.n_reg = n_reg;
     pc.NC_cap = NC_cap;
diff --git a/nextpolish2_amd/csrc/np2_kernels.hip b/nextpolish2_amd/csrc/np2_kernels.hip
--- a/nextpolish2_amd/csrc/np2_kernels.hip
+++ b/nextpolish2_amd/csrc/np2_kernels.hip
@@ -2,6 +2,7 @@
 #include "np2_kernels.hpp"
 #include "np2_blockscan.hpp"
 #include "np2_nib128.hpp"
+#include "np2_yak.hpp"
 #include "../../include/np2.h"
 
 namespace np2 {
@@ -1162,7 +1163,6 @@
     rinfo[r] = ReadInfo{rd.aln_t_s, rd.n_cols, (uint32_t)(rd.nib_off >> 4), (uint32_t)ck_off[r], rd.aln_t_e, j, cnt, 0u};
 }
 
-static constexpr uint64_t YAK_EMPTY = ~0ULL;
 
 __global__ void k_yak_insert(const uint64_t *__restrict__ words, const uint64_t *__restrict__ bucket_off,
                              uint32_t n_buckets, uint64_t *__restrict__ table, uint32_t cap_log2,
@@ -1204,33 +1204,6 @@
         while (atomicCAS((unsigned long long *)&tb[s], (unsigned long long)YAK_EMPTY, (unsigned long long)w) != YAK_EMPTY)
             s = (s + 1) & capm;
         ob[s] = (uint32_t)i;
-    }
-}
-
-__device__ __forceinline__ uint16_t yak_get(const YakDev &y, uint64_t x, uint16_t min_count) {
-    const uint64_t capm = (1ULL << y.cap_log2) - 1;
-    const uint64_t *tb = y.table + ((x & 1023) << y.cap_log2);
-    const uint64_t key = x >> 10;
-    uint64_t s = key & capm;
-    if (y.ord) {
-        const uint32_t *ob = y.ord + ((x & 1023) << y.cap_log2);
-        uint16_t c = 0;
-        int64_t at = -1;
-        for (;;) {
-            const uint64_t w = tb[s];
-            if (w == YAK_EMPTY) return c;
-            if ((w >> 10) == key && (uint16_t)(w & 1023) >= min_count && (int64_t)ob[s] > at) at = ob[s], c = (uint16_t)(w & 1023);
-            s = (s + 1) & capm;
-        }
-    }
-    for (;;) {
-        const uint64_t w = tb[s];
-        if (w == YAK_EMPTY) return 0;
-        if ((w >> 10) == key) {
-            const uint16_t c = (uint16_t)(w & 1023);
-            return c >= min_count ? c : 0;
-        }
-        s = (s + 1) & capm;
     }
 }
 
@@ -1311,30 +1284,6 @@
     if ((threadIdx.x & 63) == 0) out[w] = sc;
 }
 
-__device__ __forceinline__ void k_cand_score(const uint32_t np2_bid, const uint32_t np2_nb, YakDev y, const uint32_t *__restrict__ cand_seq_off, const uint64_t *__restrict__ cand_kmer,
-                             const uint32_t *__restrict__ n_cand_p, uint16_t min_count,
-                             uint16_t *__restrict__ kscore, uint32_t *__restrict__ long_list,
-                             uint32_t *__restrict__ n_long) {
-    const uint32_t c = np2_bid * blockDim.x + threadIdx.x;
-    const bool live = c < *n_cand_p;
-    const uint32_t len = live ? cand_seq_off[c + 1] - cand_seq_off[c] : 0u;
-    const bool is_long = live && len > y.k;
-    const uint64_t m = __ballot(is_long);
-    if (m) {
-        const uint32_t lane = threadIdx.x & 63, lead = (uint32_t)__builtin_ctzll(m);
-        uint32_t base = 0;
-        if (lane == lead) base = atomicAdd(n_long, (uint32_t)__builtin_popcountll(m));
-        base = __shfl(base, lead);
-        if (is_long) long_list[base + (uint32_t)__builtin_popcountll(m & ((1ULL << lane) - 1ULL))] = c;
-    }
-    if (!live) return;
-    uint16_t sc = 0;
-    if (!is_long) {
-        const uint64_t km = cand_kmer[c];
-        if (km != INVALID_KMER) sc = yak_get(y, km, min_count);
-    }
-    kscore[c] = sc;
-}
 __device__ __forceinline__ void k_cand_score_long(const uint32_t np2_bid, const uint32_t np2_nb, YakDev y, const uint32_t *__restrict__ cand_seq_off,
                                   const uint8_t *__restrict__ cand_seq, const uint32_t *__restrict__ long_list,
                                   const uint32_t *__restrict__ n_long, uint16_t min_count,
@@ -1484,11 +1433,10 @@
                           uint16_t min_count, uint16_t *out, bool own_strings) {
     if (n) NP2_LAUNCH(k_score_strings, grid1(n * 64), 256, s, y, strs, off, n, min_count, out, own_strings ? 1u : 0u);
 }
-void launch_cand_score(hipStream_t s, const YakDev &y, const uint32_t *cand_seq_off, const uint8_t *cand_seq,
-                       const uint64_t *cand_kmer, const uint32_t *n_cand_p, uint32_t cand_cap, uint16_t min_count,
-                       uint16_t *kscore, uint32_t *long_list, uint32_t *n_long) {
+void launch_cand_score_long(hipStream_t s, const YakDev &y, const uint32_t *cand_seq_off, const uint8_t *cand_seq,
+                            uint32_t cand_cap, uint16_t min_count, uint16_t *kscore, const uint32_t *long_list,
+                            const uint32_t *n_long) {
     if (!cand_cap) return;
-    NP2_LAUNCH(k_cand_score, grid1(cand_cap), 256, s, y, cand_seq_off, cand_kmer, n_cand_p, min_count, kscore, long_list, n_long);
     NP2_LAUNCH(k_cand_score_long, dim3(std::max<uint32_t>(16, std::min<uint32_t>(1024, cand_cap / 4096))), 256, s, y, cand_seq_off, cand_seq, long_list, n_long, min_count, kscore);
 }
 }
diff --git a/nextpolish2_amd/csrc/np2_kernels.hpp b/nextpolish2_amd/csrc/np2_kernels.hpp
--- a/nextpolish2_amd/csrc/np2_kernels.hpp
+++ b/nextpolish2_amd/csrc/np2_kernels.hpp
@@ -77,6 +77,39 @@
     uint32_t cap_log2;
     uint32_t k;
     const uint32_t *ord;
+};
+struct __attribute__((aligned(16))) RegionRec {
+    uint32_t la, ncand, bytes, pad;
+    uint64_t kept, clean;
+};
+static_assert(sizeof(RegionRec) == 32, "one line per region");
+struct RegionWriteCtx {
+    const uint8_t *__restrict__ nib;
+    const uint32_t *__restrict__ lq_start;
+    const uint32_t *__restrict__ lq_end;
+    const ReadInfo *__restrict__ rinfo;
+    const uint32_t *__restrict__ tile_rd;
+    const uint32_t *__restrict__ refnib;
+    const RegionRec *__restrict__ rrec;
+    const uint32_t *__restrict__ kept_read;
+    const uint2 *__restrict__ kept_lc;
+    const uint32_t *__restrict__ blk_coff;
+    const uint32_t *__restrict__ blk_soff;
+    uint32_t *cand_off;
+    uint32_t *reg_soff;
+    uint32_t *__restrict__ cand_order;
+    uint64_t *__restrict__ cand_kmer;
+    uint32_t *__restrict__ cand_seq_off;
+    uint8_t *__restrict__ cand_seq;
+    uint16_t *__restrict__ kscore;
+    uint32_t *__restrict__ long_list;
+    uint32_t *__restrict__ n_long;
+    YakDev yak;
+    uint32_t n_reg;
+    uint32_t ksize;
+    uint32_t cand_cap;
+    uint32_t seq_cap;
+    uint16_t min_count;
 };
 
 void launch_encode_ref(hipStream_t s, const uint8_t *read0, uint32_t L, uint8_t *refnib, uint32_t nbytes, uint32_t stride, uint32_t *err);
@@ -143,9 +176,9 @@
 void launch_lookup(hipStream_t s, const YakDev &y, const uint64_t *hashes, uint64_t n, uint16_t min_count, uint16_t *out);
 void launch_score_strings(hipStream_t s, const YakDev &y, const uint8_t *strs, const uint64_t *off, uint64_t n,
                           uint16_t min_count, uint16_t *out, bool own_strings);
-void launch_cand_score(hipStream_t s, const YakDev &y, const uint32_t *cand_seq_off, const uint8_t *cand_seq,
-                       const uint64_t *cand_kmer, const uint32_t *n_cand_p, uint32_t cand_cap, uint16_t min_count,
-                       uint16_t *kscore, uint32_t *long_list, uint32_t *n_long);
+void launch_cand_score_long(hipStream_t s, const YakDev &y, const uint32_t *cand_seq_off, const uint8_t *cand_seq,
+                            uint32_t cand_cap, uint16_t min_count, uint16_t *kscore, const uint32_t *long_list,
+                            const uint32_t *n_long);
 
 
 void launch_pair_count(hipStream_t s, const np2_read_t *reads, uint32_t R, const uint8_t *alive,
@@ -158,18 +191,14 @@
                             uint32_t *total_out, bool write_end);
 void launch_scan_small_incl(hipStream_t s, const int32_t *in, int32_t *out, uint32_t n, const uint32_t *n_dev);
 void launch_scan_small_min(hipStream_t s, const int32_t *in, int32_t *out, uint32_t n, const uint32_t *n_dev);
-void launch_region_measure(hipStream_t s, const CandPtrs &c, uint32_t n_reg, uint32_t *kept_read, uint32_t *kept_len,
-                           uint32_t *kept_col, uint32_t *reg_ncand, uint32_t *reg_bytes, uint32_t *reg_maxlen,
-                           uint32_t *blk_sum);
+void launch_region_measure(hipStream_t s, const CandPtrs &c, uint32_t n_reg, RegionRec *rrec, uint32_t *kept_read,
+                           uint2 *kept_lc, uint32_t *reg_ncand, uint32_t *reg_bytes,
+                           uint32_t *reg_maxlen, uint32_t *blk_sum);
 uint32_t cand_offsets_blocks(uint32_t n_reg);
 void launch_cand_offsets(hipStream_t s, const uint32_t *blk_sum, uint32_t n_reg, uint32_t *blk_coff, uint32_t *blk_soff,
                          uint32_t *cand_off, uint32_t *reg_soff, uint32_t *n_cand, uint32_t *n_bytes, uint32_t *grow,
                          const Lookback *lb = nullptr, uint32_t *err = nullptr);
-void launch_region_write(hipStream_t s, const CandPtrs &c, uint32_t n_reg, const uint32_t *kept_read,
-                         const uint32_t *kept_len, const uint32_t *kept_col, const uint32_t *reg_ncand,
-                         const uint32_t *reg_bytes, const uint32_t *blk_coff, const uint32_t *blk_soff, uint32_t *cand_off,
-                         uint32_t *reg_soff, uint32_t cand_cap, uint32_t seq_cap, uint32_t *cand_order, uint64_t *cand_kmer,
-                         uint32_t *cand_seq_off, uint8_t *cand_seq);
+void launch_region_write(hipStream_t s, const RegionWriteCtx &w);
 
 uint32_t tile_scan_blocks(uint32_t n_tiles);
 void launch_tile_layout(hipStream_t s, uint32_t *tile_cur, uint32_t n_tiles, uint32_t bucket_cap, uint32_t *tile_n,
diff --git a/nextpolish2_amd/csrc/np2_yak.hpp b/nextpolish2_amd/csrc/np2_yak.hpp
--- /dev/null
+++ b/nextpolish2_amd/csrc/np2_yak.hpp
@@ -0,0 +1,57 @@
+#pragma once
+#include "np2_common.hpp"
+#include "np2_kernels.hpp"
+
+namespace np2 {
+
+static constexpr uint64_t YAK_EMPTY = ~0ULL;
+
+__device__ __forceinline__ uint16_t yak_get(const YakDev &y, uint64_t x, uint16_t min_count) {
+    const uint64_t capm = (1ULL << y.cap_log2) - 1;
+    const uint64_t *tb = y.table + ((x & 1023) << y.cap_log2);
+    const uint64_t key = x >> 10;
+    uint64_t s = key & capm;
+    if (y.ord) {
+        const uint32_t *ob = y.ord + ((x & 1023) << y.cap_log2);
+        uint16_t c = 0;
+        int64_t at = -1;
+        for (;;) {
+            const uint64_t w = tb[s];
+            if (w == YAK_EMPTY) return c;
+            if ((w >> 10) == key && (uint16_t)(w & 1023) >= min_count && (int64_t)ob[s] > at) at = ob[s], c = (uint16_t)(w & 1023);
+            s = (s + 1) & capm;
+        }
+    }
+    for (;;) {
+        const uint64_t w = tb[s];
+        if (w == YAK_EMPTY) return 0;
+        if ((w >> 10) == key) {
+            const uint16_t c = (uint16_t)(w & 1023);
+            return c >= min_count ? c : 0;
+        }
+        s = (s + 1) & capm;
+    }
+}
+
+__device__ __forceinline__ uint64_t yak_first(const YakDev &y, uint64_t x) {
+    const uint64_t capm = (1ULL << y.cap_log2) - 1;
+    return y.table[((x & 1023) << y.cap_log2) + ((x >> 10) & capm)];
+}
+__device__ __forceinline__ uint16_t yak_get_after(const YakDev &y, uint64_t x, uint16_t min_count, uint64_t w0) {
+    if (y.ord) return yak_get(y, x, min_count);
+    const uint64_t capm = (1ULL << y.cap_log2) - 1;
+    const uint64_t *tb = y.table + ((x & 1023) << y.cap_log2);
+    const uint64_t key = x >> 10;
+    uint64_t s = key & capm, w = w0;
+    for (;;) {
+        if (w == YAK_EMPTY) return 0;
+        if ((w >> 10) == key) {
+            const uint16_t c = (uint16_t)(w & 1023);
+            return c >= min_count ? c : 0;
+        }
+        s = (s + 1) & capm;
+        w = tb[s];
+    }
+}
+
+}
```
